# nv-tlabs/3dgrut

Measured on AMD Instinct MI355X. Metric: train rays/sec (3DGUT forward+backward, primary rays), higher is better.
Workload: dtype f32; 1 GPU; 3DGUT fwd+bwd, 1000000 Gaussians (cloud B trained-like, seed 42), 1920x1080, one view per GPU, SH degree 3, k_buffer 0; parallelism=view-dp1

## Files before the change

3dgrut_amd/_abi.py:

```python
from __future__ import annotations

import ctypes as C
import os

ABI_VERSION = 5
_HERE = os.path.dirname(os.path.abspath(__file__))
LIB_PATH = os.path.join(_HERE, "csrc", "libgrut_amd.so")

SHUTTER_ROLLING_TOP_TO_BOTTOM, SHUTTER_ROLLING_LEFT_TO_RIGHT, SHUTTER_ROLLING_BOTTOM_TO_TOP, \
    SHUTTER_ROLLING_RIGHT_TO_LEFT, SHUTTER_GLOBAL = range(5)
CAMERA_OPENCV_PINHOLE, CAMERA_OPENCV_FISHEYE, CAMERA_FTHETA = range(3)
FTHETA_PIXELDIST_TO_ANGLE, FTHETA_ANGLE_TO_PIXELDIST = range(2)

GUT_STAGES = ["project", "depth_sort", "scan", "expand", "tile_sort", "tile_ranges", "render_fwd", "render_bwd", "project_bwd"]

GRUT_OK = 0
STATUS_NAMES = {0: "OK", -1: "BAD_INPUT", -2: "RUNTIME", -3: "NOT_READY", -4: "UNSUPPORTED"}


class GrutCamera(C.Structure):
    _fields_ = [
        ("model", C.c_int32), ("shutter", C.c_int32), ("width", C.c_int32), ("height", C.c_int32),
        ("principal_point", C.c_float * 2), ("focal_length", C.c_float * 2),
        ("radial", C.c_float * 6), ("tangential", C.c_float * 2), ("thin_prism", C.c_float * 4),
# ... 26 lines not shown
        ("width", C.c_int32), ("height", C.c_int32), ("camera", GrutCamera),
        ("pose_start", C.c_float * 7), ("pose_end", C.c_float * 7),
        ("device_T_to_world", C.c_void_p), ("device_T_to_world_end", C.c_void_p), ("out_features", C.c_void_p), ("out_opacity", C.c_void_p),
    ]


class GutStats(C.Structure):
    _fields_ = [
        ("num_particles", C.c_uint32), ("num_visible", C.c_uint32), ("num_intersections", C.c_uint64),
        ("num_tiles", C.c_uint32), ("key_bits", C.c_uint32),
        ("fwd_entries_evaluated", C.c_uint64), ("fwd_entries_accepted", C.c_uint64),
        ("bwd_entries_evaluated", C.c_uint64), ("bwd_entries_accepted", C.c_uint64),
    ]


class GrtConfig(C.Structure):
    _fields_ = [
        ("particle_kernel_degree", C.c_int32), ("particle_kernel_min_response", C.c_float),
        ("particle_kernel_min_alpha", C.c_float), ("particle_kernel_max_alpha", C.c_float),
        ("particle_kernel_density_clamping", C.c_int32), ("particle_radiance_sph_degree", C.c_int32),
        ("enable_normals", C.c_int32), ("enable_hitcounts", C.c_int32), ("enable_kernel_timings", C.c_int32),
        ("max_hits_per_trace", C.c_int32), ("particle_feature_half", C.c_int32), ("feature_output_half", C.c_int32),
        ("feature_transform_type", C.c_int32), ("particle_feature_dim", C.c_int32), ("interp_point_feature_dim", C.c_int32),
        ("feature_interpolation_support", C.c_int32), ("feature_activation_type", C.c_int32), ("feature_activation_num_frequencies", C.c_int32),
        ("primitive_type", C.c_int32), ("pipeline_type", C.c_int32),
    ]


class GrtFrame(C.Structure):
    _fields_ = [
        ("frame_id", C.c_uint32), ("sph_degree", C.c_int32), ("min_transmittance", C.c_float),
        ("num_particles", C.c_uint32), ("width", C.c_int32), ("height", C.c_int32),
        ("ray_to_world", C.c_float * 12), ("keep_hits_for_backward", C.c_int32), ("device_ray_to_world", C.c_void_p),
    ]


class GrtStats(C.Structure):
    _fields_ = [
        ("num_particles", C.c_uint32), ("num_nodes", C.c_uint32), ("nodes_visited", C.c_uint64),
        ("candidates", C.c_uint64), ("processed_hits", C.c_uint64), ("scene_aabb", C.c_float * 6),
        ("list_entries", C.c_uint64), ("packet_tests", C.c_uint64), ("list_batches", C.c_uint64),
        ("bwd_rederived_rays", C.c_uint32), ("bwd_premise_rays", C.c_uint32),
        ("bwd_atomic_instructions", C.c_uint64), ("bwd_atomic_words", C.c_uint64),
    ]


class GrutAdamGroup(C.Structure):
    _fields_ = [
        ("param", C.c_void_p), ("grad", C.c_void_p), ("exp_avg", C.c_void_p), ("exp_avg_sq", C.c_void_p),
        ("row_width", C.c_uint32), ("lr", C.c_float), ("beta1", C.c_float), ("beta2", C.c_float), ("eps", C.c_float),
    ]


VIS_NONE, VIS_BOOL_U8, VIS_INT32, VIS_FLOAT_BITS = range(4)
GRT_PRIMITIVES = {"instances": 0, "icosahedron": 1, "octahedron": 2, "tetrahedron": 3, "diamond": 4, "custom": 5, "trisurfel": 6, "trihexa": 7, "sphere": 8}


class GrtTexture(C.Structure):
    _fields_ = [("data", C.c_void_p), ("height", C.c_int32), ("width", C.c_int32), ("channels", C.c_int32)]


class GrtMaterial(C.Structure):
    _fields_ = [("diffuse", GrtTexture), ("emissive", GrtTexture), ("metallic_roughness", GrtTexture), ("normal", GrtTexture),
                ("diffuse_factor", C.c_float * 4), ("emissive_factor", C.c_float * 3), ("metallic_factor", C.c_float), ("roughness_factor", C.c_float),
                ("transmission_factor", C.c_float), ("ior", C.c_float), ("alpha_cutoff", C.c_float), ("alpha_mode", C.c_uint32)]


class GrtMesh(C.Structure):
    _fields_ = [("num_vertices", C.c_uint32), ("num_faces", C.c_uint32), ("vertices", C.c_void_p), ("triangles", C.c_void_p),
                ("vertex_normals", C.c_void_p), ("vertex_tangents", C.c_void_p), ("vertex_has_tangents", C.c_void_p), ("prim_type", C.c_void_p),
                ("mat_uv", C.c_void_p), ("mat_id", C.c_void_p), ("refractive_index", C.c_void_p), ("num_materials", C.c_uint32),
                ("materials", C.POINTER(GrtMaterial)), ("envmap", GrtTexture), ("envmap_offset", C.c_float * 2)]


class GrtHybridOptions(C.Structure):
    _fields_ = [("playground_opts", C.c_uint32), ("max_pbr_bounces", C.c_uint32), ("frame_number", C.c_uint32)]



class GutGradIO(C.Structure):
    _fields_ = [("grad_features", C.c_void_p), ("grad_opacity", C.c_void_p), ("grad_positions", C.c_void_p), ("grad_density", C.c_void_p),
                ("grad_rotation", C.c_void_p), ("grad_scale", C.c_void_p)]

MLP_ACT_NONE, MLP_ACT_RELU, MLP_ACT_SIGMOID = range(3)
PPISP_CONTROLLER_SAVED = 1984


class GrutMlpConfig(C.Structure):
    _fields_ = [("n_features", C.c_int32), ("sh_degree", C.c_int32), ("n_hidden_layers", C.c_int32), ("width", C.c_int32),
                ("n_output_dims", C.c_int32), ("output_activation", C.c_int32)]


class GrutDecodeConfig(C.Structure):
    _fields_ = [("mlp", GrutMlpConfig), ("sh_scale", C.c_float), ("unpremultiply_alpha", C.c_int32), ("center_ray", C.c_int32)]


class GrutDenoiseConfig(C.Structure):
    _fields_ = [("patch_radius", C.c_int32), ("search_radius", C.c_int32), ("h", C.c_float)]


class McmcTensor(C.Structure):
    _fields_ = [("data", C.c_void_p), ("row_elems", C.c_uint32), ("role", C.c_uint32)]


MCMC_MAX_TENSORS = 32
MCMC_ROLE_COPY, MCMC_ROLE_NEW_DENSITY, MCMC_ROLE_NEW_SCALE, MCMC_ROLE_STATE = range(4)


EXPORTED_SYMBOLS = [
    "gut_create", "gut_destroy", "gut_forward", "gut_backward", "gut_backward_unpacked", "gut_forward_split", "gut_backward_split", "gut_backward_unpacked_split", "gut_backward_factored", "gut_backward_factored_chunked", "grut_sph_grad_from_views", "gut_timings", "gut_stats",
    "gut_profile_enable", "gut_profile_select", "gut_profile_read",
    "gut_debug_fetch", "gut_debug_fetch_work", "grut_debug_pose_from_c2w", "grut_debug_frame_poses", "grut_sort_pairs_u32", "grut_sort_scratch_bytes", "grut_inclusive_scan_u32",
    "grut_scan_scratch_bytes", "grut_debug_sort_pairs_u32", "grut_debug_scan_gather_u32", "gut_debug_tile_ranges", "grt_debug_list_ranges",
    "grt_create", "grt_destroy", "grt_build_bvh", "grt_forward", "grt_backward", "grt_timings", "grt_stats", "grt_debug_fetch_work",
    "grt_debug_forward_hits", "grt_debug_fetch_instances", "grt_debug_fetch_custom_boxes", "grt_debug_fetch_lists", "grt_debug_backward_signature", "grt_build_mesh_bvh", "grt_trace_hybrid",
    "grut_selective_adam_update", "grut_pack_particles", "grut_unpack_particle_grads", "grut_activate_pack", "grut_activate_pack_backward",
    "grut_reg_partials", "grut_reg_forward", "grut_reg_backward",
    "grut_denoise",
    "grut_mcmc_relocation", "grut_mcmc_perturb",
    "grut_mcmc_classify", "grut_mcmc_classify_scratch_bytes", "grut_mcmc_sample_plan", "grut_mcmc_relocate_rows", "grut_mcmc_append_rows",
    "grut_densify_accumulate", "grut_relayout_scan", "grut_relayout_scratch_bytes", "grut_relayout_rows", "grut_split_tail",
    "grut_ssim_forward", "grut_ssim_backward", "grut_ssim_partials",
    "grut_photo_loss_forward", "grut_photo_loss_backward", "grut_photo_loss_partials",
    "grut_knn", "grut_knn_scratch_bytes",
    "grut_ppisp_forward", "grut_ppisp_backward", "grut_ppisp_partials",
    "grut_ppisp_controller_forward", "grut_ppisp_controller_backward", "grut_ppisp_controller_forward_scratch", "grut_ppisp_controller_backward_scratch",
    "grut_mlp_forward", "grut_mlp_lds_bytes", "grut_mlp_num_params",
    "grut_mlp_backward", "grut_mlp_backward_lds_bytes", "grut_mlp_backward_scratch_bytes",
    "grut_decode_forward", "grut_decode_backward",
    "grut_last_error", "grut_abi_version", "grut_set_allocator", "gut_trim", "grt_trim",
]

_lib = None
ALLOC_FN = C.CFUNCTYPE(C.c_void_p, C.c_void_p, C.c_uint64)
FREE_FN = C.CFUNCTYPE(None, C.c_void_p, C.c_void_p)
CHUNK_FN = C.CFUNCTYPE(None, C.c_void_p, C.c_uint32, C.c_uint32, C.c_uint32)


def _declare(lib):
    vp, fp, ip, up = C.c_void_p, C.c_void_p, C.c_void_p, C.c_void_p
    lib.gut_create.argtypes = [C.POINTER(GutConfig), C.POINTER(C.c_void_p)]
    lib.gut_create.restype = C.c_int
    lib.gut_destroy.argtypes = [C.c_void_p]
    lib.gut_destroy.restype = None
    lib.gut_forward.argtypes = [C.c_void_p, vp, C.POINTER(GutFrame), fp, fp, fp, fp, fp, fp, fp, ip]
    lib.gut_forward.restype = C.c_int
    lib.gut_backward.argtypes = [C.c_void_p, vp, C.POINTER(GutFrame)] + [fp] * 10
    lib.gut_backward.restype = C.c_int
    lib.gut_backward_factored.argtypes = [C.c_void_p, vp, C.POINTER(GutFrame)] + [fp] * 10
    lib.gut_backward_factored.restype = C.c_int
    lib.gut_backward_factored_chunked.argtypes = [C.c_void_p, vp, C.POINTER(GutFrame)] + [fp] * 10 + [C.c_uint32, CHUNK_FN, C.c_void_p]
    lib.gut_backward_factored_chunked.restype = C.c_int
    lib.gut_backward_unpacked.argtypes = [C.c_void_p, vp, C.POINTER(GutFrame)] + [fp] * 7 + [C.POINTER(GutGradIO), fp]
    lib.gut_backward_unpacked.restype = C.c_int
    lib.gut_forward_split.argtypes = [C.c_void_p, vp, C.POINTER(GutFrame), fp, fp, fp, fp, fp, fp, fp, fp, ip]
    lib.gut_forward_split.restype = C.c_int
    lib.gut_backward_split.argtypes = [C.c_void_p, vp, C.POINTER(GutFrame)] + [fp] * 12
    lib.gut_backward_split.restype = C.c_int
    lib.gut_backward_unpacked_split.argtypes = [C.c_void_p, vp, C.POINTER(GutFrame)] + [fp] * 8 + [C.POINTER(GutGradIO), fp, fp]
    lib.gut_backward_unpacked_split.restype = C.c_int
    lib.grut_sph_grad_from_views.argtypes = [vp, C.c_uint32, C.c_uint32, fp, fp, C.c_uint32, C.c_int32, C.c_int32, C.c_float, fp]
    lib.grut_sph_grad_from_views.restype = C.c_int
    lib.gut_timings.argtypes = [C.c_void_p, C.POINTER(C.c_float), C.POINTER(C.c_float)]
    lib.gut_timings.restype = C.c_int
    lib.gut_stats.argtypes = [C.c_void_p, C.POINTER(GutStats)]
    lib.gut_stats.restype = C.c_int
    lib.gut_profile_enable.argtypes = [C.c_void_p, C.c_int]
    lib.gut_profile_enable.restype = C.c_int
    lib.gut_profile_select.argtypes = [C.c_void_p, C.c_uint32]
    lib.gut_profile_select.restype = C.c_int
    lib.gut_profile_read.argtypes = [C.c_void_p, C.POINTER(C.c_float)]
    lib.gut_profile_read.restype = C.c_int
    lib.gut_debug_fetch_work.argtypes = [C.c_void_p, vp, up, C.c_uint64]
    lib.gut_debug_fetch_work.restype = C.c_int
    lib.grut_debug_pose_from_c2w.argtypes = [C.POINTER(C.c_float), C.POINTER(C.c_float)]
    lib.grut_debug_pose_from_c2w.restype = C.c_int
    lib.grut_debug_frame_poses.argtypes = [vp, C.c_int, vp, vp, C.POINTER(C.c_float)]
    lib.grut_debug_frame_poses.restype = C.c_int
    lib.gut_debug_fetch.argtypes = [C.c_void_p, vp] + [up] * 8
    lib.gut_debug_fetch.restype = C.c_int
    lib.grut_sort_pairs_u32.argtypes = [vp, C.c_uint32, C.c_int, C.c_int, up, up, up, up, vp, C.c_uint64,
                                        C.POINTER(C.c_void_p), C.POINTER(C.c_void_p)]
    lib.grut_sort_pairs_u32.restype = C.c_int
    lib.grut_sort_scratch_bytes.argtypes = [C.c_uint32]
    lib.grut_sort_scratch_bytes.restype = C.c_uint64
    lib.grut_inclusive_scan_u32.argtypes = [vp, C.c_uint32, up, up, vp, C.c_uint64]
    lib.grut_inclusive_scan_u32.restype = C.c_int
    lib.grut_scan_scratch_bytes.argtypes = [C.c_uint32]
    lib.grut_scan_scratch_bytes.restype = C.c_uint64
    lib.grut_debug_sort_pairs_u32.argtypes = [vp, C.c_uint32, up, C.c_int, C.c_int, up, up, up, up, C.c_int, vp, C.c_uint64,
                                              C.POINTER(C.c_void_p), C.POINTER(C.c_void_p)]
    lib.grut_debug_sort_pairs_u32.restype = C.c_int
    lib.grut_debug_scan_gather_u32.argtypes = [vp, C.c_uint32, up, up, up, vp, C.c_uint64]
    lib.grut_debug_scan_gather_u32.restype = C.c_int
    lib.gut_debug_tile_ranges.argtypes = [vp, C.c_uint32, up, C.c_uint32, C.c_uint32, up, up, up, C.POINTER(C.c_uint32)]
    lib.gut_debug_tile_ranges.restype = C.c_int
    lib.grt_debug_list_ranges.argtypes = [vp, C.c_uint32, up, C.c_uint32, up, up]
    lib.grt_debug_list_ranges.restype = C.c_int
    lib.grt_debug_fetch_lists.argtypes = [C.c_void_p, vp, up, up, C.c_uint64]
    lib.grt_debug_fetch_lists.restype = C.c_int
    lib.grt_create.argtypes = [C.POINTER(GrtConfig), C.POINTER(C.c_void_p)]
    lib.grt_create.restype = C.c_int
    lib.grt_destroy.argtypes = [C.c_void_p]
    lib.grt_destroy.restype = None
    lib.grt_build_bvh.argtypes = [C.c_void_p, vp, C.c_uint32, fp, fp, fp, fp, C.c_int, C.c_int]
    lib.grt_build_bvh.restype = C.c_int
    lib.grt_forward.argtypes = [C.c_void_p, vp, C.POINTER(GrtFrame)] + [fp] * 9 + [ip]
    lib.grt_forward.restype = C.c_int
    lib.grt_backward.argtypes = [C.c_void_p, vp, C.POINTER(GrtFrame)] + [fp] * 14
    lib.grt_backward.restype = C.c_int
    lib.grt_debug_forward_hits.argtypes = [C.c_void_p, vp, C.POINTER(GrtFrame)] + [fp] * 9 + [ip, up, up, C.c_uint32]
    lib.grt_debug_forward_hits.restype = C.c_int
    lib.grt_debug_fetch_instances.argtypes = [C.c_void_p, vp, fp]
    lib.grt_debug_fetch_instances.restype = C.c_int
    lib.grt_debug_fetch_custom_boxes.argtypes = [C.c_void_p, vp, fp]
    lib.grt_debug_fetch_custom_boxes.restype = C.c_int
    lib.grt_debug_backward_signature.argtypes = [C.c_void_p, up, up]
    lib.grt_debug_backward_signature.restype = C.c_int
    lib.grt_build_mesh_bvh.argtypes = [C.c_void_p, vp, C.c_uint32, fp, C.c_uint32, ip, C.c_int, C.c_int]
    lib.grt_build_mesh_bvh.restype = C.c_int
    lib.grt_trace_hybrid.argtypes = [C.c_void_p, vp, C.POINTER(GrtFrame), fp, fp, fp, fp, fp, C.POINTER(GrtMesh), C.POINTER(GrtHybridOptions), fp, fp, fp, up]
    lib.grt_trace_hybrid.restype = C.c_int
    lib.grt_timings.argtypes = [C.c_void_p, C.POINTER(C.c_float), C.POINTER(C.c_float), C.POINTER(C.c_float)]
    lib.grt_timings.restype = C.c_int
    lib.grut_set_allocator.argtypes = [ALLOC_FN, FREE_FN, C.c_void_p]
    lib.grut_set_allocator.restype = C.c_int
    lib.gut_trim.argtypes = [C.c_void_p]
    lib.gut_trim.restype = C.c_int
    lib.grt_trim.argtypes = [C.c_void_p]
    lib.grt_trim.restype = C.c_int
    lib.grt_debug_fetch_work.argtypes = [C.c_void_p, vp, up, C.c_uint64]
    lib.grt_debug_fetch_work.restype = C.c_int
    lib.grt_stats.argtypes = [C.c_void_p, C.POINTER(GrtStats)]
    lib.grt_stats.restype = C.c_int
    lib.grut_selective_adam_update.argtypes = [vp, C.POINTER(GrutAdamGroup), C.c_int, C.c_uint32, vp, C.c_int]
    lib.grut_selective_adam_update.restype = C.c_int
    lib.grut_pack_particles.argtypes = [vp, C.c_uint32, fp, fp, fp, fp, fp]
    lib.grut_pack_particles.restype = C.c_int
    lib.grut_unpack_particle_grads.argtypes = [vp, C.c_uint32] + [fp] * 5
    lib.grut_unpack_particle_grads.restype = C.c_int
    lib.grut_activate_pack.argtypes = [vp, C.c_uint32, fp, fp, fp, fp, fp]
    lib.grut_activate_pack.restype = C.c_int
    lib.grut_activate_pack_backward.argtypes = [vp, C.c_uint32] + [fp] * 8
# ... 223 lines not shown
```

3dgrut_amd/csrc/gut_api.hip:

```cpp
#include <initializer_list>
#include <vector>

#include "gut_internal.hpp"

namespace grut {

static thread_local char g_last_error[512] = "";
ScratchAllocator& scratch_allocator() {
    static ScratchAllocator a;
    return a;
}
void set_last_error(const char* fmt, ...) {
    va_list ap;
    va_start(ap, fmt);
    vsnprintf(g_last_error, sizeof(g_last_error), fmt, ap);
    va_end(ap);
}

static uint32_t bits_for(uint32_t n) {
    uint32_t b = 1;
    while ((1ull << b) <= n) ++b;
    return b;
}

}

using namespace grut;

struct GutHandle {
    GutConfig cfg;
    int device = -1;
    DeviceBuffer tiles_count, proj_pos, conic_opacity, extent, depth, rgb, depth_key, particle_idx;
    DeviceBuffer depth_key_tmp, particle_idx_tmp, offsets, sort_scratch, scan_scratch, counters;
    DeviceBuffer rec64;
    DeviceBuffer part_offset, pos_particle, grad_partial, grad_flag, grad_touched, g_rgb, poses_dev, walk8;
    bool flags_dirty = false;
    DeviceBuffer tile_keys, tile_vals, tile_keys_tmp, tile_vals_tmp, tile_sort_scratch, ranges;
    DeviceBuffer ck_tc, ck_d, ck_reached, ck_boundary_tile, ck_nht;
    GutCheckpoints checkpoints;
    uint32_t* host_counters = nullptr;
    hipEvent_t count_event = nullptr;
    bool have_forward = false;
    hipStream_t fwd_stream = nullptr;
    const void* fwd_density = nullptr;
    const void* fwd_ray_o = nullptr;
    const void* fwd_ray_d = nullptr;
    uint32_t fwd_frame_id = 0;
    GutParams params;
    uint32_t num_intersections = 0;
    uint32_t tile_capacity = 0;
    uint32_t ck_boundaries_capacity = 0;
    uint32_t* sorted_pos = nullptr;
    uint32_t* sorted_tile_keys = nullptr;
    uint32_t* rank_to_particle = nullptr;
    GutStats stats;
    EventTimer fwd_timer, bwd_timer;
    bool profile = false;
    bool count_work = false;
    DeviceBuffer work_counters;
    unsigned long long work_host[4] = {0, 0, 0, 0};
    bool work_pending = false;
    static constexpr int kProfRing = 64;
    hipEvent_t prof_ev[kProfRing][GUT_NUM_STAGES][2];
    bool prof_used[kProfRing][GUT_NUM_STAGES];
    int prof_slot = 0, prof_created = 0;
    int prof_fwd_slot = 0;

    uint32_t profile_mask = 0xFFFFFFFFu;
    int stage_begin(int stage, hipStream_t s, int slot) {
        if (!profile || !((profile_mask >> stage) & 1u)) return GRUT_OK;
        GRUT_HIP(hipEventRecord(prof_ev[slot][stage][0], s));
        return GRUT_OK;
    }
    int stage_end(int stage, hipStream_t s, int slot) {
        if (!profile || !((profile_mask >> stage) & 1u)) return GRUT_OK;
        GRUT_HIP(hipEventRecord(prof_ev[slot][stage][1], s));
        prof_used[slot][stage] = true;
        return GRUT_OK;
    }
};

static int validate_config(const GutConfig& c) {
    GRUT_REQUIRE(c.ut_require_all_sigma_points_valid == 0, "ut_require_all_sigma_points_valid must be false (threedgut.cuh:78)");
    GRUT_REQUIRE(c.particle_radiance_sph_degree >= 0 && c.particle_radiance_sph_degree <= 3, "sph degree must be in [0,3]");
    if (c.k_buffer_size != 0 && c.k_buffer_size != 4 && c.k_buffer_size != 8 && c.k_buffer_size != 16) {
        set_last_error("k_buffer_size=%d: the hit buffer is instantiated for 0 (unsorted), 4, 8 and 16 entries", c.k_buffer_size);
        return GRUT_ERR_UNSUPPORTED;
    }
    if (c.feature_transform_type != 0) {
        GRUT_REQUIRE(c.feature_transform_type == 1, "feature_transform_type %d: 0 (SH) or 1 (neural harmonic features)", c.feature_transform_type);
        GRUT_REQUIRE(c.feature_interpolation_support == 0 || c.feature_interpolation_support == 1, "feature_interpolation_support must be 0 (centre) or 1 (tetrahedra)");
        GRUT_REQUIRE(c.feature_activation_type >= 0 && c.feature_activation_type <= 3, "feature_activation_type must be 0..3");
        const int points = c.feature_interpolation_support == 1 ? 4 : 1;
        GRUT_REQUIRE(c.interp_point_feature_dim >= 1 && c.interp_point_feature_dim <= 16 && c.particle_feature_dim == points * c.interp_point_feature_dim,
                     "particle_feature_dim %d must be %d x interp_point_feature_dim (1..16)", c.particle_feature_dim, points);
        const int nf = c.feature_activation_num_frequencies;
        const int nr = c.interp_point_feature_dim * (c.feature_activation_type == 2 ? 2 * nf : (c.feature_activation_type == 1 ? nf : 1));
        GRUT_REQUIRE(nf >= 1 && nr >= 1 && nr <= 32, "ray feature dim %d: 1..32 supported", nr);
    }
    const int d = c.particle_kernel_degree;
    GRUT_REQUIRE(d == 0 || d == 1 || d == 2 || d == 3 || d == 4 || d == 5 || d == 8, "unsupported particle_kernel_degree %d", d);
    return GRUT_OK;
}

static GutParams make_params(const GutConfig& c, const GutFrame& f) {
    GutParams P;
    memset(&P, 0, sizeof(P));
    P.degree = c.particle_kernel_degree;
    P.min_response = c.particle_kernel_min_response;
    P.min_alpha = c.particle_kernel_min_alpha;
    P.max_alpha = c.particle_kernel_max_alpha;
    P.min_transmittance = c.min_transmittance;
    P.n_active = f.n_active_features < c.particle_radiance_sph_degree ? f.n_active_features : c.particle_radiance_sph_degree;
    if (P.n_active < 0) P.n_active = 0;
    P.ncoef = (c.particle_radiance_sph_degree + 1) * (c.particle_radiance_sph_degree + 1);
    P.hitcounts = c.enable_hitcounts;
    const float D = 3.f;
    const float lambda = c.ut_alpha * c.ut_alpha * (D + c.ut_kappa) - D;
    P.ut_w0m = lambda / (D + lambda);
    P.ut_wi = 1.f / (2.f * (D + lambda));
    P.ut_w0c = lambda / (D + lambda) + (1.f - c.ut_alpha * c.ut_alpha + c.ut_beta);
    P.ut_delta = sqrtf(c.ut_alpha * c.ut_alpha * (D + c.ut_kappa));
    P.ut_margin = c.ut_in_image_margin_factor;
    P.ut_require_all = c.ut_require_all_sigma_points_valid;
    P.n_rs_iter = c.n_rolling_shutter_iterations;
    P.k_buffer = c.k_buffer_size;
    P.global_z = c.global_z_order;
// ... 48 lines not shown
}

static int ensure_intersection_scratch(GutHandle* h, uint32_t I, uint32_t tiles) {
    const size_t n = I ? I : 1;
    if (n > h->tile_capacity) h->tile_capacity = (uint32_t)n;
    GRUT_CHECK(h->tile_keys.ensure(n * 4, 1.3f));
    GRUT_CHECK(h->tile_vals.ensure(n * 4, 1.3f));
    GRUT_CHECK(h->tile_keys_tmp.ensure(n * 4, 1.3f));
    GRUT_CHECK(h->tile_vals_tmp.ensure(n * 4, 1.3f));
    GRUT_CHECK(h->pos_particle.ensure(n * 4, 1.3f));
    GRUT_CHECK(h->tile_sort_scratch.ensure(sort_scratch_bytes((uint32_t)n), 1.3f));
    GRUT_CHECK(h->ranges.ensure((size_t)tiles * 8 + 8));
    const size_t nb = (size_t)I / kGutSegment + 1;
    if (!h->params.nht && h->params.k_buffer == 0) {
        GRUT_CHECK(h->ck_tc.ensure(nb * 4 * 64 * 16, 1.3f));
        GRUT_CHECK(h->ck_d.ensure(nb * 4 * 64 * 4, 1.3f));
    }
    GRUT_CHECK(h->ck_reached.ensure(nb * 4, 1.3f));
    GRUT_CHECK(h->ck_boundary_tile.ensure(nb * 4, 1.3f));
    h->checkpoints.tc = h->ck_tc.as<float4>();
    h->checkpoints.d = h->ck_d.as<float>();
    h->checkpoints.reached = h->ck_reached.as<uint8_t>();
    h->checkpoints.boundary_tile = h->ck_boundary_tile.as<uint32_t>();
    h->checkpoints.num_boundaries = (uint32_t)nb;
    h->ck_boundaries_capacity = (uint32_t)nb;
    if (nht_fast_path(h->params)) GRUT_CHECK(h->ck_nht.ensure(nht_checkpoint_bytes((uint32_t)nb), 1.3f));
    return GRUT_OK;
}

static GutProjected projected_view(GutHandle* h) {
    GutProjected p;
    p.tiles_count = h->tiles_count.as<uint32_t>();
    p.proj_pos = h->proj_pos.as<float2>();
    p.conic_opacity = h->conic_opacity.as<float4>();
    p.extent = h->extent.as<float2>();
    p.depth = h->depth.as<float>();
    p.rgb = h->rgb.as<float>();
    p.depth_key = h->depth_key.as<uint32_t>();
    p.particle_idx = h->particle_idx.as<uint32_t>();
    p.part_offset = h->part_offset.as<uint32_t>();
    p.rec64 = h->rec64.as<float4>();
    static const bool no_walk_cache = getenv("GRUT_GUT_NO_WALK_CACHE") != nullptr;
    p.walk8 = (no_walk_cache || h->params.gx >= 4096 || h->params.gy >= 4096) ? nullptr : h->walk8.as<uint2>();
    return p;
}

extern "C" {

int grut_abi_version(void) { return GRUT_ABI_VERSION; }
int grut_set_allocator(GrutAllocFn alloc_fn, GrutFreeFn free_fn, void* user) {
    GRUT_REQUIRE((alloc_fn == nullptr) == (free_fn == nullptr), "grut_set_allocator: give both functions or neither");
    grut::ScratchAllocator& a = grut::scratch_allocator();
    a.alloc = alloc_fn;
    a.release = free_fn;
    a.user = user;
    return GRUT_OK;
}
const char* grut_last_error(void) { return grut::g_last_error; }

int gut_create(const GutConfig* config, GutHandle** handle) {
    GRUT_REQUIRE(config && handle, "gut_create: null argument");
    GRUT_CHECK(validate_config(*config));
    GutHandle* h = new GutHandle();
    h->cfg = *config;
    memset(&h->stats, 0, sizeof(h->stats));
    if (hipGetDevice(&h->device) != hipSuccess) {
        set_last_error("gut_create: no HIP device");
        delete h;
        return GRUT_ERR_RUNTIME;
    }
    if (hipHostMalloc(reinterpret_cast<void**>(&h->host_counters), 64, hipHostMallocDefault) != hipSuccess ||
        hipEventCreateWithFlags(&h->count_event, hipEventDisableTiming) != hipSuccess) {
        set_last_error("gut_create: pinned counter / event allocation failed");
        delete h;
        return GRUT_ERR_RUNTIME;
    }
    *handle = h;
    return GRUT_OK;
}

static void release_scratch(GutHandle* h) {
    DeviceBuffer* bufs[] = {&h->tiles_count, &h->proj_pos, &h->conic_opacity, &h->extent, &h->depth, &h->rgb, &h->depth_key,
                            &h->particle_idx, &h->depth_key_tmp, &h->particle_idx_tmp, &h->offsets, &h->sort_scratch,
                            &h->scan_scratch, &h->counters, &h->rec64, &h->walk8, &h->part_offset, &h->pos_particle, &h->grad_partial, &h->grad_flag,
                            &h->grad_touched,
                            &h->g_rgb, &h->poses_dev, &h->work_counters, &h->tile_keys, &h->tile_vals, &h->tile_keys_tmp,
                            &h->tile_vals_tmp, &h->tile_sort_scratch, &h->ranges, &h->ck_tc, &h->ck_d, &h->ck_nht, &h->ck_reached,
                            &h->ck_boundary_tile};
    for (DeviceBuffer* b : bufs) b->release();
}

int gut_trim(GutHandle* h) {
    GRUT_REQUIRE(h, "gut_trim: null handle");
    if (h->fwd_stream) GRUT_HIP(hipStreamSynchronize(h->fwd_stream));
    else GRUT_HIP(hipDeviceSynchronize());
    release_scratch(h);
    h->tile_capacity = 0;
    h->have_forward = false;
    h->num_intersections = 0;
    h->sorted_pos = nullptr;
    h->sorted_tile_keys = nullptr;
    h->work_pending = false;
    h->flags_dirty = false;
    h->ck_boundaries_capacity = 0;
    memset(&h->checkpoints, 0, sizeof(h->checkpoints));
    return GRUT_OK;
}

void gut_destroy(GutHandle* h) {
    if (!h) return;
    release_scratch(h);
    if (h->host_counters) (void)hipHostFree(h->host_counters);
    if (h->count_event) (void)hipEventDestroy(h->count_event);
    h->fwd_timer.destroy();
    h->bwd_timer.destroy();
    if (h->prof_created)
        for (int r = 0; r < GutHandle::kProfRing; ++r)
            for (int st = 0; st < GUT_NUM_STAGES; ++st) {
                (void)hipEventDestroy(h->prof_ev[r][st][0]);
                (void)hipEventDestroy(h->prof_ev[r][st][1]);
            }
    delete h;
}

static int forward_impl(GutHandle* h, void* stream_, const GutFrame* frame, const float* particle_density, const void* particle_sph_,
                        const GutSplitSph& split, const float* ray_origin, const float* ray_direction, void* out_feat_density_,
                        float* out_hit_distance, float* out_hit_count, int32_t* out_visibility) {
    const float* particle_sph = reinterpret_cast<const float*>(particle_sph_);
    float* out_feat_density = reinterpret_cast<float*>(out_feat_density_);
    GRUT_REQUIRE(h && frame, "gut_forward: null handle/frame");
    GRUT_REQUIRE(frame->width > 0 && frame->height > 0, "gut_forward: empty image");
    GRUT_REQUIRE(ray_origin && ray_direction && out_feat_density && out_hit_distance && out_hit_count, "gut_forward: null ray/output buffer");
    hipStream_t s = reinterpret_cast<hipStream_t>(stream_);
    ScratchStreamScope scratch_scope(s);
    h->have_forward = false;
    const uint32_t N = frame->num_particles;
    h->params = make_params(h->cfg, *frame);
    const GutParams& P = h->params;
    const uint32_t tiles = (uint32_t)(P.gx * P.gy);
    h->stats.num_particles = N;
    h->stats.num_tiles = tiles;
    h->stats.num_visible = 0;
    h->stats.num_intersections = 0;
    h->stats.key_bits = bits_for(tiles);
    h->num_intersections = 0;
    h->fwd_stream = s;
    h->fwd_density = particle_density;
    h->fwd_ray_o = ray_origin;
    h->fwd_ray_d = ray_direction;
    h->fwd_frame_id = frame->frame_id;
    if (N == 0) {
        h->have_forward = true;
        return GRUT_OK;
    }
    GRUT_REQUIRE(particle_density && (particle_sph || split.specular) && out_visibility, "gut_forward: null particle buffer");
    GRUT_REQUIRE(!h->cfg.feature_output_half || (!frame->out_features && !frame->out_opacity), "gut_forward: feature_output_half excludes out_features / out_opacity");
    GRUT_REQUIRE(!h->cfg.feature_transform_type || (!frame->out_features && !frame->out_opacity), "gut_forward: neural harmonic features exclude out_features / out_opacity");
    if (h->cfg.enable_kernel_timings) GRUT_CHECK(h->fwd_timer.begin(s));

    GRUT_CHECK(ensure_particle_scratch(h, N));
    static const bool legacy_lists = getenv("GRUT_GUT_LEGACY_LISTS") != nullptr;
    const bool direct = h->stats.key_bits <= 16 && !legacy_lists;
    h->params.rec64 = direct ? h->rec64.as<float4>() : nullptr;
    h->params.ord_shift = h->stats.key_bits;
    h->params.sorted_keys = nullptr;
    if (frame->device_T_to_world) {
        GRUT_CHECK(h->poses_dev.ensure(sizeof(FramePoses)));
        launch_frame_poses(s, frame->device_T_to_world, frame->device_T_to_world_end, h->poses_dev.as<FramePoses>());
        h->params.poses_dev = h->poses_dev.as<FramePoses>();
    }
    if (h->count_work) {
        const size_t fwd_words = 16 + 4 * ((((size_t)tiles + 7) & ~(size_t)7) * 2);
        GRUT_CHECK(h->work_counters.ensure(fwd_words * 8 + 8192 + ((size_t)h->tile_capacity / kGutSegment + tiles + 64) * 2 * 16, 1.2f));
        GRUT_HIP(hipMemsetAsync(h->work_counters.ptr, 0, h->work_counters.bytes, s));
        h->params.work = h->work_counters.as<unsigned long long>();
        h->params.work_task_capacity = (uint32_t)((h->work_counters.bytes / 8 - fwd_words) / 2);
        h->work_pending = true;
    }
    const GutProjected proj = projected_view(h);
    uint32_t* d_counters = h->counters.as<uint32_t>();

    const int slot = h->prof_slot % GutHandle::kProfRing;
    if (h->profile) {
        for (int st = 0; st < GUT_NUM_STAGES; ++st) h->prof_used[slot][st] = false;
        h->prof_fwd_slot = slot;
        h->prof_slot++;
    }
    GRUT_CHECK(h->stage_begin(GUT_STAGE_PROJECT, s, slot));
    launch_project(s, P, particle_density, particle_sph, split, proj, out_visibility, d_counters + 1);
    GRUT_CHECK(h->stage_end(GUT_STAGE_PROJECT, s, slot));
    GRUT_CHECK(h->stage_begin(GUT_STAGE_DEPTH_SORT, s, slot));
    uint32_t *sorted_depth = nullptr, *rank_to_particle = nullptr;
    GRUT_CHECK(sort_pairs_u32(s, N, nullptr, 0, 32, proj.depth_key, proj.particle_idx, h->depth_key_tmp.as<uint32_t>(),
                              h->particle_idx_tmp.as<uint32_t>(), h->sort_scratch.ptr, h->sort_scratch.bytes, &sorted_depth,
                              &rank_to_particle, true));
    h->rank_to_particle = rank_to_particle;
    GRUT_CHECK(h->stage_end(GUT_STAGE_DEPTH_SORT, s, slot));
    GRUT_CHECK(h->stage_begin(GUT_STAGE_SCAN, s, slot));
    GRUT_CHECK(inclusive_scan_u32(s, N, proj.tiles_count, rank_to_particle, h->offsets.as<uint32_t>(), h->scan_scratch.ptr,
                                  h->scan_scratch.bytes));
    GRUT_CHECK(h->stage_end(GUT_STAGE_SCAN, s, slot));
    GRUT_CHECK(h->ranges.ensure((size_t)tiles * 8 + 8));
    launch_prepare_tail(s, h->offsets.as<uint32_t>() + (N - 1), d_counters + 1, h->host_counters, h->ranges.as<uint32_t>(), tiles * 2u,
                        h->ck_reached.as<uint32_t>(), h->ck_reached.ptr ? h->ck_boundaries_capacity : 0u);
    GRUT_HIP(hipEventRecord(h->count_event, s));
    const uint32_t tile_mask = (h->stats.key_bits >= 32) ? 0xFFFFFFFFu : ((1u << h->stats.key_bits) - 1u);
    bool first_tail = true;
    auto enqueue_tail = [&](uint32_t n, const uint32_t* n_dev) -> int {
        GRUT_CHECK(h->stage_begin(GUT_STAGE_EXPAND, s, slot));
        launch_expand(s, P, proj, rank_to_particle, h->offsets.as<uint32_t>(), n, h->tile_keys.as<uint32_t>(),
                      direct ? h->tile_vals.as<uint32_t>() : nullptr , h->pos_particle.as<uint32_t>());
        GRUT_CHECK(h->stage_end(GUT_STAGE_EXPAND, s, slot));
        GRUT_CHECK(h->stage_begin(GUT_STAGE_TILE_SORT, s, slot));
        uint32_t *sorted_tiles = nullptr, *sorted_idx = nullptr;
        GRUT_CHECK(sort_pairs_u32(s, n, n_dev, 0, (int)h->stats.key_bits, h->tile_keys.as<uint32_t>(), h->tile_vals.as<uint32_t>(),
                                  h->tile_keys_tmp.as<uint32_t>(), h->tile_vals_tmp.as<uint32_t>(), h->tile_sort_scratch.ptr,
                                  h->tile_sort_scratch.bytes, &sorted_tiles, &sorted_idx, !direct));
        h->sorted_tile_keys = sorted_tiles;
        h->params.sorted_keys = sorted_tiles;
        h->sorted_pos = sorted_idx;
        GRUT_CHECK(h->stage_end(GUT_STAGE_TILE_SORT, s, slot));
        GRUT_CHECK(h->stage_begin(GUT_STAGE_TILE_RANGES, s, slot));
        if (!first_tail) {
            GRUT_HIP(hipMemsetAsync(h->ranges.ptr, 0, (size_t)tiles * 8, s));
            GRUT_HIP(hipMemsetAsync(h->ck_reached.ptr, 0, (size_t)h->ck_boundaries_capacity * 4, s));
        }
        first_tail = false;
        launch_tile_ranges(s, n, n_dev, tile_mask, tiles, sorted_tiles, h->ranges.as<uint32_t>(), h->checkpoints.boundary_tile);
        GRUT_CHECK(h->stage_end(GUT_STAGE_TILE_RANGES, s, slot));
        GRUT_CHECK(h->stage_begin(GUT_STAGE_RENDER_FWD, s, slot));
        if (nht_fast_path(P))
            launch_render_nhtp_fwd(s, P, h->ranges.as<uint32_t>(), sorted_idx, h->pos_particle.as<uint32_t>(), particle_density, particle_sph, ray_origin,
                                   ray_direction, out_feat_density, out_hit_distance, out_hit_count, h->ck_nht.ptr, h->checkpoints, true);
        else if (P.nht)
            launch_render_nht_fwd(s, P, h->ranges.as<uint32_t>(), sorted_idx, h->pos_particle.as<uint32_t>(), particle_density, particle_sph, ray_origin,
                                  ray_direction, out_feat_density, out_hit_distance, out_hit_count);
        else if (P.k_buffer > 0)
            launch_render_k_fwd(s, P, h->ranges.as<uint32_t>(), sorted_idx, h->pos_particle.as<uint32_t>(), particle_density, proj.rgb, ray_origin,
                                ray_direction, out_feat_density, out_hit_distance, out_hit_count);
        else
            launch_render_fwd(s, P, h->ranges.as<uint32_t>(), sorted_idx, h->pos_particle.as<uint32_t>(), particle_density, proj.rgb, ray_origin,
                              ray_direction, out_feat_density, out_hit_distance, out_hit_count, h->checkpoints, true);
        GRUT_CHECK(h->stage_end(GUT_STAGE_RENDER_FWD, s, slot));
        return GRUT_OK;
    };
    const bool speculative = h->tile_capacity > 0;
    if (speculative) GRUT_CHECK(enqueue_tail(h->tile_capacity, h->offsets.as<uint32_t>() + (N - 1)));
    GRUT_HIP(hipEventSynchronize(h->count_event));
    const uint32_t I = h->host_counters[0];
    h->stats.num_visible = h->host_counters[1];
    h->stats.num_intersections = I;
    h->num_intersections = I;
    if (I == 0) {
        const float far = 1e6f;
        uint32_t bits;
        memcpy(&bits, &far, 4);
        GRUT_HIP(hipMemsetAsync(out_feat_density, 0, (size_t)P.W * P.H * (P.nht ? P.nht_ray_dim + 1 : 4) * (P.out_half ? 2 : 4), s));
        GRUT_HIP(hipMemsetD32Async(reinterpret_cast<hipDeviceptr_t>(out_hit_distance), (int)bits, (size_t)P.W * P.H, s));
        GRUT_HIP(hipMemsetAsync(out_hit_count, 0, (size_t)P.W * P.H * 4, s));
        if (P.out_features) GRUT_HIP(hipMemsetAsync(P.out_features, 0, (size_t)P.W * P.H * 12, s));
        if (P.out_opacity) GRUT_HIP(hipMemsetAsync(P.out_opacity, 0, (size_t)P.W * P.H * 4, s));
        if (h->cfg.enable_kernel_timings) GRUT_CHECK(h->fwd_timer.end(s));
        h->have_forward = true;
        return GRUT_OK;
    }
    if (!speculative || I > h->tile_capacity) {
        GRUT_CHECK(ensure_intersection_scratch(h, I + I / 2, tiles));
        first_tail = false;
        GRUT_CHECK(enqueue_tail(I, nullptr));
    }
    h->checkpoints.num_boundaries = I / kGutSegment + 1;
    GRUT_HIP(hipGetLastError());
    if (h->cfg.enable_kernel_timings) GRUT_CHECK(h->fwd_timer.end(s));
    h->have_forward = true;
    return GRUT_OK;
}

int gut_forward(GutHandle* h, void* stream, const GutFrame* frame, const float* particle_density, const void* particle_sph,
                const float* ray_origin, const float* ray_direction, void* out_feat_density, float* out_hit_distance,
                float* out_hit_count, int32_t* out_visibility) {
    return forward_impl(h, stream, frame, particle_density, particle_sph, GutSplitSph{}, ray_origin, ray_direction, out_feat_density,
                        out_hit_distance, out_hit_count, out_visibility);
}

static int split_preconditions(const GutHandle* h, const char* who, std::initializer_list<const void*> buffers) {
    GRUT_REQUIRE(h, "%s: null handle", who);
    const GutConfig& cfg = h->cfg;
    const char* why = cfg.feature_transform_type ? "neural harmonic features have no albedo / specular tensors"
                      : cfg.particle_feature_half ? "particle_feature_half (the model's tensors are fp32)"
                      : cfg.particle_radiance_sph_degree != 3 ? "particle_radiance_sph_degree != 3 (the tensors are [N,3] and [N,45])"
                      : cfg.k_buffer_size != 0 ? "k_buffer_size > 0 (the sorted mode runs on the [N,48] buffer)" : nullptr;
    if (why) {
        set_last_error("%s: unsupported configuration: %s", who, why);
        return GRUT_ERR_UNSUPPORTED;
    }
    for (const void* p : buffers) {
        GRUT_REQUIRE(p, "%s: null albedo / specular buffer", who);
        GRUT_REQUIRE((reinterpret_cast<uintptr_t>(p) & 15u) == 0, "%s: the albedo / specular buffers must be 16-byte aligned", who);
    }
    return GRUT_OK;
}

int gut_forward_split(GutHandle* h, void* stream, const GutFrame* frame, const float* particle_density, const float* sph_albedo,
                      const float* sph_specular, const float* ray_origin, const float* ray_direction, void* out_feat_density,
                      float* out_hit_distance, float* out_hit_count, int32_t* out_visibility) {
    GRUT_CHECK(split_preconditions(h, "gut_forward_split", {sph_albedo, sph_specular}));
    return forward_impl(h, stream, frame, particle_density, nullptr, GutSplitSph{sph_albedo, sph_specular}, ray_origin, ray_direction,
                        out_feat_density, out_hit_distance, out_hit_count, out_visibility);
}

static int prepare_grad_slots(GutHandle* h, hipStream_t s, size_t I, GutGradSlots& slots) {
    const size_t touched_bytes = h->grad_touched.bytes, flag_bytes = h->grad_flag.bytes;
    GRUT_CHECK(h->grad_partial.ensure(2 * I * (size_t)slots.stride * 4, 1.3f));
    GRUT_CHECK(h->grad_touched.ensure((size_t)h->params.N * 8, 1.25f));
    GRUT_CHECK(h->grad_flag.ensure(2 * I, 1.3f));
    if (h->flags_dirty || h->grad_touched.bytes != touched_bytes) GRUT_HIP(hipMemsetAsync(h->grad_touched.ptr, 0, h->grad_touched.bytes, s));
    if (h->flags_dirty || h->grad_flag.bytes != flag_bytes) GRUT_HIP(hipMemsetAsync(h->grad_flag.ptr, 0, h->grad_flag.bytes, s));
    h->flags_dirty = true;
    slots.partial = h->grad_partial.as<float>();
    slots.touched = h->grad_touched.as<unsigned long long>();
    slots.flag = h->grad_flag.as<uint8_t>();
    return GRUT_OK;
}

static int backward_impl(GutHandle* h, void* stream_, const GutFrame* frame, const float* particle_density, const void* particle_sph_,
                         const float* ray_origin, const float* ray_direction, const void* feat_density_, const float* grad_feat_density,
                         const float* hit_distance, const float* grad_hit_distance, float* grad_particle_density, float* grad_particle_sph,
                         float* grad_radiance, const GutGradIO* io = nullptr, uint32_t num_chunks = 1, GrutChunkFn on_chunk = nullptr,
                         void* chunk_user = nullptr, const GutSplitSph& split = {}, const GutSplitSphGrad& g_split = {}) {
    const float* particle_sph = reinterpret_cast<const float*>(particle_sph_);
    const float* feat_density = reinterpret_cast<const float*>(feat_density_);
    GRUT_REQUIRE(h && frame, "gut_backward: null handle/frame");
    hipStream_t s = reinterpret_cast<hipStream_t>(stream_);
    ScratchStreamScope scratch_scope(s);
    if (!h->have_forward || h->fwd_stream != s) {
        set_last_error("gut_backward: no forward context on this stream");
        return GRUT_ERR_NOT_READY;
    }
    const GutParams& P = h->params;
    GRUT_REQUIRE(frame->num_particles == P.N && frame->width == P.W && frame->height == P.H, "gut_backward: frame differs from the forward frame");
    if (frame->frame_id != h->fwd_frame_id || (P.N > 0 && (particle_density != h->fwd_density || ray_origin != h->fwd_ray_o || ray_direction != h->fwd_ray_d))) {
        set_last_error("gut_backward: the forward context belongs to another forward (a later gut_forward ran on this handle before this "
                       "backward); run each backward before the next forward, or use one handle per in-flight frame");
        return GRUT_ERR_NOT_READY;
    }
    if (P.N == 0) return GRUT_OK;
    if (P.nht) {
        if (grad_radiance) {
            set_last_error("gut_backward_factored: neural harmonic features have no per-view factorisation; reduce the dense gradients");
            return GRUT_ERR_UNSUPPORTED;
        }
        const bool fast = nht_fast_path(P);
        if (io && !fast) {
            set_last_error("gut_backward_unpacked: this feature shape runs on the generic kernels, which write packed gradients only");
            return GRUT_ERR_UNSUPPORTED;
        }
        GRUT_REQUIRE(particle_density && particle_sph && feat_density && (io || grad_feat_density) && hit_distance && (io || grad_particle_density) &&
                         grad_particle_sph, "gut_backward: null buffer");
        if (h->cfg.enable_kernel_timings) GRUT_CHECK(h->bwd_timer.begin(s));
        GRUT_HIP(hipMemsetAsync(grad_particle_sph, 0, (size_t)P.N * P.nht_k * 4, s));
        const size_t I = h->num_intersections;
        if (fast) {
            const int slot = h->prof_fwd_slot;
            const GutProjected proj = projected_view(h);
            const GutGradOut g_out = io ? GutGradOut{nullptr, io->grad_positions, io->grad_density, io->grad_rotation, io->grad_scale}
                                        : GutGradOut{grad_particle_density, nullptr, nullptr, nullptr, nullptr};
            if (io) {
                GRUT_REQUIRE(io->grad_positions && io->grad_density && io->grad_rotation && io->grad_scale, "gut_backward_unpacked: null gradient output");
                GRUT_REQUIRE((reinterpret_cast<uintptr_t>(io->grad_rotation) & 15u) == 0, "gut_backward_unpacked: grad_rotation must be 16-byte aligned");
            }
            GutGradSlots slots;
            slots.stride = 16;
            slots.partial = nullptr;
            slots.touched = nullptr;
            slots.flag = nullptr;
            slots.pos_particle = h->pos_particle.as<uint32_t>();
            slots.part_offset = proj.part_offset;
            if (I > 0) {
                GRUT_CHECK(prepare_grad_slots(h, s, I, slots));
                GRUT_CHECK(h->stage_begin(GUT_STAGE_RENDER_BWD, s, slot));
                launch_render_nhtp_bwd(s, P, h->ranges.as<uint32_t>(), h->sorted_pos, particle_density, particle_sph, ray_origin, ray_direction, feat_density,
                                       io ? nullptr : grad_feat_density, io ? io->grad_features : nullptr, io ? io->grad_opacity : nullptr, hit_distance,
                                       grad_hit_distance, slots, grad_particle_sph, h->ck_nht.ptr, h->checkpoints);
                GRUT_CHECK(h->stage_end(GUT_STAGE_RENDER_BWD, s, slot));
            }
            GRUT_CHECK(h->stage_begin(GUT_STAGE_PROJECT_BWD, s, slot));
            launch_grad_finalize_nht(s, P, proj, particle_density, slots, I > 0, g_out);
            GRUT_CHECK(h->stage_end(GUT_STAGE_PROJECT_BWD, s, slot));
            GRUT_HIP(hipGetLastError());
            h->flags_dirty = false;
        } else {
            GRUT_HIP(hipMemsetAsync(grad_particle_density, 0, (size_t)P.N * 48, s));
            if (I > 0)
                launch_render_nht_bwd(s, P, h->ranges.as<uint32_t>(), h->sorted_pos, h->pos_particle.as<uint32_t>(), particle_density, particle_sph, ray_origin,
                                      ray_direction, feat_density, grad_feat_density, hit_distance, grad_hit_distance, grad_particle_density, grad_particle_sph);
        }
        GRUT_HIP(hipGetLastError());
        if (h->cfg.enable_kernel_timings) GRUT_CHECK(h->bwd_timer.end(s));
        return GRUT_OK;
    }
    const GutGradIn g_in = io ? GutGradIn{nullptr, io->grad_features, io->grad_opacity} : GutGradIn{grad_feat_density, nullptr, nullptr};
    const GutGradOut g_out = io ? GutGradOut{nullptr, io->grad_positions, io->grad_density, io->grad_rotation, io->grad_scale}
                                : GutGradOut{grad_particle_density, nullptr, nullptr, nullptr, nullptr};
    if (io) {
        GRUT_REQUIRE(io->grad_positions && io->grad_density && io->grad_rotation && io->grad_scale, "gut_backward_unpacked: null gradient output");
        GRUT_REQUIRE((reinterpret_cast<uintptr_t>(io->grad_rotation) & 15u) == 0, "gut_backward_unpacked: grad_rotation must be 16-byte aligned");
        if (P.k_buffer > 0) {
            set_last_error("gut_backward_unpacked: the sorted (k_buffer_size > 0) backward accumulates into packed rows; use gut_backward");
            return GRUT_ERR_UNSUPPORTED;
        }
    }
    GRUT_REQUIRE(particle_density && (particle_sph || split.specular) && feat_density && (io || grad_feat_density) && hit_distance &&
                     (io || grad_particle_density) && (grad_particle_sph || grad_radiance || g_split.specular), "gut_backward: null buffer");
    if (h->cfg.enable_kernel_timings) GRUT_CHECK(h->bwd_timer.begin(s));
    const GutProjected proj = projected_view(h);
    const int slot = h->prof_fwd_slot;
    const bool has_gdist = grad_hit_distance != nullptr;
    GutGradSlots slots;
    slots.stride = has_gdist ? 20 : 16;
    slots.partial = nullptr;
    slots.touched = nullptr;
    slots.flag = nullptr;
    slots.pos_particle = h->pos_particle.as<uint32_t>();
    slots.part_offset = proj.part_offset;
    const size_t I = h->num_intersections;
    if (P.k_buffer > 0) {
        GRUT_CHECK(h->g_rgb.ensure((size_t)P.N * 12, 1.25f));
        GRUT_HIP(hipMemsetAsync(h->g_rgb.ptr, 0, (size_t)P.N * 12, s));
        GRUT_HIP(hipMemsetAsync(grad_particle_density, 0, (size_t)P.N * 48, s));
        if (I > 0) {
            GRUT_CHECK(h->stage_begin(GUT_STAGE_RENDER_BWD, s, slot));
            launch_render_k_bwd(s, P, h->ranges.as<uint32_t>(), h->sorted_pos, h->pos_particle.as<uint32_t>(), particle_density, proj.rgb, ray_origin,
                                ray_direction, feat_density, grad_feat_density, hit_distance, grad_hit_distance, grad_particle_density,
                                h->g_rgb.as<float>());
            GRUT_CHECK(h->stage_end(GUT_STAGE_RENDER_BWD, s, slot));
        }
        GRUT_CHECK(h->stage_begin(GUT_STAGE_PROJECT_BWD, s, slot));
        launch_project_bwd(s, P, proj, particle_density, particle_sph, split, h->g_rgb.as<float>(), g_out, grad_particle_sph, g_split, grad_radiance);
        GRUT_CHECK(h->stage_end(GUT_STAGE_PROJECT_BWD, s, slot));
        GRUT_HIP(hipGetLastError());
        if (h->cfg.enable_kernel_timings) GRUT_CHECK(h->bwd_timer.end(s));
        return GRUT_OK;
    }
    if (I > 0) {
        GRUT_CHECK(prepare_grad_slots(h, s, I, slots));
        GRUT_CHECK(h->stage_begin(GUT_STAGE_RENDER_BWD, s, slot));
        launch_render_bwd(s, P, h->ranges.as<uint32_t>(), h->sorted_pos, particle_density, proj.rgb, ray_origin, ray_direction, feat_density,
                          g_in, hit_distance, grad_hit_distance, slots, h->checkpoints);
        GRUT_CHECK(h->stage_end(GUT_STAGE_RENDER_BWD, s, slot));
    }
    GRUT_CHECK(h->stage_begin(GUT_STAGE_PROJECT_BWD, s, slot));
    GRUT_CHECK(h->g_rgb.ensure((size_t)P.N * 12, 1.25f));
    if (num_chunks <= 1 || !on_chunk) {
        launch_grad_finalize(s, P, proj, particle_density, particle_sph, split, slots, has_gdist, I > 0, h->g_rgb.as<float>(), g_out,
                             grad_particle_sph, g_split, grad_radiance);
    } else {
        const uint32_t per = ((P.N + num_chunks - 1) / num_chunks + 127u) & ~127u;
        uint32_t c = 0;
        for (uint32_t first = 0; first < P.N; first += per, ++c) {
            const uint32_t end = first + per < P.N ? first + per : P.N;
            launch_grad_finalize(s, P, proj, particle_density, particle_sph, split, slots, has_gdist, I > 0, h->g_rgb.as<float>(), g_out,
                                 grad_particle_sph, g_split, grad_radiance, first, end);
            on_chunk(chunk_user, c, first, end - first);
        }
    }
    GRUT_CHECK(h->stage_end(GUT_STAGE_PROJECT_BWD, s, slot));
    GRUT_HIP(hipGetLastError());
    h->flags_dirty = false;
    if (h->cfg.enable_kernel_timings) GRUT_CHECK(h->bwd_timer.end(s));
    return GRUT_OK;
}

int gut_backward(GutHandle* h, void* stream, const GutFrame* frame, const float* particle_density, const void* particle_sph,
                 const float* ray_origin, const float* ray_direction, const void* feat_density, const float* grad_feat_density,
                 const float* hit_distance, const float* grad_hit_distance, float* grad_particle_density, float* grad_particle_sph) {
    return backward_impl(h, stream, frame, particle_density, particle_sph, ray_origin, ray_direction, feat_density, grad_feat_density, hit_distance,
                         grad_hit_distance, grad_particle_density, grad_particle_sph, nullptr);
}

int gut_backward_unpacked(GutHandle* h, void* stream, const GutFrame* frame, const float* particle_density, const void* particle_sph,
                          const float* ray_origin, const float* ray_direction, const void* feat_density, const float* hit_distance,
                          const float* grad_hit_distance, const GutGradIO* io, float* grad_particle_sph) {
    GRUT_REQUIRE(io, "gut_backward_unpacked: null GutGradIO");
    return backward_impl(h, stream, frame, particle_density, particle_sph, ray_origin, ray_direction, feat_density, nullptr, hit_distance,
                         grad_hit_distance, nullptr, grad_particle_sph, nullptr, io);
}

int gut_backward_split(GutHandle* h, void* stream, const GutFrame* frame, const float* particle_density, const float* sph_albedo,
                       const float* sph_specular, const float* ray_origin, const float* ray_direction, const void* feat_density,
                       const float* grad_feat_density, const float* hit_distance, const float* grad_hit_distance, float* grad_particle_density,
                       float* grad_sph_albedo, float* grad_sph_specular) {
    GRUT_CHECK(split_preconditions(h, "gut_backward_split", {sph_albedo, sph_specular, grad_sph_albedo, grad_sph_specular}));
    return backward_impl(h, stream, frame, particle_density, nullptr, ray_origin, ray_direction, feat_density, grad_feat_density, hit_distance,
                         grad_hit_distance, grad_particle_density, nullptr, nullptr, nullptr, 1, nullptr, nullptr,
                         GutSplitSph{sph_albedo, sph_specular}, GutSplitSphGrad{grad_sph_albedo, grad_sph_specular});
}

int gut_backward_unpacked_split(GutHandle* h, void* stream, const GutFrame* frame, const float* particle_density, const float* sph_albedo,
                                const float* sph_specular, const float* ray_origin, const float* ray_direction, const void* feat_density,
                                const float* hit_distance, const float* grad_hit_distance, const GutGradIO* io, float* grad_sph_albedo,
                                float* grad_sph_specular) {
    GRUT_CHECK(split_preconditions(h, "gut_backward_unpacked_split", {sph_albedo, sph_specular, grad_sph_albedo, grad_sph_specular}));
    GRUT_REQUIRE(io, "gut_backward_unpacked_split: null GutGradIO");
    return backward_impl(h, stream, frame, particle_density, nullptr, ray_origin, ray_direction, feat_density, nullptr, hit_distance,
                         grad_hit_distance, nullptr, nullptr, nullptr, io, 1, nullptr, nullptr, GutSplitSph{sph_albedo, sph_specular},
                         GutSplitSphGrad{grad_sph_albedo, grad_sph_specular});
}

int gut_backward_factored(GutHandle* h, void* stream, const GutFrame* frame, const float* particle_density, const void* particle_sph,
                          const float* ray_origin, const float* ray_direction, const void* feat_density, const float* grad_feat_density,
                          const float* hit_distance, const float* grad_hit_distance, float* grad_particle_density, float* grad_radiance) {
    GRUT_REQUIRE(grad_radiance, "gut_backward_factored: null buffer");
    return backward_impl(h, stream, frame, particle_density, particle_sph, ray_origin, ray_direction, feat_density, grad_feat_density, hit_distance,
                         grad_hit_distance, grad_particle_density, nullptr, grad_radiance);
}

int gut_backward_factored_chunked(GutHandle* h, void* stream, const GutFrame* frame, const float* particle_density, const void* particle_sph,
                                  const float* ray_origin, const float* ray_direction, const void* feat_density, const float* grad_feat_density,
                                  const float* hit_distance, const float* grad_hit_distance, float* grad_particle_density, float* grad_radiance,
                                  uint32_t num_chunks, GrutChunkFn on_chunk, void* user) {
    GRUT_REQUIRE(grad_radiance && on_chunk && num_chunks >= 1, "gut_backward_factored_chunked: null buffer / callback");
    GRUT_REQUIRE(!h || h->cfg.k_buffer_size == 0, "gut_backward_factored_chunked: the sorted mode finalises in one piece");
    return backward_impl(h, stream, frame, particle_density, particle_sph, ray_origin, ray_direction, feat_density, grad_feat_density, hit_distance,
                         grad_hit_distance, grad_particle_density, nullptr, grad_radiance, nullptr, num_chunks < 2 ? 2 : num_chunks, on_chunk, user);
}

int grut_sph_grad_from_views(void* stream, uint32_t num_particles, uint32_t num_views, const float* view_factors, const float* positions,
                             uint32_t position_stride, int32_t n_active_features, int32_t sph_degree, float scale, float* grad_particle_sph) {
    GRUT_REQUIRE(num_views > 0 && sph_degree >= 0 && sph_degree <= 3 && position_stride >= 3, "grut_sph_grad_from_views: bad arguments");
    if (num_particles == 0) return GRUT_OK;
    GRUT_REQUIRE(view_factors && positions && grad_particle_sph, "grut_sph_grad_from_views: null buffer");
    launch_sph_grad_from_views(reinterpret_cast<hipStream_t>(stream), num_particles, num_views, view_factors, positions, position_stride,
                               n_active_features, (sph_degree + 1) * (sph_degree + 1), scale, grad_particle_sph);
    GRUT_HIP(hipGetLastError());
    return GRUT_OK;
}

int gut_timings(GutHandle* h, float* forward_ms, float* backward_ms) {
    GRUT_REQUIRE(h, "gut_timings: null handle");
    if (forward_ms) *forward_ms = h->fwd_timer.collect();
    if (backward_ms) *backward_ms = h->bwd_timer.collect();
    return GRUT_OK;
}

int gut_profile_enable(GutHandle* h, int enable) {
    GRUT_REQUIRE(h, "gut_profile_enable: null handle");
    if (enable && h->prof_created == 0) {
        for (int r = 0; r < GutHandle::kProfRing; ++r)
            for (int st = 0; st < GUT_NUM_STAGES; ++st) {
                GRUT_HIP(hipEventCreate(&h->prof_ev[r][st][0]));
                GRUT_HIP(hipEventCreate(&h->prof_ev[r][st][1]));
                h->prof_used[r][st] = false;
            }
        h->prof_created = 1;
    }
    h->profile = enable != 0;
    h->count_work = enable >= 2;
    return GRUT_OK;
}

int gut_profile_select(GutHandle* h, uint32_t stage_mask) {
    GRUT_REQUIRE(h, "gut_profile_select: null handle");
    h->profile_mask = stage_mask;
    return GRUT_OK;
}

int gut_profile_read(GutHandle* h, float* stage_ms) {
    GRUT_REQUIRE(h && stage_ms, "gut_profile_read: null argument");
    GRUT_REQUIRE(h->prof_created, "gut_profile_read: profiling was never enabled");
    for (int st = 0; st < GUT_NUM_STAGES; ++st) {
        double sum = 0;
        int n = 0;
        for (int r = 0; r < GutHandle::kProfRing; ++r) {
            if (!h->prof_used[r][st]) continue;
            float ms = 0.f;
            GRUT_HIP(hipEventSynchronize(h->prof_ev[r][st][1]));
            GRUT_HIP(hipEventElapsedTime(&ms, h->prof_ev[r][st][0], h->prof_ev[r][st][1]));
            sum += ms;
            n++;
            h->prof_used[r][st] = false;
        }
        stage_ms[st] = n ? (float)(sum / n) : -1.f;
    }
    h->prof_slot = 0;
    return GRUT_OK;
}

int gut_stats(GutHandle* h, GutStats* stats) {
    GRUT_REQUIRE(h && stats, "gut_stats: null argument");
// ... 64 lines not shown
```

3dgrut_amd/csrc/gut_internal.hpp:

```cpp
#pragma once

#include "camera.hpp"
#include "common.hpp"

namespace grut {

struct GutParams {
    int degree;
    float min_response, min_alpha, max_alpha, min_transmittance;
    int n_active, ncoef, hitcounts;
    float ut_w0m, ut_wi, ut_w0c, ut_delta, ut_margin;
    int ut_require_all, n_rs_iter, k_buffer, global_z, rect_bounding, tight_opacity, tile_culling;
    int W, H, gx, gy;
    uint32_t N;
    GrutCamera cam;
    FramePoses poses;
    unsigned long long* work;
    const float4* rec64;
    const uint32_t* sorted_keys;
    uint32_t ord_shift;
    int nht, nht_k, nht_ipd, nht_support, nht_act, nht_nf, nht_ray_dim;
    int sph_half, out_half;
    uint32_t work_task_capacity;
    float* out_features;
    float* out_opacity;
    const FramePoses* poses_dev;
};
#ifdef __HIPCC__
__device__ __forceinline__ const FramePoses& frame_poses(const GutParams& P) { return P.poses_dev ? *P.poses_dev : P.poses; }
#endif
void launch_frame_poses(hipStream_t s, const float* T_start, const float* T_end, FramePoses* out);
void launch_prepare_tail(hipStream_t s, const uint32_t* last_offset, uint32_t* num_visible, uint32_t* host_counters, uint32_t* ranges_words,
                         uint32_t n_ranges_words, uint32_t* reached_words, uint32_t n_reached_words);

struct GutProjected {
    uint32_t* tiles_count;
    float2* proj_pos;
    float4* conic_opacity;
    float2* extent;
    float* depth;
    float* rgb;
    uint32_t* depth_key;
    uint32_t* particle_idx;
    uint32_t* part_offset;
    float4* rec64;
    uint2* walk8;
};

struct GutGradSlots {
    float* partial;
    unsigned long long* touched;
    uint8_t* flag;
    const uint32_t* pos_particle;
    const uint32_t* part_offset;
    int stride;
};
constexpr uint32_t kGutTouchBits = 64;

struct GutGradOut {
    float* packed;
    float* pos;
    float* dns;
    float* rot;
    float* scl;
};
struct GutGradIn {
    const float* fd;
    const float* rgb;
    const float* opa;
};
struct GutSplitSph {
    const float* albedo = nullptr;
    const float* specular = nullptr;
};
struct GutSplitSphGrad {
    float* albedo = nullptr;
    float* specular = nullptr;
};
#ifdef __HIPCC__
__device__ __forceinline__ float4 load_grad_in(const GutGradIn& g, size_t pix) {
    if (g.fd) return reinterpret_cast<const float4*>(g.fd)[pix];
    float4 r = make_float4(0.f, 0.f, 0.f, 0.f);
    if (g.rgb) { r.x = g.rgb[3 * pix]; r.y = g.rgb[3 * pix + 1]; r.z = g.rgb[3 * pix + 2]; }
    if (g.opa) r.w = g.opa[pix];
    return r;
}
#endif

#ifndef GRUT_GUT_SEGMENT
#define GRUT_GUT_SEGMENT 64
#endif
constexpr uint32_t kGutSegment = GRUT_GUT_SEGMENT;

struct GutCheckpoints {
    float4* tc;
    float* d;
    uint8_t* reached;
    uint32_t* boundary_tile;
    uint32_t num_boundaries;
};

constexpr uint32_t kGutCounterReplicas = 64, kGutCounterStride = 32, kGutCounterWords = kGutCounterReplicas * kGutCounterStride + 32;
void launch_project(hipStream_t s, const GutParams& P, const float* density12, const float* sph, const GutSplitSph& split, const GutProjected& out,
                    int32_t* visibility, uint32_t* num_visible);
void launch_expand(hipStream_t s, const GutParams& P, const GutProjected& proj, const uint32_t* rank_to_particle,
                   const uint32_t* offsets, uint32_t capacity, uint32_t* tile_keys, uint32_t* tile_vals, uint32_t* pos_particle);
void launch_gather_particle_idx(hipStream_t s, uint32_t n, const uint32_t* sorted_pos, const uint32_t* pos_particle, uint32_t* out);
void launch_tile_ranges(hipStream_t s, uint32_t n, const uint32_t* n_dev, uint32_t tile_mask, uint32_t num_tiles,
                        const uint32_t* sorted_tile_keys, uint32_t* ranges, uint32_t* boundary_tile);
void launch_render_fwd(hipStream_t s, const GutParams& P, const uint32_t* ranges, const uint32_t* sorted_pos, const uint32_t* pos_particle,
                       const float* density12,
                       const float* rgb, const float* ray_o, const float* ray_d, float* out_fd, float* out_dist, float* out_cnt,
                       const GutCheckpoints& ck, bool write_checkpoints);
void launch_render_bwd(hipStream_t s, const GutParams& P, const uint32_t* ranges, const uint32_t* sorted_pos, const float* density12,
                       const float* rgb, const float* ray_o, const float* ray_d, const float* fd, const GutGradIn& g_fd, const float* dist,
                       const float* g_dist, const GutGradSlots& slots, const GutCheckpoints& ck);
void launch_render_nht_fwd(hipStream_t s, const GutParams& P, const uint32_t* ranges, const uint32_t* sorted_pos, const uint32_t* pos_particle,
                           const float* density12, const float* features, const float* ray_o, const float* ray_d, float* out_fd, float* out_dist,
                           float* out_cnt);
void launch_render_nht_bwd(hipStream_t s, const GutParams& P, const uint32_t* ranges, const uint32_t* sorted_pos, const uint32_t* pos_particle,
                           const float* density12, const float* features, const float* ray_o, const float* ray_d, const float* fd, const float* g_fd,
                           const float* dist, const float* g_dist, float* g_density12, float* g_features);
bool nht_fast_path(const GutParams& P);
uint64_t nht_checkpoint_bytes(uint32_t num_boundaries);
void launch_render_nhtp_fwd(hipStream_t s, const GutParams& P, const uint32_t* ranges, const uint32_t* sorted_pos, const uint32_t* pos_particle,
                            const float* density12, const float* features, const float* ray_o, const float* ray_d, float* out_fd, float* out_dist,
                            float* out_cnt, void* ck_nht, const GutCheckpoints& ck, bool write_checkpoints);
void launch_render_nhtp_bwd(hipStream_t s, const GutParams& P, const uint32_t* ranges, const uint32_t* sorted_pos, const float* density12,
                            const float* features, const float* ray_o, const float* ray_d, const float* fd, const float* g_fd, const float* g_feat,
                            const float* g_opa, const float* dist, const float* g_dist, const GutGradSlots& slots, float* g_features,
                            const void* ck_nht, const GutCheckpoints& ck);
void launch_grad_finalize_nht(hipStream_t s, const GutParams& P, const GutProjected& proj, const float* density12, const GutGradSlots& slots,
                              bool have_partials, const GutGradOut& g_out);
void launch_render_k_fwd(hipStream_t s, const GutParams& P, const uint32_t* ranges, const uint32_t* sorted_pos, const uint32_t* pos_particle,
                         const float* density12, const float* rgb, const float* ray_o, const float* ray_d, float* out_fd, float* out_dist,
                         float* out_cnt);
void launch_render_k_bwd(hipStream_t s, const GutParams& P, const uint32_t* ranges, const uint32_t* sorted_pos, const uint32_t* pos_particle,
                         const float* density12, const float* rgb, const float* ray_o, const float* ray_d, const float* fd, const float* g_fd,
                         const float* dist, const float* g_dist, float* g_density12, float* g_rgb);
void launch_project_bwd(hipStream_t s, const GutParams& P, const GutProjected& proj, const float* density12, const float* sph,
                        const GutSplitSph& split, const float* g_rgb, const GutGradOut& g_out, float* g_sph, const GutSplitSphGrad& g_split,
                        float* g_radiance, uint32_t first = 0u, uint32_t end = 0xFFFFFFFFu);
void launch_grad_finalize(hipStream_t s, const GutParams& P, const GutProjected& proj, const float* density12, const float* sph,
                          const GutSplitSph& split, const GutGradSlots& slots, bool has_gdist, bool have_partials, float* g_rgb,
                          const GutGradOut& g_out, float* g_sph, const GutSplitSphGrad& g_split, float* g_radiance, uint32_t first = 0u,
                          uint32_t end = 0xFFFFFFFFu);
void launch_sph_grad_from_views(hipStream_t s, uint32_t N, uint32_t n_views, const float* factors, const float* positions, uint32_t pos_stride,
                                int n_active, int ncoef, float scale, float* g_sph);

}
```

3dgrut_amd/csrc/gut_kernels.hip:

```cpp
#include <cstdlib>

#include <hip/hip_fp16.h>

#include "gut_internal.hpp"

namespace grut {

namespace {

#define GRUT_SH_CONSTANTS                                                                                                   \
    constexpr float kC0 = 0.28209479177387814f, kC1 = 0.4886025119029199f;                                                  \
    constexpr float kC2[5] = {1.0925484305920792f, -1.0925484305920792f, 0.31539156525252005f, -1.0925484305920792f,        \
                              0.5462742152960396f};                                                                         \
    constexpr float kC3[7] = {-0.5900435899266435f, 2.890611442640554f, -0.4570457994644658f, 0.3731763325901154f,          \
                              -0.4570457994644658f, 1.445305721320277f, -0.5900435899266435f};                               \
    (void)kC0; (void)kC1; (void)kC2; (void)kC3

__device__ __forceinline__ void sh_basis(int deg, f3 d, float b[16]) {
    GRUT_SH_CONSTANTS;
    const float x = d.x, y = d.y, z = d.z;
#pragma unroll
    for (int i = 0; i < 16; ++i) b[i] = 0.f;
    b[0] = kC0;
    if (deg > 0) {
// ... 149 lines not shown

__device__ __forceinline__ int bcast_i(int v, int src) { return __builtin_amdgcn_readlane(v, src); }
__device__ __forceinline__ float bcast_f(float v, int src) { return __int_as_float(__builtin_amdgcn_readlane(__float_as_int(v), src)); }
template <typename Emit>
__device__ __forceinline__ void coop_tile_walk(int lane, int gx, bool culling, TileBBox bb, const TileConic& co, float cx, float cy, float pmax,
                                               Emit&& emit) {
    const int lx = lane & 7, ly = lane >> 3;
    for (int by = bb.miny; by < bb.maxy; by += 8)
        for (int bx = bb.minx; bx < bb.maxx; bx += 8) {
            const int x = bx + lx, y = by + ly;
            bool keep = (x < bb.maxx) && (y < bb.maxy);
            if (keep && culling) keep = tile_min_power((float)x, (float)y, co, cx, cy) < pmax;
            emit(keep, (uint32_t)(y * gx + x));
        }
}

constexpr int kRowWalkSide = 4;
__device__ __forceinline__ int row_bcast_i(int v, int src_lane) { return __shfl(v, src_lane, 64); }
__device__ __forceinline__ float row_bcast_f(float v, int src_lane) { return __shfl(v, src_lane, 64); }
template <typename Emit>
__device__ __forceinline__ void row_tile_walk(int lane, int gx, bool culling, bool active, TileBBox bb, const TileConic& co, float cx, float cy,
                                              float pmax, Emit&& emit) {
    const int lx = lane & 3, ly = (lane >> 2) & 3;
    int bx = bb.minx, by = bb.miny;
    bool run = active && bb.minx < bb.maxx && bb.miny < bb.maxy;
    while (__ballot(run)) {
        const int x = bx + lx, y = by + ly;
        bool keep = run && (x < bb.maxx) && (y < bb.maxy);
        if (keep && culling) keep = tile_min_power((float)x, (float)y, co, cx, cy) < pmax;
        emit(keep, (uint32_t)(y * gx + x));
        bx += 4;
        if (bx >= bb.maxx) {
            bx = bb.minx;
            by += 4;
            run = run && by < bb.maxy;
        }
    }
}
__device__ __forceinline__ int bbox_area(const TileBBox& b) { return (b.maxx - b.minx) * (b.maxy - b.miny); }
__device__ __forceinline__ bool bbox_fits_row(const TileBBox& b) { return (b.maxx - b.minx) <= kRowWalkSide && (b.maxy - b.miny) <= kRowWalkSide; }
__device__ __forceinline__ bool bbox_fits_half(const TileBBox& b) {
    const int w = b.maxx - b.minx, h = b.maxy - b.miny;
    return (w <= 8 && h <= 4) || (w <= 4 && h <= 8);
}
__device__ __forceinline__ bool half_block_tile(int lane, const TileBBox& b, int& x, int& y) {
    const int hl = lane & 31;
    const bool wide = (b.maxx - b.minx) > 4;
    x = b.minx + (wide ? (hl & 7) : (hl & 3));
    y = b.miny + (wide ? (hl >> 3) : (hl >> 2));
    return (x < b.maxx) && (y < b.maxy);
}
struct GroupPick {
    int rank;
    int steps;
};
template <int GROUP>
__device__ __forceinline__ GroupPick group_rank(int lane, bool member) {
    const unsigned long long m = __ballot(member);
    const int shift = lane & ~(GROUP - 1) & 63;
    const unsigned long long gmask = (GROUP == 64) ? ~0ull : ((1ull << GROUP) - 1ull);
    const unsigned long long mine = (m >> shift) & gmask;
    GroupPick g;
    g.rank = __popcll(mine & ((1ull << (lane & (GROUP - 1))) - 1ull));
    int steps = 0;
#pragma unroll
    for (int s = 0; s < 64; s += GROUP) steps = max(steps, (int)__popcll((m >> s) & gmask));
    g.steps = steps;
    return g;
}
template <int GROUP>
__device__ __forceinline__ int group_source(int lane, bool member, const GroupPick& g, int j, bool& act) {
    const unsigned long long sel = __ballot(member && g.rank == j);
    const int shift = lane & ~(GROUP - 1) & 63;
    const unsigned long long gmask = (GROUP == 64) ? ~0ull : ((1ull << GROUP) - 1ull);
    const unsigned long long mine = (sel >> shift) & gmask;
    act = mine != 0;
    return shift | (act ? (__ffsll((long long)mine) - 1) : 0);
}

struct __attribute__((packed, aligned(4))) Float4A4 {
    float x, y, z, w;
};

template <int MODEL, int ROLLING, bool SPLIT = false>
#ifndef GRUT_PROJECT_WAVES_MAX
#define GRUT_PROJECT_WAVES_MAX 6
#endif
__global__ __launch_bounds__(256) __attribute__((amdgpu_waves_per_eu(6, GRUT_PROJECT_WAVES_MAX))) void gut_project_kernel(GutParams P, const float4* __restrict__ density12,
                                                          const float* __restrict__ sph, GutProjected out,
                                                          int32_t* __restrict__ visibility, uint32_t* __restrict__ num_visible,
                                                          const float* __restrict__ sph_specular) {
    const uint32_t i = blockIdx.x * blockDim.x + threadIdx.x;
    const int lane = threadIdx.x & 63;
    const FramePoses& FP = frame_poses(P);
    bool has_tiles = false;
    uint32_t ntiles = 0;
    int vis = 0;
    float cx = 0.f, cy = 0.f, ex = 0.f, ey = 0.f, depth = 0.f, pmax_tile = 0.f, view_z_keep = 0.f;
    float4 co = make_float4(0.f, 0.f, 0.f, 0.f);
    TileBBox bb = {0, 0, 0, 0};
    f3 pos = mk3(0.f, 0.f, 0.f);
    float4 a = make_float4(0.f, 0.f, 0.f, 0.f), b = a, c = a;
    if (i < P.N) {
        a = density12[3 * (size_t)i + 0];
        b = density12[3 * (size_t)i + 1];
        c = density12[3 * (size_t)i + 2];
        pos = mk3(a.x, a.y, a.z);
        const float opacity = a.w;

        const float view_z = add_rn_u(FP.view_t[2], add_rn(add_rn(mul_rn_u(FP.view_R[6], pos.x), mul_rn_u(FP.view_R[7], pos.y)), mul_rn_u(FP.view_R[8], pos.z)));
        view_z_keep = view_z;
        bool ok = (opacity >= P.min_alpha) && (view_z >= 0.2f);
        if (ok) {
            const m3 rotT = quat_wxyz_to_rotT(b.x, b.y, b.z, b.w);
            float spx[7], spy[7];
            int nvalid = 0;
            nvalid += project_point_with_shutter<MODEL, ROLLING>(P.cam, FP, P.n_rs_iter, pos, P.ut_margin, spx[0], spy[0]) ? 1 : 0;
            cx = spx[0] * P.ut_w0m; cy = spy[0] * P.ut_w0m;
            const f3 axes[3] = {rotT.r0 * (P.ut_delta * c.x), rotT.r1 * (P.ut_delta * c.y), rotT.r2 * (P.ut_delta * c.z)};
#pragma unroll
            for (int k = 0; k < 3; ++k) {
                nvalid += project_point_with_shutter<MODEL, ROLLING>(P.cam, FP, P.n_rs_iter, pos + axes[k], P.ut_margin, spx[k + 1], spy[k + 1]) ? 1 : 0;
                cx += P.ut_wi * spx[k + 1]; cy += P.ut_wi * spy[k + 1];
                nvalid += project_point_with_shutter<MODEL, ROLLING>(P.cam, FP, P.n_rs_iter, pos - axes[k], P.ut_margin, spx[k + 4], spy[k + 4]) ? 1 : 0;
                cx += P.ut_wi * spx[k + 4]; cy += P.ut_wi * spy[k + 4];
            }
            ok = P.ut_require_all ? (nvalid == 7) : (nvalid > 0);
            if (ok) {
                float cov0, cov1, cov2;
                {
                    const float dx = spx[0] - cx, dy = spy[0] - cy;
                    cov0 = P.ut_w0c * dx * dx; cov1 = P.ut_w0c * dx * dy; cov2 = P.ut_w0c * dy * dy;
                }
#pragma unroll
                for (int k = 1; k < 7; ++k) {
                    const float dx = spx[k] - cx, dy = spy[k] - cy;
                    cov0 += P.ut_wi * dx * dx; cov1 += P.ut_wi * dx * dy; cov2 += P.ut_wi * dy * dy;
                }
                const float ca = cov0 + 0.3f, cb = cov1, cc = cov2 + 0.3f;
                const float det = ca * cc - cb * cb;
                ok = det != 0.f;
                if (ok) {
                    const float idet = 1.f / det;
                    co.x = cc * idet; co.y = -cb * idet; co.z = ca * idet;
                    const float cov_det = cov0 * cov2 - cov1 * cov1;
                    co.w = opacity * sqrtf(fmaxf(0.000025f, cov_det * idet));
                    ok = co.w >= P.min_alpha;
                    if (ok) {
                        const float pmax = logf(co.w / P.min_alpha);
                        const float ef = P.tight_opacity ? fminf(3.33f, sqrtf(2.f * pmax)) : 3.33f;
                        const float mid = 0.5f * (ca + cc);
                        const float lambda = mid + sqrtf(fmaxf(0.01f, mid * mid - det));
                        const float radius = ef * sqrtf(lambda);
                        ex = P.rect_bounding ? fminf(ef * sqrtf(ca), radius) : radius;
                        ey = P.rect_bounding ? fminf(ef * sqrtf(cc), radius) : radius;
                        ok = radius > 0.f;
                        if (ok) {
                            vis = 1;
                            bb = tile_space_bbox(P.gx, P.gy, cx, cy, ex, ey);
                            pmax_tile = logf(co.w / P.min_alpha);
                            if (!P.tile_culling) ntiles = (uint32_t)((bb.maxx - bb.minx) * (bb.maxy - bb.miny));
                        }
                    }
                }
            }
        }
    }
    uint32_t walk_mask = 0u, walk_kind = 0u;
    if (P.tile_culling) {
        const TileConic tc = tile_conic(co);
        const int area = vis ? bbox_area(bb) : 0;
        const bool small = area > 0 && bbox_fits_row(bb);
        const int row_shift = lane & 48;
        const GroupPick rows = group_rank<16>(lane, small);
        for (int k = 0; k < rows.steps; ++k) {
            bool act;
            const int src = group_source<16>(lane, small, rows, k, act);
            const TileBBox sb = {row_bcast_i(bb.minx, src), row_bcast_i(bb.miny, src), row_bcast_i(bb.maxx, src), row_bcast_i(bb.maxy, src)};
            const TileConic sco = {row_bcast_f(tc.cx, src), row_bcast_f(tc.cy, src), row_bcast_f(tc.cz, src), row_bcast_f(tc.rcpx, src),
                                   row_bcast_f(tc.rcpy, src)};
            uint32_t cnt = 0, m16 = 0u;
            row_tile_walk(lane, P.gx, true, act, sb, sco, row_bcast_f(cx, src), row_bcast_f(cy, src), row_bcast_f(pmax_tile, src),
                          [&](bool keep, uint32_t) { m16 = (uint32_t)((__ballot(keep) >> row_shift) & 0xFFFFull); cnt += (uint32_t)__popc(m16); });
            if (lane == src && act) { ntiles = cnt; walk_mask = m16; walk_kind = 1u; }
        }
        const bool halfc = area > 0 && !small && bbox_fits_half(bb);
        const int half_shift = lane & 32;
        const GroupPick halves = group_rank<32>(lane, halfc);
        for (int k = 0; k < halves.steps; ++k) {
// ... 296 lines not shown
}

constexpr uint32_t kGatherSmall = 32;

__device__ __forceinline__ float4 quat_contract(const float m[9], float4 q2) {
    const float r = q2.x, x = q2.y, y = q2.z, z = q2.w;
    const float m00 = m[0], m01 = m[1], m02 = m[2], m10 = m[3], m11 = m[4], m12 = m[5], m20 = m[6], m21 = m[7], m22 = m[8];
    const float s01 = m01 + m10, s02 = m02 + m20, s12 = m12 + m21;
    const float a01 = m01 - m10, a02 = m20 - m02, a12 = m12 - m21;
    float4 d;
    d.x = z * a01 + y * a02 + x * a12;
    d.y = y * s01 + z * s02 + r * a12 - 2.f * x * (m11 + m22);
    d.z = x * s01 + z * s12 + r * a02 - 2.f * y * (m00 + m22);
    d.w = x * s02 + y * s12 + r * a01 - 2.f * z * (m00 + m11);
    return d;
}

template <int STRIDE>
struct QuadAcc {
    float4 a;
    float4 x;
    __device__ __forceinline__ void clear() { a = make_float4(0.f, 0.f, 0.f, 0.f); x = a; }
    __device__ __forceinline__ void add_rows4(const float* __restrict__ partial, size_t sb, int b0, int b1, int b2, int b3, int c) {
        const float4 z = make_float4(0.f, 0.f, 0.f, 0.f);
        const float4* r0 = reinterpret_cast<const float4*>(partial + (sb + (size_t)b0) * STRIDE);
        const float4* r1 = reinterpret_cast<const float4*>(partial + (sb + (size_t)(b1 < 0 ? b0 : b1)) * STRIDE);
        const float4* r2 = reinterpret_cast<const float4*>(partial + (sb + (size_t)(b2 < 0 ? b0 : b2)) * STRIDE);
        const float4* r3 = reinterpret_cast<const float4*>(partial + (sb + (size_t)(b3 < 0 ? b0 : b3)) * STRIDE);
        const float4 v0 = r0[c], v1 = r1[c], v2 = r2[c], v3 = r3[c];
        float4 w0 = z, w1 = z, w2 = z, w3 = z;
        if (STRIDE > 16 && c == 0) { w0 = r0[4]; w1 = r1[4]; w2 = r2[4]; w3 = r3[4]; }
        a.x += v0.x; a.y += v0.y; a.z += v0.z; a.w += v0.w;
        if (b1 >= 0) { a.x += v1.x; a.y += v1.y; a.z += v1.z; a.w += v1.w; }
        if (b2 >= 0) { a.x += v2.x; a.y += v2.y; a.z += v2.z; a.w += v2.w; }
        if (b3 >= 0) { a.x += v3.x; a.y += v3.y; a.z += v3.z; a.w += v3.w; }
        if (STRIDE > 16 && c == 0) {
            x.x += w0.x; x.y += w0.y; x.z += w0.z; x.w += w0.w;
            if (b1 >= 0) { x.x += w1.x; x.y += w1.y; x.z += w1.z; x.w += w1.w; }
            if (b2 >= 0) { x.x += w2.x; x.y += w2.y; x.z += w2.z; x.w += w2.w; }
            if (b3 >= 0) { x.x += w3.x; x.y += w3.y; x.z += w3.z; x.w += w3.w; }
        }
    }
    __device__ __forceinline__ void add_row(const float* __restrict__ partial, size_t slot, int c) {
        const float4* row = reinterpret_cast<const float4*>(partial + slot * STRIDE);
        const float4 v = row[c];
        a.x += v.x; a.y += v.y; a.z += v.z; a.w += v.w;
        if (STRIDE > 16 && c == 0) {
            const float4 w = row[4];
            x.x += w.x; x.y += w.y; x.z += w.z; x.w += w.w;
        }
    }
};
template <int J>
__device__ __forceinline__ float quad_bcast(float v) {
    return __int_as_float(__builtin_amdgcn_update_dpp(0, __float_as_int(v), J | (J << 2) | (J << 4) | (J << 6), 0xf, 0xf, false));
}
template <int X>
__device__ __forceinline__ float quad_bcast_xor(float v) {
    constexpr int perm = X == 1 ? (1 | (0 << 2) | (3 << 4) | (2 << 6)) : (2 | (3 << 2) | (0 << 4) | (1 << 6));
    return __int_as_float(__builtin_amdgcn_update_dpp(0, __float_as_int(v), perm, 0xf, 0xf, false));
}
__device__ __forceinline__ float xor_sum_quads(float v) {
    v += __shfl_xor(v, 4, 64);
    v += __shfl_xor(v, 8, 64);
    v += __shfl_xor(v, 16, 64);
    v += __shfl_xor(v, 32, 64);
    return v;
}

__device__ __forceinline__ void store_split_sh_part(float* __restrict__ g_albedo, float* __restrict__ g_specular, size_t i, int c, const float (&o)[12]) {
    const bool first = c == 0;
    float* sp = g_specular + 45 * i + (first ? 0 : 12 * c - 3);
    Float4A4* w = reinterpret_cast<Float4A4*>(sp);
    w[0] = first ? Float4A4{o[3], o[4], o[5], o[6]} : Float4A4{o[0], o[1], o[2], o[3]};
    w[1] = first ? Float4A4{o[7], o[8], o[9], o[10]} : Float4A4{o[4], o[5], o[6], o[7]};
    if (first) {
        sp[8] = o[11];
        float* al = g_albedo + 3 * i;
        al[0] = o[0]; al[1] = o[1]; al[2] = o[2];
    } else {
        w[2] = Float4A4{o[8], o[9], o[10], o[11]};
    }
}
template <int STRIDE, bool NHT = false, bool FUSE_SH = false, bool SPLIT = false>
__global__ __launch_bounds__(256) void gut_grad_gather_kernel(GutParams P, GutProjected proj, const float4* __restrict__ density12,
                                                              GutGradSlots slots, int have_partials, GutGradOut g_out,
                                                              float* __restrict__ g_rgb, uint32_t first, uint32_t end,
                                                              const float* __restrict__ sph = nullptr, float* __restrict__ g_sph = nullptr,
                                                              const float* __restrict__ sph_specular = nullptr,
                                                              float* __restrict__ g_sph_specular = nullptr) {
    static_assert(!SPLIT || FUSE_SH, "split rows exist in the fused finalisation only");
    const int lane = threadIdx.x & 63, c = threadIdx.x & 3;
    const uint32_t i = first + blockIdx.x * 64u + (threadIdx.x >> 2);
    const uint32_t count = (i < end) ? proj.tiles_count[i] : 0u;
    const bool has = count != 0;
    QuadAcc<STRIDE> acc;
    acc.clear();
    const uint32_t off = (i < end) ? proj.part_offset[i] : 0u;
    const unsigned long long touched = (have_partials && i < end) ? slots.touched[i] : 0ull;
    float4 q = make_float4(1.f, 0.f, 0.f, 0.f), sc = make_float4(1.f, 1.f, 1.f, 0.f);
    if (has) { q = density12[3 * (size_t)i + 1]; sc = density12[3 * (size_t)i + 2]; }
    float4 sh0 = make_float4(0.f, 0.f, 0.f, 0.f), sh1 = sh0, sh2 = sh0, pa = sh0;
    f3 rad = mk3(0.f, 0.f, 0.f);
    if (FUSE_SH && has) {
        if (SPLIT) {
            const float* sp = sph_specular + 45 * (size_t)i + (c == 0 ? 0 : 12 * c - 3);
            const Float4A4 v0 = reinterpret_cast<const Float4A4*>(sp)[0], v1 = reinterpret_cast<const Float4A4*>(sp)[1];
            const Float4A4 v2 = *reinterpret_cast<const Float4A4*>(sp + (c == 0 ? 5 : 8));
            sh0 = make_float4(v0.x, v0.y, v0.z, v0.w);
            sh1 = make_float4(v1.x, v1.y, v1.z, v1.w);
            sh2 = make_float4(v2.x, v2.y, v2.z, v2.w);
            if (c == 0) {
                const float* al = sph + 3 * (size_t)i;
                sh0 = make_float4(al[0], al[1], al[2], v0.x);
                sh1 = make_float4(v0.y, v0.z, v0.w, v1.x);
                sh2 = make_float4(v1.y, v1.z, v1.w, v2.w);
            }
        } else {
            const float4* row = reinterpret_cast<const float4*>(sph + 48 * (size_t)i) + 3 * c;
            sh0 = row[0]; sh1 = row[1]; sh2 = row[2];
        }
        pa = density12[3 * (size_t)i];
        rad = mk3(proj.rgb[3 * (size_t)i], proj.rgb[3 * (size_t)i + 1], proj.rgb[3 * (size_t)i + 2]);
    }
    if (have_partials) {
        if (has && count <= kGatherSmall) {
            static_assert(2 * kGatherSmall <= kGutTouchBits, "the quad path reads its marks from the particle's word alone");
            const size_t sb = 2 * (size_t)off;
            const uint32_t nb = 2 * count;
            unsigned long long m = touched;
            if (nb < 64) m &= (1ull << nb) - 1ull;
            while (m) {
                const int b0 = __ffsll((long long)m) - 1;
                m &= m - 1;
                const int b1 = m ? __ffsll((long long)m) - 1 : -1;
                m &= m - 1;
                const int b2 = m ? __ffsll((long long)m) - 1 : -1;
                m &= m - 1;
                const int b3 = m ? __ffsll((long long)m) - 1 : -1;
                m &= m - 1;
                acc.add_rows4(slots.partial, sb, b0, b1, b2, b3, c);
            }
        }
        unsigned long long big = __ballot(has && count > kGatherSmall && c == 0);
        while (big) {
            const int src = __ffsll((long long)big) - 1;
            big &= big - 1;
            const size_t s0 = 2 * (size_t)(uint32_t)__builtin_amdgcn_readlane((int)off, src);
            const uint32_t n2 = 2u * (uint32_t)__builtin_amdgcn_readlane((int)count, src);
            QuadAcc<STRIDE> part;
            part.clear();
            const int g = lane >> 2;
            const unsigned long long m0 = (unsigned long long)(uint32_t)__builtin_amdgcn_readlane((int)(uint32_t)touched, src) |
                                          ((unsigned long long)(uint32_t)__builtin_amdgcn_readlane((int)(uint32_t)(touched >> 32), src) << 32);
#pragma nounroll
            for (uint32_t base = 0; base < n2; base += 64) {
                unsigned long long m = m0;
                if (base > 0) {
                    const bool set = (base + (uint32_t)lane < n2) && slots.flag[s0 + base + lane] != 0;
                    if (set) slots.flag[s0 + base + lane] = 0;
                    m = __ballot(set);
                }
                if (m == 0) continue;
                int b[4], nb = 0;
#pragma unroll
                for (int j = 0; j < 4; ++j)
                    if ((m >> (g + 16 * j)) & 1ull) b[nb++] = g + 16 * j;
                if (nb > 0)
                    part.add_rows4(slots.partial, s0 + base, b[0], nb > 1 ? b[1] : -1, nb > 2 ? b[2] : -1, nb > 3 ? b[3] : -1, c);
            }
            part.a.x = xor_sum_quads(part.a.x); part.a.y = xor_sum_quads(part.a.y);
            part.a.z = xor_sum_quads(part.a.z); part.a.w = xor_sum_quads(part.a.w);
            if (STRIDE > 16) {
                part.x.x = xor_sum_quads(part.x.x); part.x.y = xor_sum_quads(part.x.y);
                part.x.z = xor_sum_quads(part.x.z); part.x.w = xor_sum_quads(part.x.w);
            }
            if ((lane >> 2) == (src >> 2)) acc = part;
        }
        if (touched != 0ull && c == 0) slots.touched[i] = 0ull;
    }
    float r[20];
    r[0] = quad_bcast<0>(acc.a.x); r[1] = quad_bcast<0>(acc.a.y); r[2] = quad_bcast<0>(acc.a.z); r[3] = quad_bcast<0>(acc.a.w);
    r[4] = quad_bcast<1>(acc.a.x); r[5] = quad_bcast<1>(acc.a.y); r[6] = quad_bcast<1>(acc.a.z); r[7] = quad_bcast<1>(acc.a.w);
    r[8] = quad_bcast<2>(acc.a.x); r[9] = quad_bcast<2>(acc.a.y); r[10] = quad_bcast<2>(acc.a.z); r[11] = quad_bcast<2>(acc.a.w);
    r[12] = quad_bcast<3>(acc.a.x); r[13] = quad_bcast<3>(acc.a.y); r[14] = quad_bcast<3>(acc.a.z); r[15] = quad_bcast<3>(acc.a.w);
    r[16] = quad_bcast<0>(acc.x.x); r[17] = quad_bcast<0>(acc.x.y); r[18] = quad_bcast<0>(acc.x.z); r[19] = 0.f;
    if (i >= end) return;
    float4* gd = reinterpret_cast<float4*>(g_out.packed + 12 * (size_t)i);
    if (FUSE_SH && !has) {
        if (SPLIT) {
            const float zero[12] = {0.f, 0.f, 0.f, 0.f, 0.f, 0.f, 0.f, 0.f, 0.f, 0.f, 0.f, 0.f};
            store_split_sh_part(g_sph, g_sph_specular, (size_t)i, c, zero);
        } else {
            float4* out = reinterpret_cast<float4*>(g_sph + 48 * (size_t)i) + 3 * c;
            out[0] = out[1] = out[2] = make_float4(0.f, 0.f, 0.f, 0.f);
        }
    }
    if (!has) {
        if (g_out.packed) {
            if (c < 3) gd[c] = make_float4(0.f, 0.f, 0.f, 0.f);
        } else if (c == 0) {
            g_out.pos[3 * (size_t)i] = 0.f; g_out.pos[3 * (size_t)i + 1] = 0.f; g_out.pos[3 * (size_t)i + 2] = 0.f;
            g_out.dns[i] = 0.f;
        } else if (c == 1) {
            reinterpret_cast<float4*>(g_out.rot)[i] = make_float4(0.f, 0.f, 0.f, 0.f);
        } else if (c == 2) {
// ... 259 lines not shown
    } else {
        for (int row = 0; row < nrows; ++row)
            if (lane < rowlen) g_sph[(size_t)(wave_base + row) * rowlen + lane] = rows[row * kShStride + lane];
    }
}

__global__ __launch_bounds__(128) void sph_grad_from_views_kernel(uint32_t N, uint32_t n_views, const float* __restrict__ factors,
                                                                  const float* __restrict__ positions, uint32_t pos_stride, int n_active,
                                                                  int ncoef, float scale, float* __restrict__ g_sph) {
    __shared__ float s_rows[2][64 * kShStride];
    const int wave = threadIdx.x >> 6, lane = threadIdx.x & 63;
    const uint32_t wave_base = blockIdx.x * 128u + (uint32_t)wave * 64u;
    const uint32_t i = wave_base + lane;
    const int rowlen = 3 * ncoef;
    const int nact = min((n_active + 1) * (n_active + 1), ncoef);
    float* rows = s_rows[wave];
    float* myrow = rows + lane * kShStride;
    const int nrows = (int)min(64u, N > wave_base ? N - wave_base : 0u);
    if (i < N) {
        const f3 mu = mk3(positions[(size_t)i * pos_stride], positions[(size_t)i * pos_stride + 1], positions[(size_t)i * pos_stride + 2]);
        float acc[48];
#pragma unroll
        for (int k = 0; k < 48; ++k) acc[k] = 0.f;
        for (uint32_t v = 0; v < n_views; ++v) {
            const float* view = factors + (size_t)v * 3 * ((size_t)N + 1);
            const f3 g = mk3(view[3 * (size_t)i], view[3 * (size_t)i + 1], view[3 * (size_t)i + 2]);
            if (g.x == 0.f && g.y == 0.f && g.z == 0.f) continue;
            float ilen;
            const f3 dir = sh_view_direction(mu, mk3(view[3 * (size_t)N], view[3 * (size_t)N + 1], view[3 * (size_t)N + 2]), ilen);
            float basis[16];
            sh_basis_pinned(n_active, dir, basis);
#pragma unroll
            for (int k = 0; k < 16; ++k)
                if (k < nact) { acc[3 * k] = add_rn(acc[3 * k], mul_rn(basis[k], g.x)); acc[3 * k + 1] = add_rn(acc[3 * k + 1], mul_rn(basis[k], g.y)); acc[3 * k + 2] = add_rn(acc[3 * k + 2], mul_rn(basis[k], g.z)); }
        }
#pragma unroll
        for (int k = 0; k < 48; ++k)
            if (k < rowlen) myrow[k] = acc[k] * scale;
    }
    __syncthreads();
    if (rowlen == 48) {
        float4* dst = reinterpret_cast<float4*>(g_sph + (size_t)wave_base * 48);
        const int total4 = nrows * 12;
#pragma unroll
        for (int it = 0; it < 12; ++it) {
            const int q = lane + 64 * it;
            if (q < total4) {
                const float* d = rows + (q / 12) * kShStride + 4 * (q % 12);
                dst[q] = make_float4(d[0], d[1], d[2], d[3]);
            }
        }
    } else {
        for (int row = 0; row < nrows; ++row)
            if (lane < rowlen) g_sph[(size_t)(wave_base + row) * rowlen + lane] = rows[row * kShStride + lane];
    }
}

__global__ __launch_bounds__(256) void gut_prepare_tail_kernel(const uint32_t* __restrict__ last_offset, uint32_t* __restrict__ num_visible,
                                                               uint32_t* __restrict__ host_counters, uint32_t* __restrict__ ranges_words,
                                                               uint32_t n_ranges_words, uint32_t* __restrict__ reached_words, uint32_t n_reached_words) {
    const uint32_t i = blockIdx.x * blockDim.x + threadIdx.x, stride = gridDim.x * blockDim.x;
    if (blockIdx.x == 0 && threadIdx.x < 64) {
        uint32_t v = 0u;
        if (threadIdx.x < kGutCounterReplicas) { v = num_visible[threadIdx.x * kGutCounterStride]; num_visible[threadIdx.x * kGutCounterStride] = 0u; }
#pragma unroll
        for (int o = 32; o >= 1; o >>= 1) v += __shfl_xor(v, o, 64);
        if (threadIdx.x == 0) {
            __hip_atomic_store(&host_counters[0], *last_offset, __ATOMIC_RELAXED, __HIP_MEMORY_SCOPE_SYSTEM);
            __hip_atomic_store(&host_counters[1], v, __ATOMIC_RELAXED, __HIP_MEMORY_SCOPE_SYSTEM);
        }
    }
    for (uint32_t k = i; k < n_ranges_words; k += stride) ranges_words[k] = 0u;
    for (uint32_t k = i; k < n_reached_words; k += stride) reached_words[k] = 0u;
}

}

void launch_prepare_tail(hipStream_t s, const uint32_t* last_offset, uint32_t* num_visible, uint32_t* host_counters, uint32_t* ranges_words,
                         uint32_t n_ranges_words, uint32_t* reached_words, uint32_t n_reached_words) {
    hipLaunchKernelGGL(gut_prepare_tail_kernel, dim3(64), dim3(256), 0, s, last_offset, num_visible, host_counters, ranges_words, n_ranges_words,
                       reached_words, n_reached_words);
}

void launch_project(hipStream_t s, const GutParams& P, const float* density12, const float* sph, const GutSplitSph& split, const GutProjected& out,
                    int32_t* visibility, uint32_t* num_visible) {
#define GRUT_PROJECT_LAUNCH(M_, R_)                                                                                                                 \
    do {                                                                                                                                            \
        if (split.specular)                                                                                                                         \
            hipLaunchKernelGGL((gut_project_kernel<M_, R_, true>), dim3(div_up(P.N, 256)), dim3(256), 0, s, P,                                      \
                               reinterpret_cast<const float4*>(density12), split.albedo, out, visibility, num_visible, split.specular);           \
        else                                                                                                                                        \
            hipLaunchKernelGGL((gut_project_kernel<M_, R_, false>), dim3(div_up(P.N, 256)), dim3(256), 0, s, P,                                     \
                               reinterpret_cast<const float4*>(density12), sph, out, visibility, num_visible, static_cast<const float*>(nullptr)); \
    } while (0)
    const bool rolling = P.cam.shutter != GRUT_SHUTTER_GLOBAL;
    switch (P.cam.model) {
    case GRUT_CAMERA_OPENCV_PINHOLE: if (rolling) GRUT_PROJECT_LAUNCH(GRUT_CAMERA_OPENCV_PINHOLE, 1); else GRUT_PROJECT_LAUNCH(GRUT_CAMERA_OPENCV_PINHOLE, 0); break;
    case GRUT_CAMERA_OPENCV_FISHEYE: if (rolling) GRUT_PROJECT_LAUNCH(GRUT_CAMERA_OPENCV_FISHEYE, 1); else GRUT_PROJECT_LAUNCH(GRUT_CAMERA_OPENCV_FISHEYE, 0); break;
    case GRUT_CAMERA_FTHETA: if (rolling) GRUT_PROJECT_LAUNCH(GRUT_CAMERA_FTHETA, 1); else GRUT_PROJECT_LAUNCH(GRUT_CAMERA_FTHETA, 0); break;
    default: GRUT_PROJECT_LAUNCH(-1, 1); break;
    }
#undef GRUT_PROJECT_LAUNCH
}
void launch_expand(hipStream_t s, const GutParams& P, const GutProjected& proj, const uint32_t* rank_to_particle,
                   const uint32_t* offsets, uint32_t capacity, uint32_t* tile_keys, uint32_t* tile_vals, uint32_t* pos_particle) {
    hipLaunchKernelGGL(gut_expand_kernel, dim3(div_up(P.N, 256)), dim3(256), 0, s, P, proj, rank_to_particle, offsets, capacity,
                       tile_keys, tile_vals, pos_particle);
}
void launch_gather_particle_idx(hipStream_t s, uint32_t n, const uint32_t* sorted_pos, const uint32_t* pos_particle, uint32_t* out) {
    if (n) hipLaunchKernelGGL(gut_gather_particle_idx_kernel, dim3(div_up(n, 256)), dim3(256), 0, s, n, sorted_pos, pos_particle, out);
}
void launch_tile_ranges(hipStream_t s, uint32_t n, const uint32_t* n_dev, uint32_t tile_mask, uint32_t num_tiles,
                        const uint32_t* sorted_tile_keys, uint32_t* ranges, uint32_t* boundary_tile) {
    hipLaunchKernelGGL(gut_tile_ranges_kernel, dim3(div_up(div_up(n, 4u), 256)), dim3(256), 0, s, n, n_dev, tile_mask, num_tiles, sorted_tile_keys,
                       reinterpret_cast<uint2*>(ranges), boundary_tile);
}

void launch_project_bwd(hipStream_t s, const GutParams& P, const GutProjected& proj, const float* density12, const float* sph,
                        const GutSplitSph& split, const float* g_rgb, const GutGradOut& g_out, float* g_sph, const GutSplitSphGrad& g_split,
                        float* g_radiance, uint32_t first, uint32_t end) {
    if (end > P.N) end = P.N;
    if (end <= first) return;
    if (split.specular)
        hipLaunchKernelGGL((gut_project_bwd_kernel<false, true>), dim3(div_up(end - first, 128)), dim3(128), 0, s, P, proj.tiles_count,
                           reinterpret_cast<const float4*>(density12), split.albedo, proj.rgb, g_rgb, g_out, g_split.albedo, g_radiance, first, end,
                           split.specular, g_split.specular);
    else if (g_radiance)
        hipLaunchKernelGGL(gut_project_bwd_kernel<true>, dim3(div_up(end - first, 128)), dim3(128), 0, s, P, proj.tiles_count,
                           reinterpret_cast<const float4*>(density12), sph, proj.rgb, g_rgb, g_out, g_sph, g_radiance, first, end);
    else
        hipLaunchKernelGGL(gut_project_bwd_kernel<false>, dim3(div_up(end - first, 128)), dim3(128), 0, s, P, proj.tiles_count,
                           reinterpret_cast<const float4*>(density12), sph, proj.rgb, g_rgb, g_out, g_sph, g_radiance, first, end);
}
void launch_sph_grad_from_views(hipStream_t s, uint32_t N, uint32_t n_views, const float* factors, const float* positions, uint32_t pos_stride,
                                int n_active, int ncoef, float scale, float* g_sph) {
    hipLaunchKernelGGL(sph_grad_from_views_kernel, dim3(div_up(N, 128)), dim3(128), 0, s, N, n_views, factors, positions, pos_stride, n_active,
                       ncoef, scale, g_sph);
}
void launch_grad_finalize_nht(hipStream_t s, const GutParams& P, const GutProjected& proj, const float* density12, const GutGradSlots& slots,
                              bool have_partials, const GutGradOut& g_out) {
    hipLaunchKernelGGL((gut_grad_gather_kernel<16, true>), dim3(div_up(P.N, 64)), dim3(256), 0, s, P, proj, reinterpret_cast<const float4*>(density12),
                       slots, have_partials ? 1 : 0, g_out, static_cast<float*>(nullptr), 0u, P.N);
}
void launch_grad_finalize(hipStream_t s, const GutParams& P, const GutProjected& proj, const float* density12, const float* sph,
                          const GutSplitSph& split, const GutGradSlots& slots, bool has_gdist, bool have_partials, float* g_rgb,
                          const GutGradOut& g_out, float* g_sph, const GutSplitSphGrad& g_split, float* g_radiance, uint32_t first, uint32_t end) {
    if (end > P.N) end = P.N;
    if (end <= first) return;
    const dim3 grid(div_up(end - first, 64)), block(256);
    static const bool unfused = [] { const char* e = getenv("GRUT_GUT_UNFUSED_FINALIZE"); return e && e[0] == '1'; }();
    if (!unfused && split.specular) {
        if (has_gdist)
            hipLaunchKernelGGL((gut_grad_gather_kernel<20, false, true, true>), grid, block, 0, s, P, proj, reinterpret_cast<const float4*>(density12),
                               slots, have_partials ? 1 : 0, g_out, g_rgb, first, end, split.albedo, g_split.albedo, split.specular, g_split.specular);
        else
            hipLaunchKernelGGL((gut_grad_gather_kernel<16, false, true, true>), grid, block, 0, s, P, proj, reinterpret_cast<const float4*>(density12),
                               slots, have_partials ? 1 : 0, g_out, g_rgb, first, end, split.albedo, g_split.albedo, split.specular, g_split.specular);
        return;
    }
    if (!unfused && !g_radiance && g_sph && P.ncoef == 16 && !P.sph_half) {
        if (has_gdist)
            hipLaunchKernelGGL((gut_grad_gather_kernel<20, false, true>), grid, block, 0, s, P, proj, reinterpret_cast<const float4*>(density12), slots,
                               have_partials ? 1 : 0, g_out, g_rgb, first, end, sph, g_sph);
        else
            hipLaunchKernelGGL((gut_grad_gather_kernel<16, false, true>), grid, block, 0, s, P, proj, reinterpret_cast<const float4*>(density12), slots,
                               have_partials ? 1 : 0, g_out, g_rgb, first, end, sph, g_sph);
        return;
    }
    if (has_gdist)
        hipLaunchKernelGGL(gut_grad_gather_kernel<20>, grid, block, 0, s, P, proj, reinterpret_cast<const float4*>(density12), slots,
                           have_partials ? 1 : 0, g_out, g_rgb, first, end);
    else
        hipLaunchKernelGGL(gut_grad_gather_kernel<16>, grid, block, 0, s, P, proj, reinterpret_cast<const float4*>(density12), slots,
                           have_partials ? 1 : 0, g_out, g_rgb, first, end);
    launch_project_bwd(s, P, proj, density12, sph, split, g_rgb, g_out, g_sph, g_split, g_radiance, first, end);
}

}
```

3dgrut_amd/gut_tracer.py:

```python
from __future__ import annotations

import ctypes as C
import os

import torch

from . import _abi
from .camera import camera_from_batch

_FALSE_DEFAULTS = dict(
    particle_kernel_degree=2, particle_kernel_min_response=0.0113, particle_kernel_min_alpha=1.0 / 255.0,
    particle_kernel_max_alpha=0.99, min_transmittance=0.0001, particle_radiance_sph_degree=3,
    enable_hitcounts=True, enable_kernel_timings=False)
_SPLAT_DEFAULTS = dict(
    ut_alpha=1.0, ut_beta=2.0, ut_kappa=0.0, ut_in_image_margin_factor=0.1, ut_require_all_sigma_points_valid=False,
    n_rolling_shutter_iterations=5, k_buffer_size=0, global_z_order=True, rect_bounding=True,
    tight_opacity_bounding=True, tile_based_culling=True)


def _conf_get(node, name, default=None):
    if node is None:
        return default
    if isinstance(node, dict):
        return node.get(name, default)
# ... 5 lines not shown
            return node[name]
        except Exception:
            return default


def fused_activations_requested(conf) -> bool:
    return bool(_conf_get(_conf_get(conf, "render"), "fused_activations", False)) or bool(os.environ.get("GRUT_FUSED_ACTIVATIONS"))


def split_sh_requested(conf) -> bool:
    return bool(_conf_get(_conf_get(conf, "render"), "split_sh_features", False)) or bool(os.environ.get("GRUT_SPLIT_SH"))


def has_standard_activations(gaussians) -> bool:
    return (all(hasattr(gaussians, a) for a in ("density", "rotation", "scale", "density_activation", "scale_activation", "rotation_activation"))
            and gaussians.density_activation is torch.sigmoid and gaussians.scale_activation is torch.exp
            and gaussians.rotation_activation is torch.nn.functional.normalize)


def nht_config_from_conf(conf, cfg) -> bool:
    model = _conf_get(conf, "model")
    if str(_conf_get(model, "feature_type", "sh")).lower() != "nht":
        return False
    nf = _conf_get(model, "nht_features")
    act = _conf_get(nf, "activation")
    interp = str(_conf_get(nf, "interpolation_type", "none")).lower()
    if interp not in ("none", "barycentric"):
        raise NotImplementedError(f"3dgrut_amd: nht_features.interpolation_type={interp!r} (the reference supports none / barycentric)")
    points = 4 if interp == "barycentric" else 1
    dim = int(_conf_get(nf, "dim", 48))
    if dim % points:
        raise ValueError(f"nht_features.dim = {dim} is not divisible by the {points} interpolation points of interpolation_type={interp!r}")
    cfg.feature_transform_type = 1
    cfg.particle_feature_dim = dim
    cfg.interp_point_feature_dim = dim // points
    cfg.feature_interpolation_support = 1 if points == 4 else 0
    act_name = str(_conf_get(act, "type", "none") if act is not None else "none").lower()
    if act_name not in ("none", "siren", "sincos", "relu"):
        raise ValueError(f"Unknown nht_features.activation.type: {act_name}")
    cfg.feature_activation_type = {"none": 0, "siren": 1, "sincos": 2, "relu": 3}[act_name]
    cfg.feature_activation_num_frequencies = 1 if act_name in ("none", "relu") else int(_conf_get(act, "num_frequencies", 1))
    return True


def ray_feature_dim_of(cfg) -> int:
    if not cfg.feature_transform_type:
        return 3
    a, n = cfg.feature_activation_type, cfg.feature_activation_num_frequencies
    return cfg.interp_point_feature_dim * (2 * n if a == 2 else (n if a == 1 else 1))


def gut_config_from_conf(conf) -> _abi.GutConfig:
    render = _conf_get(conf, "render")
    splat = _conf_get(render, "splat")
    cfg = _abi.GutConfig()
    for k, d in _FALSE_DEFAULTS.items():
        v = _conf_get(render, k, d)
        setattr(cfg, k, type(d)(v) if not isinstance(d, bool) else int(bool(v)))
    for k, d in _SPLAT_DEFAULTS.items():
        v = _conf_get(splat, k, d)
        setattr(cfg, k, type(d)(v) if not isinstance(d, bool) else int(bool(v)))
    nht_config_from_conf(conf, cfg)
    cfg.particle_feature_half = int(bool(_conf_get(render, "particle_feature_half", False)))
    cfg.feature_output_half = int(bool(_conf_get(render, "feature_output_half", False)))
    if _conf_get(splat, "fine_grained_load_balancing", False):
        pass
    return cfg


def _ptr(t):
    return C.c_void_p(t.data_ptr()) if t is not None else None


def _stream_ptr(device):
    return C.c_void_p(torch.cuda.current_stream(device).cuda_stream)


def _uninitialised(shape, **opts):
    if os.environ.get("GRUT_POISON_OUTPUTS"):
        return torch.full(shape, float("nan") if opts.get("dtype") == torch.float32 else -1, **opts)
    return torch.empty(shape, **opts)


class _GutNative:

    def __init__(self, cfg: _abi.GutConfig):
        if not torch.cuda.is_available():
            raise RuntimeError("3dgrut_amd.Tracer needs a ROCm GPU (there is no CPU fallback)")
        torch.zeros(1, device="cuda")
        self.lib = _abi.load_library()
        self.cfg = cfg
        self.handle = C.c_void_p()
        _abi.check(self.lib.gut_create(C.byref(cfg), C.byref(self.handle)), "gut_create")
        self.ncoef = (cfg.particle_radiance_sph_degree + 1) ** 2
        self._timings = {}

    def __del__(self):
        try:
            if getattr(self, "handle", None) and self.handle.value:
                self.lib.gut_destroy(self.handle)
                self.handle = C.c_void_p()
        except Exception:
            pass

    def make_frame(self, frame_id, n_active, n, height, width, cam, pose_start, pose_end) -> _abi.GutFrame:
        f = _abi.GutFrame()
        f.frame_id, f.n_active_features, f.num_particles = int(frame_id) & 0xFFFFFFFF, int(n_active), int(n)
        f.width, f.height = int(width), int(height)
        f.camera = cam
        for i in range(7):
            f.pose_start[i] = float(pose_start[i])
            f.pose_end[i] = float(pose_end[i])
        return f

    def trace(self, frame, particle_density, particle_sph, ray_ori, ray_dir):
        return self._trace(frame, particle_density, (particle_sph,), ray_ori, ray_dir)

    def trace_split(self, frame, particle_density, sph_albedo, sph_specular, ray_ori, ray_dir):
        return self._trace(frame, particle_density, (sph_albedo, sph_specular), ray_ori, ray_dir)

    def _trace(self, frame, particle_density, sph, ray_ori, ray_dir):
        dev = ray_ori.device
        H, W = frame.height, frame.width
        N = frame.num_particles
        opts = dict(dtype=torch.float32, device=dev)
        half_out = bool(self.cfg.feature_output_half)
        fd_opts = dict(dtype=torch.float16 if half_out else torch.float32, device=dev)
        if N == 0:
            out_fd = torch.zeros((H, W, 4), **fd_opts)
            out_dist = torch.full((H, W, 1), 1e6, **opts)
            out_cnt = torch.zeros((H, W, 1), **opts)
            vis_i32 = torch.zeros((N, 1), dtype=torch.int32, device=dev)
        else:
            out_fd = _uninitialised((H, W, 4), **fd_opts)
            out_dist = _uninitialised((H, W, 1), **opts)
            out_cnt = _uninitialised((H, W, 1), **opts) if self.cfg.enable_hitcounts else torch.zeros((H, W, 1), **opts)
            vis_i32 = _uninitialised((N, 1), dtype=torch.int32, device=dev)
        if half_out:
            out_feat = out_opa = None
        elif N == 0:
            out_feat, out_opa = torch.zeros((H, W, 3), **opts), torch.zeros((H, W, 1), **opts)
        else:
            out_feat, out_opa = _uninitialised((H, W, 3), **opts), _uninitialised((H, W, 1), **opts)
        frame.out_features, frame.out_opacity = (None, None) if half_out else (out_feat.data_ptr(), out_opa.data_ptr())
        fn, name = (self.lib.gut_forward, "gut_forward") if len(sph) == 1 else (self.lib.gut_forward_split, "gut_forward_split")
        _abi.check(fn(self.handle, _stream_ptr(dev), C.byref(frame), _ptr(particle_density), *map(_ptr, sph),
                      _ptr(ray_ori), _ptr(ray_dir), _ptr(out_fd), _ptr(out_dist), _ptr(out_cnt), _ptr(vis_i32)), name)
        frame.out_features, frame.out_opacity = None, None
        if half_out:
            f32 = out_fd.float()
            out_feat, out_opa = f32[..., :3].contiguous(), f32[..., 3:].contiguous()
        return out_fd, out_dist, out_cnt, vis_i32.view(torch.float32), out_feat, out_opa

    @property
    def ray_feature_dim(self):
        return ray_feature_dim_of(self.cfg)

    def trace_nht(self, frame, particle_density, particle_features, ray_ori, ray_dir):
        dev = ray_ori.device
        H, W, N = frame.height, frame.width, frame.num_particles
        nr = self.ray_feature_dim
        fd = torch.zeros((H, W, nr + 1), dtype=torch.float16 if self.cfg.feature_output_half else torch.float32, device=dev)
        dist = torch.full((H, W, 1), 1e6, dtype=torch.float32, device=dev)
        cnt = torch.zeros((H, W, 1), dtype=torch.float32, device=dev)
        vis = torch.zeros((N, 1), dtype=torch.int32, device=dev)
        if self.cfg.particle_feature_half and particle_features.dtype != torch.float16:
            particle_features = particle_features.to(torch.float16)
        _abi.check(self.lib.gut_forward(self.handle, _stream_ptr(dev), C.byref(frame), _ptr(particle_density), _ptr(particle_features.contiguous()),
                                        _ptr(ray_ori), _ptr(ray_dir), _ptr(fd), _ptr(dist), _ptr(cnt), _ptr(vis)), "gut_forward")
        return fd, dist, cnt, vis.view(torch.float32), particle_features

    def trace_bwd_nht(self, frame, particle_density, particle_features, ray_ori, ray_dir, fd, g_fd, dist, g_dist):
        dev = ray_ori.device
        g_density = torch.empty_like(particle_density)
        g_feat = torch.empty(particle_features.shape, dtype=torch.float32, device=dev)
        _abi.check(self.lib.gut_backward(self.handle, _stream_ptr(dev), C.byref(frame), _ptr(particle_density), _ptr(particle_features),
                                         _ptr(ray_ori), _ptr(ray_dir), _ptr(fd), _ptr(g_fd), _ptr(dist), _ptr(g_dist),
                                         _ptr(g_density), _ptr(g_feat)), "gut_backward")
        return g_density, g_feat

    def trace_bwd(self, frame, particle_density, particle_sph, ray_ori, ray_dir, fd, g_fd, dist, g_dist):
        dev = ray_ori.device
        g_density = torch.empty_like(particle_density)
        g_sph = torch.empty_like(particle_sph, dtype=torch.float32)
        _abi.check(self.lib.gut_backward(self.handle, _stream_ptr(dev), C.byref(frame), _ptr(particle_density), _ptr(particle_sph),
                                         _ptr(ray_ori), _ptr(ray_dir), _ptr(fd), _ptr(g_fd), _ptr(dist), _ptr(g_dist),
                                         _ptr(g_density), _ptr(g_sph)), "gut_backward")
        return g_density, g_sph

    def trace_bwd_unpacked(self, frame, particle_density, particle_sph, ray_ori, ray_dir, fd, g_feat, g_opa, dist, g_dist):
        dev = ray_ori.device
        n = particle_density.shape[0]
        opts = dict(dtype=torch.float32, device=dev)
        g_pos, g_dns, g_rot, g_scl = torch.empty((n, 3), **opts), torch.empty((n, 1), **opts), torch.empty((n, 4), **opts), torch.empty((n, 3), **opts)
        g_sph = torch.empty_like(particle_sph, dtype=torch.float32)
        io = _abi.GutGradIO(_ptr(g_feat), _ptr(g_opa), _ptr(g_pos), _ptr(g_dns), _ptr(g_rot), _ptr(g_scl))
        _abi.check(self.lib.gut_backward_unpacked(self.handle, _stream_ptr(dev), C.byref(frame), _ptr(particle_density), _ptr(particle_sph),
                                                  _ptr(ray_ori), _ptr(ray_dir), _ptr(fd), _ptr(dist), _ptr(g_dist), C.byref(io), _ptr(g_sph)),
                   "gut_backward_unpacked")
        return g_pos, g_dns, g_rot, g_scl, g_sph

    def trace_bwd_split(self, frame, particle_density, sph_albedo, sph_specular, ray_ori, ray_dir, fd, g_fd, dist, g_dist):
        g_density, g_albedo, g_specular = torch.empty_like(particle_density), torch.empty_like(sph_albedo), torch.empty_like(sph_specular)
        _abi.check(self.lib.gut_backward_split(self.handle, _stream_ptr(ray_ori.device), C.byref(frame), _ptr(particle_density), _ptr(sph_albedo),
                                               _ptr(sph_specular), _ptr(ray_ori), _ptr(ray_dir), _ptr(fd), _ptr(g_fd), _ptr(dist), _ptr(g_dist),
                                               _ptr(g_density), _ptr(g_albedo), _ptr(g_specular)), "gut_backward_split")
        return g_density, g_albedo, g_specular

    def trace_bwd_unpacked_split(self, frame, particle_density, sph_albedo, sph_specular, ray_ori, ray_dir, fd, g_feat, g_opa, dist, g_dist):
        n = particle_density.shape[0]
        opts = dict(dtype=torch.float32, device=ray_ori.device)
        g_pos, g_dns, g_rot, g_scl = torch.empty((n, 3), **opts), torch.empty((n, 1), **opts), torch.empty((n, 4), **opts), torch.empty((n, 3), **opts)
        g_albedo, g_specular = torch.empty_like(sph_albedo), torch.empty_like(sph_specular)
        io = _abi.GutGradIO(_ptr(g_feat), _ptr(g_opa), _ptr(g_pos), _ptr(g_dns), _ptr(g_rot), _ptr(g_scl))
        _abi.check(self.lib.gut_backward_unpacked_split(self.handle, _stream_ptr(ray_ori.device), C.byref(frame), _ptr(particle_density),
                                                        _ptr(sph_albedo), _ptr(sph_specular), _ptr(ray_ori), _ptr(ray_dir), _ptr(fd), _ptr(dist),
                                                        _ptr(g_dist), C.byref(io), _ptr(g_albedo), _ptr(g_specular)), "gut_backward_unpacked_split")
        return g_pos, g_dns, g_rot, g_scl, g_albedo, g_specular

    def trace_bwd_factored(self, frame, particle_density, particle_sph, ray_ori, ray_dir, fd, g_fd, dist, g_dist):
        dev = ray_ori.device
        g_density = torch.empty_like(particle_density)
        g_radiance = torch.empty((particle_density.shape[0] + 1, 3), dtype=torch.float32, device=dev)
        _abi.check(self.lib.gut_backward_factored(self.handle, _stream_ptr(dev), C.byref(frame), _ptr(particle_density), _ptr(particle_sph),
                                                  _ptr(ray_ori), _ptr(ray_dir), _ptr(fd), _ptr(g_fd), _ptr(dist), _ptr(g_dist),
                                                  _ptr(g_density), _ptr(g_radiance)), "gut_backward_factored")
        return g_density, g_radiance

    def trace_bwd_factored_chunked(self, frame, particle_density, particle_sph, ray_ori, ray_dir, fd, g_fd, dist, g_dist, num_chunks, on_chunk):
        dev = ray_ori.device
        g_density = torch.empty_like(particle_density)
        g_radiance = torch.empty((particle_density.shape[0] + 1, 3), dtype=torch.float32, device=dev)
        errors = []

        def _cb(_user, chunk, first, count):
            try:
                on_chunk(int(chunk), int(first), int(count), g_density, g_radiance)
            except BaseException as e:
                errors.append(e)
        cb = _abi.CHUNK_FN(_cb)
        rc = self.lib.gut_backward_factored_chunked(self.handle, _stream_ptr(dev), C.byref(frame), _ptr(particle_density), _ptr(particle_sph),
                                                    _ptr(ray_ori), _ptr(ray_dir), _ptr(fd), _ptr(g_fd), _ptr(dist), _ptr(g_dist),
                                                    _ptr(g_density), _ptr(g_radiance), int(num_chunks), cb, None)
        if errors:
            raise errors[0]
        _abi.check(rc, "gut_backward_factored_chunked")
        return g_density, g_radiance

    def collect_times(self):
        if not self.cfg.enable_kernel_timings:
            return {}
        f, b = C.c_float(-1), C.c_float(-1)
        _abi.check(self.lib.gut_timings(self.handle, C.byref(f), C.byref(b)), "gut_timings")
        if f.value >= 0:
            self._timings["forward_render"] = f.value
        if b.value >= 0:
            self._timings["backward_render"] = b.value
        return dict(self._timings)

    def trim(self):
        _abi.check(self.lib.gut_trim(self.handle), "gut_trim")

    def stats(self) -> _abi.GutStats:
        s = _abi.GutStats()
        _abi.check(self.lib.gut_stats(self.handle, C.byref(s)), "gut_stats")
        return s


class _NhtAutograd(torch.autograd.Function):

    @staticmethod
    def forward(ctx, native, frame, ray_ori, ray_dir, mog_pos, mog_rot, mog_scl, mog_dns, mog_feat, exchange=None):
        particle_density = _abi.pack_particles(mog_pos, mog_dns, mog_rot, mog_scl)
        fd, dist, cnt, vis, feats_k = native.trace_nht(frame, particle_density, mog_feat.contiguous(), ray_ori, ray_dir)
        ctx.save_for_backward(ray_ori, ray_dir, fd, dist, particle_density, feats_k)
        ctx.native, ctx.frame, ctx.exchange = native, frame, exchange
        nr = native.ray_feature_dim
        f32 = fd.float()
        ctx.mark_non_differentiable(cnt, vis)
        ctx.set_materialize_grads(False)
        return f32[..., :nr].unsqueeze(0).contiguous(), f32[..., nr:].unsqueeze(0).contiguous(), dist, cnt, vis

    @staticmethod
    def backward(ctx, g_feat, g_opa, g_dist, _g_cnt, _g_vis):
        ray_ori, ray_dir, fd, dist, particle_density, feats_k = ctx.saved_tensors
        H, W, nr = fd.shape[0], fd.shape[1], fd.shape[2] - 1
        c = ctx.native.cfg
        if (ctx.exchange is None and c.particle_feature_dim == 48 and c.interp_point_feature_dim == 12 and c.feature_interpolation_support == 1
                and c.feature_activation_type == 2 and c.feature_activation_num_frequencies == 1 and int(c.k_buffer_size) == 0
                and not os.environ.get("GRUT_NHT_GENERIC")):
            g_pos, g_dns, g_rot, g_scl, g_features = ctx.native.trace_bwd_unpacked(
                ctx.frame, particle_density, feats_k, ray_ori, ray_dir, fd,
                None if g_feat is None else g_feat.reshape(H, W, nr).float().contiguous(), None if g_opa is None else g_opa.reshape(H, W, 1).float().contiguous(),
                dist, None if g_dist is None else g_dist.contiguous())
            return None, None, None, None, g_pos, g_rot, g_scl, g_dns, g_features, None
        g_feat = fd.new_zeros((H, W, nr), dtype=torch.float32) if g_feat is None else g_feat.reshape(H, W, nr).float()
        g_opa = fd.new_zeros((H, W, 1), dtype=torch.float32) if g_opa is None else g_opa.reshape(H, W, 1).float()
        g_fd = torch.cat([g_feat, g_opa], dim=-1).contiguous()
        g_density, g_features = ctx.native.trace_bwd_nht(ctx.frame, particle_density, feats_k, ray_ori, ray_dir, fd, g_fd, dist,
                                                         None if g_dist is None else g_dist.contiguous())
        if ctx.exchange is not None:
            g_density, g_features = ctx.exchange.reduce_dense(g_density, g_features)
        g_pos, g_dns, g_rot, g_scl = _abi.unpack_particle_grads(g_density)
        return None, None, None, None, g_pos, g_rot, g_scl, g_dns, g_features, None


class Tracer:
    class _Autograd(torch.autograd.Function):
        @staticmethod
        def forward(ctx, native, frame, ray_ori, ray_dir, mog_pos, mog_rot, mog_scl, mog_dns, mog_sph, raw=False, exchange=None):
            if raw:
                particle_density = _abi.activate_pack(mog_pos, mog_dns, mog_rot, mog_scl)
            else:
                particle_density = _abi.pack_particles(mog_pos, mog_dns, mog_rot, mog_scl)
            ctx.raw = (mog_dns, mog_rot, mog_scl) if raw else None
            particle_features = mog_sph.contiguous()
            if native.cfg.particle_feature_half and particle_features.dtype != torch.float16:
                particle_features = particle_features.to(torch.float16)
            fd, dist, cnt, vis, feat, opa = native.trace(frame, particle_density, particle_features, ray_ori, ray_dir)
            ctx.save_for_backward(ray_ori, ray_dir, fd, dist, particle_density, particle_features)
            ctx.native, ctx.frame, ctx.exchange = native, frame, exchange
            feat = feat.unsqueeze(0)
            opa = opa.unsqueeze(0)
            ctx.mark_non_differentiable(cnt, vis)
            ctx.set_materialize_grads(False)
            return feat, opa, dist, cnt, vis

        @staticmethod
        def backward(ctx, g_feat, g_opa, g_dist, _g_cnt, _g_vis):
            ray_ori, ray_dir, fd, dist, particle_density, particle_features = ctx.saved_tensors
            H, W = fd.shape[0], fd.shape[1]
            g_dist = None if g_dist is None else g_dist.contiguous()
            if ctx.exchange is None and ctx.raw is None and int(ctx.native.cfg.k_buffer_size) == 0:
                g_pos, g_dns, g_rot, g_scl, g_sph = ctx.native.trace_bwd_unpacked(
                    ctx.frame, particle_density, particle_features, ray_ori, ray_dir, fd,
                    None if g_feat is None else g_feat.reshape(H, W, 3).contiguous(), None if g_opa is None else g_opa.reshape(H, W, 1).contiguous(),
                    dist, g_dist)
                return None, None, None, None, g_pos, g_rot, g_scl, g_dns, g_sph, None, None
            g_feat = fd.new_zeros((H, W, 3)) if g_feat is None else g_feat.reshape(H, W, 3)
            g_opa = fd.new_zeros((H, W, 1)) if g_opa is None else g_opa.reshape(H, W, 1)
            g_fd = torch.cat([g_feat, g_opa], dim=-1)
            if ctx.exchange is None:
                g_density, g_sph = ctx.native.trace_bwd(ctx.frame, particle_density, particle_features, ray_ori, ray_dir, fd, g_fd, dist, g_dist)
            else:
                if getattr(ctx.exchange, "chunks", 1) > 1 and int(ctx.native.cfg.k_buffer_size) == 0:
                    g_density, g_sph = ctx.exchange.reduce_packed_pipelined(
                        lambda n, cb: ctx.native.trace_bwd_factored_chunked(ctx.frame, particle_density, particle_features, ray_ori, ray_dir, fd, g_fd,
                                                                            dist, g_dist, n, cb),
                        particle_density, int(ctx.frame.n_active_features), int(ctx.native.cfg.particle_radiance_sph_degree))
                else:
                    g_density, g_radiance = ctx.native.trace_bwd_factored(ctx.frame, particle_density, particle_features, ray_ori, ray_dir,
                                                                          fd, g_fd, dist, g_dist)
                    g_density, g_sph = ctx.exchange.reduce_packed(g_density, g_radiance, particle_density, int(ctx.frame.n_active_features),
                                                                  int(ctx.native.cfg.particle_radiance_sph_degree))
            if ctx.raw is not None:
                g_pos, g_dns, g_rot, g_scl = _abi.activate_pack_backward(*ctx.raw, g_density)
                return None, None, None, None, g_pos, g_rot, g_scl, g_dns, g_sph, None, None
            g_pos, g_dns, g_rot, g_scl = _abi.unpack_particle_grads(g_density)
            return None, None, None, None, g_pos, g_rot, g_scl, g_dns, g_sph, None, None

    class _AutogradSplit(torch.autograd.Function):

        @staticmethod
        def forward(ctx, native, frame, ray_ori, ray_dir, mog_pos, mog_rot, mog_scl, mog_dns, sph_albedo, sph_specular, raw=False):
            if raw:
                particle_density = _abi.activate_pack(mog_pos, mog_dns, mog_rot, mog_scl)
            else:
                particle_density = _abi.pack_particles(mog_pos, mog_dns, mog_rot, mog_scl)
            ctx.raw = (mog_dns, mog_rot, mog_scl) if raw else None
            fd, dist, cnt, vis, feat, opa = native.trace_split(frame, particle_density, sph_albedo, sph_specular, ray_ori, ray_dir)
            ctx.save_for_backward(ray_ori, ray_dir, fd, dist, particle_density, sph_albedo, sph_specular)
            ctx.native, ctx.frame = native, frame
            feat = feat.unsqueeze(0)
            opa = opa.unsqueeze(0)
            ctx.mark_non_differentiable(cnt, vis)
            ctx.set_materialize_grads(False)
            return feat, opa, dist, cnt, vis

        @staticmethod
        def backward(ctx, g_feat, g_opa, g_dist, _g_cnt, _g_vis):
            ray_ori, ray_dir, fd, dist, particle_density, sph_albedo, sph_specular = ctx.saved_tensors
            H, W = fd.shape[0], fd.shape[1]
            g_dist = None if g_dist is None else g_dist.contiguous()
            if ctx.raw is None:
                g_pos, g_dns, g_rot, g_scl, g_albedo, g_specular = ctx.native.trace_bwd_unpacked_split(
                    ctx.frame, particle_density, sph_albedo, sph_specular, ray_ori, ray_dir, fd,
                    None if g_feat is None else g_feat.reshape(H, W, 3).contiguous(), None if g_opa is None else g_opa.reshape(H, W, 1).contiguous(),
                    dist, g_dist)
                return None, None, None, None, g_pos, g_rot, g_scl, g_dns, g_albedo, g_specular, None
            g_feat = fd.new_zeros((H, W, 3)) if g_feat is None else g_feat.reshape(H, W, 3)
            g_opa = fd.new_zeros((H, W, 1)) if g_opa is None else g_opa.reshape(H, W, 1)
            g_fd = torch.cat([g_feat, g_opa], dim=-1)
            g_density, g_albedo, g_specular = ctx.native.trace_bwd_split(ctx.frame, particle_density, sph_albedo, sph_specular, ray_ori, ray_dir,
                                                                         fd, g_fd, dist, g_dist)
            g_pos, g_dns, g_rot, g_scl = _abi.activate_pack_backward(*ctx.raw, g_density)
            return None, None, None, None, g_pos, g_rot, g_scl, g_dns, g_albedo, g_specular, None

    def __init__(self, conf):
        self.device = "cuda"
        self.conf = conf
        self.tracer_wrapper = _GutNative(gut_config_from_conf(conf))
        self._fused_activations = fused_activations_requested(conf)
        self._split_sh = split_sh_requested(conf)
        self.stats_split = {"split_calls": 0, "cat_calls": 0}
        self.gradient_exchange = None

    @property
    def timings(self):
        return self.tracer_wrapper.collect_times()

    def build_acc(self, gaussians, rebuild=True):
        pass

    def _constant_normals(self, like):
        key = (tuple(like.shape), like.device, like.dtype)
        if getattr(self, "_normals_key", None) != key:
            self._normals = torch.nn.functional.normalize(torch.ones_like(like), dim=3)
            self._normals_key = key
        return self._normals

    def _split_sh_tensors(self, gaussians, device):
        c = self.tracer_wrapper.cfg
        if (not self._split_sh or self.gradient_exchange is not None or c.feature_transform_type or c.particle_feature_half
                or int(c.particle_radiance_sph_degree) != 3 or int(c.k_buffer_size) != 0):
            return None
        n = int(gaussians.num_gaussians)
        albedo, specular = getattr(gaussians, "features_albedo", None), getattr(gaussians, "features_specular", None)
        for t, cols in ((albedo, 3), (specular, 45)):
            if (n == 0 or not torch.is_tensor(t) or t.dtype != torch.float32 or t.device != device or tuple(t.shape) != (n, cols)
                    or not t.is_contiguous() or t.data_ptr() % 16):
                return None
        return albedo, specular

    def render(self, gaussians, gpu_batch, train=False, frame_id=0):
        rays_o = gpu_batch.rays_ori if not isinstance(gpu_batch, dict) else gpu_batch["rays_ori"]
        rays_d = gpu_batch.rays_dir if not isinstance(gpu_batch, dict) else gpu_batch["rays_dir"]
        T0 = gpu_batch["T_to_world"] if isinstance(gpu_batch, dict) else gpu_batch.T_to_world
        T1 = (gpu_batch.get("T_to_world_end") if isinstance(gpu_batch, dict) else getattr(gpu_batch, "T_to_world_end", None))
        in_world = bool(gpu_batch.get("rays_in_world_space", False) if isinstance(gpu_batch, dict) else getattr(gpu_batch, "rays_in_world_space", False))
        dev_poses = torch.is_tensor(T0) and T0.is_cuda and not in_world and (T1 is None or (torch.is_tensor(T1) and T1.is_cuda))
        cam, pose_start, pose_end = camera_from_batch(gpu_batch, poses_on_device=dev_poses)
        H, W = int(rays_o.shape[1]), int(rays_o.shape[2])
        native = self.tracer_wrapper
        frame = native.make_frame(frame_id, gaussians.n_active_features, gaussians.num_gaussians, H, W, cam, pose_start, pose_end)
        if dev_poses:
            t0 = T0.detach().reshape(-1, 4, 4)[0].to(torch.float32).contiguous()
            t1 = None if T1 is None else T1.detach().reshape(-1, 4, 4)[0].to(torch.float32).contiguous()
            frame.device_T_to_world = t0.data_ptr()
            frame.device_T_to_world_end = None if t1 is None else t1.data_ptr()
            frame._keepalive = (t0, t1)
        split = self._split_sh_tensors(gaussians, rays_o.device)
        if split is not None:
            if getattr(gaussians, "ray_feature_dim", 3) != 3:
                raise NotImplementedError("3dgrut_amd: only SH radiance features (ray_feature_dim = 3) are supported")
            self.stats_split["split_calls"] += 1
            raw = self._fused_activations and has_standard_activations(gaussians)
            pred_features, pred_opacity, pred_dist, hits_count, mog_visibility = Tracer._AutogradSplit.apply(
                native, frame, rays_o.contiguous().float(), rays_d.contiguous().float(), gaussians.positions.contiguous(),
                (gaussians.rotation if raw else gaussians.get_rotation()).contiguous(), (gaussians.scale if raw else gaussians.get_scale()).contiguous(),
                (gaussians.density if raw else gaussians.get_density()).contiguous(), split[0], split[1], raw)
            timings = native.collect_times()
            return {"pred_features": pred_features, "pred_opacity": pred_opacity, "pred_dist": pred_dist.unsqueeze(0),
                    "pred_normals": self._constant_normals(pred_features), "hits_count": hits_count.unsqueeze(0),
                    "frame_time_ms": timings["forward_render"] if "forward_render" in timings else 0.0, "mog_visibility": mog_visibility}
        self.stats_split["cat_calls"] += 1
        feats = gaussians.get_features()
# ... 37 lines not shown
```

include/grut_amd.h:

```cpp
#ifndef GRUT_AMD_H
#define GRUT_AMD_H

#include <stddef.h>
#include <stdint.h>

#ifdef __cplusplus
extern "C" {
#endif

typedef enum GrutStatus {
    GRUT_OK              = 0,
    GRUT_ERR_BAD_INPUT   = -1,
    GRUT_ERR_RUNTIME     = -2,
    GRUT_ERR_NOT_READY   = -3,
    GRUT_ERR_UNSUPPORTED = -4
} GrutStatus;

enum { GRUT_SHUTTER_ROLLING_TOP_TO_BOTTOM = 0,
       GRUT_SHUTTER_ROLLING_LEFT_TO_RIGHT = 1,
       GRUT_SHUTTER_ROLLING_BOTTOM_TO_TOP = 2,
       GRUT_SHUTTER_ROLLING_RIGHT_TO_LEFT = 3,
       GRUT_SHUTTER_GLOBAL                = 4 };

enum { GRUT_CAMERA_OPENCV_PINHOLE = 0,
// ... 40 lines not shown
    int32_t particle_feature_half;
    int32_t feature_output_half;
    int32_t feature_transform_type;
    int32_t particle_feature_dim;
    int32_t interp_point_feature_dim;
    int32_t feature_interpolation_support;
    int32_t feature_activation_type;
    int32_t feature_activation_num_frequencies;
} GutConfig;

typedef struct GutFrame {
    uint32_t   frame_id;
    int32_t    n_active_features;
    uint32_t   num_particles;
    int32_t    width, height;
    GrutCamera camera;
    float      pose_start[7];
    float      pose_end[7];
    const float* device_T_to_world;
    const float* device_T_to_world_end;
    float* out_features;
    float* out_opacity;
} GutFrame;

typedef struct GutStats {
    uint32_t num_particles;
    uint32_t num_visible;
    uint64_t num_intersections;
    uint32_t num_tiles;
    uint32_t key_bits;
    uint64_t fwd_entries_evaluated, fwd_entries_accepted;
    uint64_t bwd_entries_evaluated, bwd_entries_accepted;
} GutStats;

typedef struct GutHandle GutHandle;

int  gut_create(const GutConfig* config, GutHandle** handle);
void gut_destroy(GutHandle* handle);
int  gut_trim(GutHandle* handle);

int gut_forward(GutHandle* handle, void* stream, const GutFrame* frame,
                const float* particle_density, const void* particle_sph,
                const float* ray_origin, const float* ray_direction,
                void* out_feat_density, float* out_hit_distance,
                float* out_hit_count, int32_t* out_visibility);

int gut_backward(GutHandle* handle, void* stream, const GutFrame* frame,
                 const float* particle_density, const void* particle_sph,
                 const float* ray_origin, const float* ray_direction,
                 const void* feat_density, const float* grad_feat_density,
                 const float* hit_distance, const float* grad_hit_distance,
                 float* grad_particle_density, float* grad_particle_sph);

typedef struct GutGradIO {
    const float* grad_features;
    const float* grad_opacity;
    float* grad_positions;
    float* grad_density;
    float* grad_rotation;
    float* grad_scale;
} GutGradIO;
int gut_backward_unpacked(GutHandle* handle, void* stream, const GutFrame* frame,
                          const float* particle_density, const void* particle_sph,
                          const float* ray_origin, const float* ray_direction,
                          const void* feat_density, const float* hit_distance, const float* grad_hit_distance,
                          const GutGradIO* io, float* grad_particle_sph);

int gut_forward_split(GutHandle* handle, void* stream, const GutFrame* frame,
                      const float* particle_density, const float* sph_albedo, const float* sph_specular,
                      const float* ray_origin, const float* ray_direction,
                      void* out_feat_density, float* out_hit_distance,
                      float* out_hit_count, int32_t* out_visibility);
int gut_backward_split(GutHandle* handle, void* stream, const GutFrame* frame,
                       const float* particle_density, const float* sph_albedo, const float* sph_specular,
                       const float* ray_origin, const float* ray_direction,
                       const void* feat_density, const float* grad_feat_density,
                       const float* hit_distance, const float* grad_hit_distance,
                       float* grad_particle_density, float* grad_sph_albedo, float* grad_sph_specular);
int gut_backward_unpacked_split(GutHandle* handle, void* stream, const GutFrame* frame,
                                const float* particle_density, const float* sph_albedo, const float* sph_specular,
                                const float* ray_origin, const float* ray_direction,
                                const void* feat_density, const float* hit_distance, const float* grad_hit_distance,
                                const GutGradIO* io, float* grad_sph_albedo, float* grad_sph_specular);

int gut_backward_factored(GutHandle* handle, void* stream, const GutFrame* frame,
                          const float* particle_density, const void* particle_sph,
                          const float* ray_origin, const float* ray_direction,
                          const void* feat_density, const float* grad_feat_density,
                          const float* hit_distance, const float* grad_hit_distance,
                          float* grad_particle_density, float* grad_radiance);

typedef void (*GrutChunkFn)(void* user, uint32_t chunk, uint32_t first_particle, uint32_t num_particles);
int gut_backward_factored_chunked(GutHandle* handle, void* stream, const GutFrame* frame,
                                  const float* particle_density, const void* particle_sph,
                                  const float* ray_origin, const float* ray_direction,
                                  const void* feat_density, const float* grad_feat_density,
                                  const float* hit_distance, const float* grad_hit_distance,
                                  float* grad_particle_density, float* grad_radiance,
                                  uint32_t num_chunks, GrutChunkFn on_chunk, void* user);
int grut_sph_grad_from_views(void* stream, uint32_t num_particles, uint32_t num_views, const float* view_factors,
                             const float* positions, uint32_t position_stride, int32_t n_active_features, int32_t sph_degree,
                             float scale, float* grad_particle_sph);

int gut_timings(GutHandle* handle, float* forward_ms, float* backward_ms);
int gut_stats(GutHandle* handle, GutStats* stats);

enum { GUT_STAGE_PROJECT = 0, GUT_STAGE_DEPTH_SORT, GUT_STAGE_SCAN, GUT_STAGE_EXPAND, GUT_STAGE_TILE_SORT,
       GUT_STAGE_TILE_RANGES, GUT_STAGE_RENDER_FWD, GUT_STAGE_RENDER_BWD, GUT_STAGE_PROJECT_BWD, GUT_NUM_STAGES };
int gut_profile_enable(GutHandle* handle, int enable);
int gut_profile_select(GutHandle* handle, uint32_t stage_mask);
int gut_profile_read(GutHandle* handle, float* stage_ms );

int grut_sort_pairs_u32(void* stream, uint32_t n, int begin_bit, int end_bit,
                        uint32_t* keys, uint32_t* values,
                        uint32_t* keys_tmp, uint32_t* values_tmp,
                        void* scratch, uint64_t scratch_bytes,
                        uint32_t** sorted_keys, uint32_t** sorted_values);
uint64_t grut_sort_scratch_bytes(uint32_t n);
int grut_inclusive_scan_u32(void* stream, uint32_t n, const uint32_t* in, uint32_t* out,
                            void* scratch, uint64_t scratch_bytes);
uint64_t grut_scan_scratch_bytes(uint32_t n);
int grut_debug_sort_pairs_u32(void* stream, uint32_t n, const uint32_t* n_dev, int begin_bit, int end_bit,
                              uint32_t* keys, uint32_t* values, uint32_t* keys_tmp, uint32_t* values_tmp, int values_iota,
                              void* scratch, uint64_t scratch_bytes, uint32_t** sorted_keys, uint32_t** sorted_values);
int grut_debug_scan_gather_u32(void* stream, uint32_t n, const uint32_t* in, const uint32_t* gather, uint32_t* out,
                               void* scratch, uint64_t scratch_bytes);
int gut_debug_tile_ranges(void* stream, uint32_t n, const uint32_t* n_dev, uint32_t tile_mask, uint32_t num_tiles,
                          const uint32_t* sorted_tile_keys, uint32_t* ranges, uint32_t* boundary_tile, uint32_t* segment);

int gut_debug_fetch_work(GutHandle* handle, void* stream, unsigned long long* out, uint64_t count);
int grut_debug_pose_from_c2w(const float* c2w16, float* out7);
int grut_debug_frame_poses(void* stream, int on_device, const float* T_start, const float* T_end, float* host_out47);
int gut_debug_fetch(GutHandle* handle, void* stream,
                    uint32_t* tiles_count, float* proj_pos, float* conic_opacity, float* extent,
                    float* depth, float* rgb, uint32_t* sorted_particle_idx, uint32_t* tile_ranges);

typedef struct GrtConfig {
    int32_t particle_kernel_degree;
    float   particle_kernel_min_response;
    float   particle_kernel_min_alpha;
    float   particle_kernel_max_alpha;
    int32_t particle_kernel_density_clamping;
    int32_t particle_radiance_sph_degree;
    int32_t enable_normals;
    int32_t enable_hitcounts;
    int32_t enable_kernel_timings;
    int32_t max_hits_per_trace;
    int32_t particle_feature_half;
    int32_t feature_output_half;
    int32_t feature_transform_type;
    int32_t particle_feature_dim;
    int32_t interp_point_feature_dim;
    int32_t feature_interpolation_support;
    int32_t feature_activation_type;
    int32_t feature_activation_num_frequencies;
    int32_t primitive_type;
    int32_t pipeline_type;
} GrtConfig;
enum { GRUT_PIPELINE_REFERENCE = 0, GRUT_PIPELINE_BARYCENTRIC_SURFELS = 1, GRUT_PIPELINE_REFERENCE_SLANG = 2 };
enum { GRUT_PRIM_INSTANCES = 0, GRUT_PRIM_ICOSAHEDRON = 1, GRUT_PRIM_OCTAHEDRON = 2, GRUT_PRIM_TETRAHEDRON = 3, GRUT_PRIM_DIAMOND = 4, GRUT_PRIM_CUSTOM = 5,
       GRUT_PRIM_TRISURFEL = 6,
       GRUT_PRIM_TRIHEXA = 7,
       GRUT_PRIM_SPHERE = 8 };

typedef struct GrtFrame {
    uint32_t frame_id;
// ... 263 lines not shown
```

Before: 1.081 billion rays/s.

## Read particle attributes directly from separate tensors, skipping the pack kernel

Adds tensor-based forward/backward entry points that take separate position, density, rotation and scale tensors. When the configuration allows, the project and gradient-finalize kernels read these rows in place, so the per-iteration pack into a packed [N,12] buffer is skipped. Otherwise the pack runs into a cached internal buffer. The autograd path uses the new entry points by default for fp32, non-raw, no-exchange training. This removes one full pass over the particle data plus its allocation, but the kernels now gather from several separate arrays, which may coalesce less well.

```diff
diff --git a/3dgrut_amd/_abi.py b/3dgrut_amd/_abi.py
--- a/3dgrut_amd/_abi.py
+++ b/3dgrut_amd/_abi.py
@@ -132,6 +132,11 @@
     _fields_ = [("grad_features", C.c_void_p), ("grad_opacity", C.c_void_p), ("grad_positions", C.c_void_p), ("grad_density", C.c_void_p),
                 ("grad_rotation", C.c_void_p), ("grad_scale", C.c_void_p)]
 
+
+class GutParticleTensors(C.Structure):
+    _fields_ = [("positions", C.c_void_p), ("density", C.c_void_p), ("rotation", C.c_void_p), ("scale", C.c_void_p)]
+
+
 MLP_ACT_NONE, MLP_ACT_RELU, MLP_ACT_SIGMOID = range(3)
 PPISP_CONTROLLER_SAVED = 1984
 
@@ -158,7 +163,8 @@
 
 
 EXPORTED_SYMBOLS = [
-    "gut_create", "gut_destroy", "gut_forward", "gut_backward", "gut_backward_unpacked", "gut_forward_split", "gut_backward_split", "gut_backward_unpacked_split", "gut_backward_factored", "gut_backward_factored_chunked", "grut_sph_grad_from_views", "gut_timings", "gut_stats",
+    "gut_create", "gut_destroy", "gut_forward", "gut_backward", "gut_backward_unpacked", "gut_forward_split", "gut_backward_split", "gut_backward_unpacked_split",
+    "gut_forward_tensors", "gut_backward_unpacked_tensors", "gut_forward_split_tensors", "gut_backward_unpacked_split_tensors", "gut_backward_factored", "gut_backward_factored_chunked", "grut_sph_grad_from_views", "gut_timings", "gut_stats",
     "gut_profile_enable", "gut_profile_select", "gut_profile_read",
     "gut_debug_fetch", "gut_debug_fetch_work", "grut_debug_pose_from_c2w", "grut_debug_frame_poses", "grut_sort_pairs_u32", "grut_sort_scratch_bytes", "grut_inclusive_scan_u32",
     "grut_scan_scratch_bytes", "grut_debug_sort_pairs_u32", "grut_debug_scan_gather_u32", "gut_debug_tile_ranges", "grt_debug_list_ranges",
@@ -209,6 +215,15 @@
     lib.gut_backward_split.restype = C.c_int
     lib.gut_backward_unpacked_split.argtypes = [C.c_void_p, vp, C.POINTER(GutFrame)] + [fp] * 8 + [C.POINTER(GutGradIO), fp, fp]
     lib.gut_backward_unpacked_split.restype = C.c_int
+    pt = C.POINTER(GutParticleTensors)
+    lib.gut_forward_tensors.argtypes = [C.c_void_p, vp, C.POINTER(GutFrame), pt, fp, fp, fp, fp, fp, fp, ip]
+    lib.gut_forward_tensors.restype = C.c_int
+    lib.gut_backward_unpacked_tensors.argtypes = [C.c_void_p, vp, C.POINTER(GutFrame), pt] + [fp] * 6 + [C.POINTER(GutGradIO), fp]
+    lib.gut_backward_unpacked_tensors.restype = C.c_int
+    lib.gut_forward_split_tensors.argtypes = [C.c_void_p, vp, C.POINTER(GutFrame), pt, fp, fp, fp, fp, fp, fp, fp, ip]
+    lib.gut_forward_split_tensors.restype = C.c_int
+    lib.gut_backward_unpacked_split_tensors.argtypes = [C.c_void_p, vp, C.POINTER(GutFrame), pt] + [fp] * 7 + [C.POINTER(GutGradIO), fp, fp]
+    lib.gut_backward_unpacked_split_tensors.restype = C.c_int
     lib.grut_sph_grad_from_views.argtypes = [vp, C.c_uint32, C.c_uint32, fp, fp, C.c_uint32, C.c_int32, C.c_int32, C.c_float, fp]
     lib.grut_sph_grad_from_views.restype = C.c_int
     lib.gut_timings.argtypes = [C.c_void_p, C.POINTER(C.c_float), C.POINTER(C.c_float)]
diff --git a/3dgrut_amd/csrc/gut_api.hip b/3dgrut_amd/csrc/gut_api.hip
--- a/3dgrut_amd/csrc/gut_api.hip
+++ b/3dgrut_amd/csrc/gut_api.hip
@@ -32,6 +32,7 @@
     int device = -1;
     DeviceBuffer tiles_count, proj_pos, conic_opacity, extent, depth, rgb, depth_key, particle_idx;
     DeviceBuffer depth_key_tmp, particle_idx_tmp, offsets, sort_scratch, scan_scratch, counters;
+    DeviceBuffer packed;
     DeviceBuffer rec64;
     DeviceBuffer part_offset, pos_particle, grad_partial, grad_flag, grad_touched, g_rgb, poses_dev, walk8;
     bool flags_dirty = false;
@@ -43,6 +44,8 @@
     bool have_forward = false;
     hipStream_t fwd_stream = nullptr;
     const void* fwd_density = nullptr;
+    bool fwd_tensors = false;
+    const float* fwd_rows = nullptr;
     const void* fwd_ray_o = nullptr;
     const void* fwd_ray_d = nullptr;
     uint32_t fwd_frame_id = 0;
@@ -257,7 +260,7 @@
 static void release_scratch(GutHandle* h) {
     DeviceBuffer* bufs[] = {&h->tiles_count, &h->proj_pos, &h->conic_opacity, &h->extent, &h->depth, &h->rgb, &h->depth_key,
                             &h->particle_idx, &h->depth_key_tmp, &h->particle_idx_tmp, &h->offsets, &h->sort_scratch,
-                            &h->scan_scratch, &h->counters, &h->rec64, &h->walk8, &h->part_offset, &h->pos_particle, &h->grad_partial, &h->grad_flag,
+                            &h->scan_scratch, &h->counters, &h->packed, &h->rec64, &h->walk8, &h->part_offset, &h->pos_particle, &h->grad_partial, &h->grad_flag,
                             &h->grad_touched,
                             &h->g_rgb, &h->poses_dev, &h->work_counters, &h->tile_keys, &h->tile_vals, &h->tile_keys_tmp,
                             &h->tile_vals_tmp, &h->tile_sort_scratch, &h->ranges, &h->ck_tc, &h->ck_d, &h->ck_nht, &h->ck_reached,
@@ -300,7 +303,7 @@
 
 static int forward_impl(GutHandle* h, void* stream_, const GutFrame* frame, const float* particle_density, const void* particle_sph_,
                         const GutSplitSph& split, const float* ray_origin, const float* ray_direction, void* out_feat_density_,
-                        float* out_hit_distance, float* out_hit_count, int32_t* out_visibility) {
+                        float* out_hit_distance, float* out_hit_count, int32_t* out_visibility, const GutParticleTensors* tensors = nullptr) {
     const float* particle_sph = reinterpret_cast<const float*>(particle_sph_);
     float* out_feat_density = reinterpret_cast<float*>(out_feat_density_);
     GRUT_REQUIRE(h && frame, "gut_forward: null handle/frame");
@@ -320,7 +323,9 @@
     h->stats.key_bits = bits_for(tiles);
     h->num_intersections = 0;
     h->fwd_stream = s;
-    h->fwd_density = particle_density;
+    h->fwd_density = tensors ? tensors->positions : particle_density;
+    h->fwd_tensors = tensors != nullptr;
+    h->fwd_rows = nullptr;
     h->fwd_ray_o = ray_origin;
     h->fwd_ray_d = ray_direction;
     h->fwd_frame_id = frame->frame_id;
@@ -328,7 +333,7 @@
         h->have_forward = true;
         return GRUT_OK;
     }
-    GRUT_REQUIRE(particle_density && (particle_sph || split.specular) && out_visibility, "gut_forward: null particle buffer");
+    GRUT_REQUIRE((particle_density || tensors) && (particle_sph || split.specular) && out_visibility, "gut_forward: null particle buffer");
     GRUT_REQUIRE(!h->cfg.feature_output_half || (!frame->out_features && !frame->out_opacity), "gut_forward: feature_output_half excludes out_features / out_opacity");
     GRUT_REQUIRE(!h->cfg.feature_transform_type || (!frame->out_features && !frame->out_opacity), "gut_forward: neural harmonic features exclude out_features / out_opacity");
     if (h->cfg.enable_kernel_timings) GRUT_CHECK(h->fwd_timer.begin(s));
@@ -339,6 +344,17 @@
     h->params.rec64 = direct ? h->rec64.as<float4>() : nullptr;
     h->params.ord_shift = h->stats.key_bits;
     h->params.sorted_keys = nullptr;
+    GutTensorRows rows;
+    if (tensors) {
+        if (gut_rows_in_place(h->params, split.specular != nullptr)) {
+            rows = GutTensorRows{tensors->positions, tensors->density, reinterpret_cast<const float4*>(tensors->rotation), tensors->scale};
+        } else {
+            GRUT_CHECK(h->packed.ensure((size_t)N * 48, 1.25f));
+            GRUT_CHECK(grut_pack_particles(s, N, tensors->positions, tensors->density, tensors->rotation, tensors->scale, h->packed.as<float>()));
+            particle_density = h->packed.as<float>();
+        }
+        h->fwd_rows = particle_density;
+    }
     if (frame->device_T_to_world) {
         GRUT_CHECK(h->poses_dev.ensure(sizeof(FramePoses)));
         launch_frame_poses(s, frame->device_T_to_world, frame->device_T_to_world_end, h->poses_dev.as<FramePoses>());
@@ -362,7 +378,7 @@
         h->prof_slot++;
     }
     GRUT_CHECK(h->stage_begin(GUT_STAGE_PROJECT, s, slot));
-    launch_project(s, P, particle_density, particle_sph, split, proj, out_visibility, d_counters + 1);
+    launch_project(s, P, particle_density, rows, particle_sph, split, proj, out_visibility, d_counters + 1);
     GRUT_CHECK(h->stage_end(GUT_STAGE_PROJECT, s, slot));
     GRUT_CHECK(h->stage_begin(GUT_STAGE_DEPTH_SORT, s, slot));
     uint32_t *sorted_depth = nullptr, *rank_to_particle = nullptr;
@@ -502,7 +518,8 @@
                          const float* ray_origin, const float* ray_direction, const void* feat_density_, const float* grad_feat_density,
                          const float* hit_distance, const float* grad_hit_distance, float* grad_particle_density, float* grad_particle_sph,
                          float* grad_radiance, const GutGradIO* io = nullptr, uint32_t num_chunks = 1, GrutChunkFn on_chunk = nullptr,
-                         void* chunk_user = nullptr, const GutSplitSph& split = {}, const GutSplitSphGrad& g_split = {}) {
+                         void* chunk_user = nullptr, const GutSplitSph& split = {}, const GutSplitSphGrad& g_split = {},
+                         const GutParticleTensors* tensors = nullptr) {
     const float* particle_sph = reinterpret_cast<const float*>(particle_sph_);
     const float* feat_density = reinterpret_cast<const float*>(feat_density_);
     GRUT_REQUIRE(h && frame, "gut_backward: null handle/frame");
@@ -514,12 +531,16 @@
     }
     const GutParams& P = h->params;
     GRUT_REQUIRE(frame->num_particles == P.N && frame->width == P.W && frame->height == P.H, "gut_backward: frame differs from the forward frame");
-    if (frame->frame_id != h->fwd_frame_id || (P.N > 0 && (particle_density != h->fwd_density || ray_origin != h->fwd_ray_o || ray_direction != h->fwd_ray_d))) {
+    const void* token = tensors ? tensors->positions : particle_density;
+    if (frame->frame_id != h->fwd_frame_id || (tensors != nullptr) != h->fwd_tensors ||
+        (P.N > 0 && (token != h->fwd_density || ray_origin != h->fwd_ray_o || ray_direction != h->fwd_ray_d))) {
         set_last_error("gut_backward: the forward context belongs to another forward (a later gut_forward ran on this handle before this "
                        "backward); run each backward before the next forward, or use one handle per in-flight frame");
         return GRUT_ERR_NOT_READY;
     }
     if (P.N == 0) return GRUT_OK;
+    const bool rows_in_records = tensors && !h->fwd_rows;
+    if (tensors) particle_density = h->fwd_rows;
     if (P.nht) {
         if (grad_radiance) {
             set_last_error("gut_backward_factored: neural harmonic features have no per-view factorisation; reduce the dense gradients");
@@ -585,7 +606,7 @@
             return GRUT_ERR_UNSUPPORTED;
         }
     }
-    GRUT_REQUIRE(particle_density && (particle_sph || split.specular) && feat_density && (io || grad_feat_density) && hit_distance &&
+    GRUT_REQUIRE((particle_density || rows_in_records) && (particle_sph || split.specular) && feat_density && (io || grad_feat_density) && hit_distance &&
                      (io || grad_particle_density) && (grad_particle_sph || grad_radiance || g_split.specular), "gut_backward: null buffer");
     if (h->cfg.enable_kernel_timings) GRUT_CHECK(h->bwd_timer.begin(s));
     const GutProjected proj = projected_view(h);
@@ -628,7 +649,7 @@
     GRUT_CHECK(h->g_rgb.ensure((size_t)P.N * 12, 1.25f));
     if (num_chunks <= 1 || !on_chunk) {
         launch_grad_finalize(s, P, proj, particle_density, particle_sph, split, slots, has_gdist, I > 0, h->g_rgb.as<float>(), g_out,
-                             grad_particle_sph, g_split, grad_radiance);
+                             grad_particle_sph, g_split, grad_radiance, 0u, 0xFFFFFFFFu, rows_in_records);
     } else {
         const uint32_t per = ((P.N + num_chunks - 1) / num_chunks + 127u) & ~127u;
         uint32_t c = 0;
@@ -680,6 +701,66 @@
     return backward_impl(h, stream, frame, particle_density, nullptr, ray_origin, ray_direction, feat_density, nullptr, hit_distance,
                          grad_hit_distance, nullptr, nullptr, nullptr, io, 1, nullptr, nullptr, GutSplitSph{sph_albedo, sph_specular},
                          GutSplitSphGrad{grad_sph_albedo, grad_sph_specular});
+}
+
+}
+
+static int tensor_preconditions(const GutHandle* h, const char* who, const GutFrame* frame, const GutParticleTensors* t) {
+    GRUT_REQUIRE(h && frame, "%s: null handle/frame", who);
+    const GutConfig& cfg = h->cfg;
+    const char* why = cfg.feature_transform_type ? "neural harmonic features run on the packed [N,12] rows"
+                      : cfg.particle_feature_half ? "particle_feature_half (the fused gradient finalisation reads fp32 coefficients)"
+                      : cfg.k_buffer_size != 0 ? "k_buffer_size > 0 (the sorted mode runs on the packed [N,12] rows)" : nullptr;
+    if (why) {
+        set_last_error("%s: unsupported configuration: %s", who, why);
+        return GRUT_ERR_UNSUPPORTED;
+    }
+    GRUT_REQUIRE(t, "%s: null GutParticleTensors", who);
+    if (frame->num_particles == 0) return GRUT_OK;
+    GRUT_REQUIRE(t->positions && t->density && t->rotation && t->scale, "%s: null positions / density / rotation / scale tensor", who);
+    GRUT_REQUIRE((reinterpret_cast<uintptr_t>(t->rotation) & 15u) == 0, "%s: the rotation tensor must be 16-byte aligned", who);
+    GRUT_REQUIRE(frame->num_particles <= 0x55555555u, "%s: too many particles", who);
+    return GRUT_OK;
+}
+
+extern "C" {
+
+int gut_forward_tensors(GutHandle* h, void* stream, const GutFrame* frame, const GutParticleTensors* particles, const void* particle_sph,
+                        const float* ray_origin, const float* ray_direction, void* out_feat_density, float* out_hit_distance,
+                        float* out_hit_count, int32_t* out_visibility) {
+    GRUT_CHECK(tensor_preconditions(h, "gut_forward_tensors", frame, particles));
+    return forward_impl(h, stream, frame, nullptr, particle_sph, GutSplitSph{}, ray_origin, ray_direction, out_feat_density, out_hit_distance,
+                        out_hit_count, out_visibility, particles);
+}
+
+int gut_backward_unpacked_tensors(GutHandle* h, void* stream, const GutFrame* frame, const GutParticleTensors* particles,
+                                  const void* particle_sph, const float* ray_origin, const float* ray_direction, const void* feat_density,
+                                  const float* hit_distance, const float* grad_hit_distance, const GutGradIO* io, float* grad_particle_sph) {
+    GRUT_CHECK(tensor_preconditions(h, "gut_backward_unpacked_tensors", frame, particles));
+    GRUT_REQUIRE(io, "gut_backward_unpacked_tensors: null GutGradIO");
+    return backward_impl(h, stream, frame, nullptr, particle_sph, ray_origin, ray_direction, feat_density, nullptr, hit_distance, grad_hit_distance,
+                         nullptr, grad_particle_sph, nullptr, io, 1, nullptr, nullptr, GutSplitSph{}, GutSplitSphGrad{}, particles);
+}
+
+int gut_forward_split_tensors(GutHandle* h, void* stream, const GutFrame* frame, const GutParticleTensors* particles, const float* sph_albedo,
+                              const float* sph_specular, const float* ray_origin, const float* ray_direction, void* out_feat_density,
+                              float* out_hit_distance, float* out_hit_count, int32_t* out_visibility) {
+    GRUT_CHECK(split_preconditions(h, "gut_forward_split_tensors", {sph_albedo, sph_specular}));
+    GRUT_CHECK(tensor_preconditions(h, "gut_forward_split_tensors", frame, particles));
+    return forward_impl(h, stream, frame, nullptr, nullptr, GutSplitSph{sph_albedo, sph_specular}, ray_origin, ray_direction, out_feat_density,
+                        out_hit_distance, out_hit_count, out_visibility, particles);
+}
+
+int gut_backward_unpacked_split_tensors(GutHandle* h, void* stream, const GutFrame* frame, const GutParticleTensors* particles,
+                                        const float* sph_albedo, const float* sph_specular, const float* ray_origin, const float* ray_direction,
+                                        const void* feat_density, const float* hit_distance, const float* grad_hit_distance, const GutGradIO* io,
+                                        float* grad_sph_albedo, float* grad_sph_specular) {
+    GRUT_CHECK(split_preconditions(h, "gut_backward_unpacked_split_tensors", {sph_albedo, sph_specular, grad_sph_albedo, grad_sph_specular}));
+    GRUT_CHECK(tensor_preconditions(h, "gut_backward_unpacked_split_tensors", frame, particles));
+    GRUT_REQUIRE(io, "gut_backward_unpacked_split_tensors: null GutGradIO");
+    return backward_impl(h, stream, frame, nullptr, nullptr, ray_origin, ray_direction, feat_density, nullptr, hit_distance, grad_hit_distance,
+                         nullptr, nullptr, nullptr, io, 1, nullptr, nullptr, GutSplitSph{sph_albedo, sph_specular},
+                         GutSplitSphGrad{grad_sph_albedo, grad_sph_specular}, particles);
 }
 
 int gut_backward_factored(GutHandle* h, void* stream, const GutFrame* frame, const float* particle_density, const void* particle_sph,
diff --git a/3dgrut_amd/csrc/gut_internal.hpp b/3dgrut_amd/csrc/gut_internal.hpp
--- a/3dgrut_amd/csrc/gut_internal.hpp
+++ b/3dgrut_amd/csrc/gut_internal.hpp
@@ -77,6 +77,16 @@
     float* albedo = nullptr;
     float* specular = nullptr;
 };
+struct GutTensorRows {
+    const float* pos = nullptr;
+    const float* dns = nullptr;
+    const float4* rot = nullptr;
+    const float* scl = nullptr;
+};
+bool gut_finalize_unfused();
+inline bool gut_rows_in_place(const GutParams& P, bool split) {
+    return P.rec64 && !P.nht && P.k_buffer == 0 && !P.sph_half && (split || P.ncoef == 16) && !gut_finalize_unfused();
+}
 #ifdef __HIPCC__
 __device__ __forceinline__ float4 load_grad_in(const GutGradIn& g, size_t pix) {
     if (g.fd) return reinterpret_cast<const float4*>(g.fd)[pix];
@@ -101,8 +111,8 @@
 };
 
 constexpr uint32_t kGutCounterReplicas = 64, kGutCounterStride = 32, kGutCounterWords = kGutCounterReplicas * kGutCounterStride + 32;
-void launch_project(hipStream_t s, const GutParams& P, const float* density12, const float* sph, const GutSplitSph& split, const GutProjected& out,
-                    int32_t* visibility, uint32_t* num_visible);
+void launch_project(hipStream_t s, const GutParams& P, const float* density12, const GutTensorRows& rows, const float* sph, const GutSplitSph& split,
+                    const GutProjected& out, int32_t* visibility, uint32_t* num_visible);
 void launch_expand(hipStream_t s, const GutParams& P, const GutProjected& proj, const uint32_t* rank_to_particle,
                    const uint32_t* offsets, uint32_t capacity, uint32_t* tile_keys, uint32_t* tile_vals, uint32_t* pos_particle);
 void launch_gather_particle_idx(hipStream_t s, uint32_t n, const uint32_t* sorted_pos, const uint32_t* pos_particle, uint32_t* out);
@@ -144,7 +154,7 @@
 void launch_grad_finalize(hipStream_t s, const GutParams& P, const GutProjected& proj, const float* density12, const float* sph,
                           const GutSplitSph& split, const GutGradSlots& slots, bool has_gdist, bool have_partials, float* g_rgb,
                           const GutGradOut& g_out, float* g_sph, const GutSplitSphGrad& g_split, float* g_radiance, uint32_t first = 0u,
-                          uint32_t end = 0xFFFFFFFFu);
+                          uint32_t end = 0xFFFFFFFFu, bool rows_in_records = false);
 void launch_sph_grad_from_views(hipStream_t s, uint32_t N, uint32_t n_views, const float* factors, const float* positions, uint32_t pos_stride,
                                 int n_active, int ncoef, float scale, float* g_sph);
 
diff --git a/3dgrut_amd/csrc/gut_kernels.hip b/3dgrut_amd/csrc/gut_kernels.hip
--- a/3dgrut_amd/csrc/gut_kernels.hip
+++ b/3dgrut_amd/csrc/gut_kernels.hip
@@ -255,11 +255,13 @@
     float x, y, z, w;
 };
 
-template <int MODEL, int ROLLING, bool SPLIT = false>
+template <bool TENSORS> struct ProjectRows { using type = const float4* __restrict__; };
+template <> struct ProjectRows<true> { using type = GutTensorRows; };
+template <int MODEL, int ROLLING, bool SPLIT = false, bool TENSORS = false>
 #ifndef GRUT_PROJECT_WAVES_MAX
 #define GRUT_PROJECT_WAVES_MAX 6
 #endif
-__global__ __launch_bounds__(256) __attribute__((amdgpu_waves_per_eu(6, GRUT_PROJECT_WAVES_MAX))) void gut_project_kernel(GutParams P, const float4* __restrict__ density12,
+__global__ __launch_bounds__(256) __attribute__((amdgpu_waves_per_eu(6, GRUT_PROJECT_WAVES_MAX))) void gut_project_kernel(GutParams P, typename ProjectRows<TENSORS>::type density12,
                                                           const float* __restrict__ sph, GutProjected out,
                                                           int32_t* __restrict__ visibility, uint32_t* __restrict__ num_visible,
                                                           const float* __restrict__ sph_specular) {
@@ -275,9 +277,16 @@
     f3 pos = mk3(0.f, 0.f, 0.f);
     float4 a = make_float4(0.f, 0.f, 0.f, 0.f), b = a, c = a;
     if (i < P.N) {
-        a = density12[3 * (size_t)i + 0];
-        b = density12[3 * (size_t)i + 1];
-        c = density12[3 * (size_t)i + 2];
+        if constexpr (TENSORS) {
+            const GutTensorRows& t = density12;
+            a = make_float4(t.pos[3 * (size_t)i], t.pos[3 * (size_t)i + 1], t.pos[3 * (size_t)i + 2], t.dns[i]);
+            b = t.rot[i];
+            c = make_float4(t.scl[3 * (size_t)i], t.scl[3 * (size_t)i + 1], t.scl[3 * (size_t)i + 2], 0.f);
+        } else {
+            a = density12[3 * (size_t)i + 0];
+            b = density12[3 * (size_t)i + 1];
+            c = density12[3 * (size_t)i + 2];
+        }
         pos = mk3(a.x, a.y, a.z);
         const float opacity = a.w;
 
@@ -740,7 +749,7 @@
         w[2] = Float4A4{o[8], o[9], o[10], o[11]};
     }
 }
-template <int STRIDE, bool NHT = false, bool FUSE_SH = false, bool SPLIT = false>
+template <int STRIDE, bool NHT = false, bool FUSE_SH = false, bool SPLIT = false, bool REC = false>
 __global__ __launch_bounds__(256) void gut_grad_gather_kernel(GutParams P, GutProjected proj, const float4* __restrict__ density12,
                                                               GutGradSlots slots, int have_partials, GutGradOut g_out,
                                                               float* __restrict__ g_rgb, uint32_t first, uint32_t end,
@@ -748,6 +757,7 @@
                                                               const float* __restrict__ sph_specular = nullptr,
                                                               float* __restrict__ g_sph_specular = nullptr) {
     static_assert(!SPLIT || FUSE_SH, "split rows exist in the fused finalisation only");
+    static_assert(!REC || FUSE_SH, "frames without packed rows run the fused finalisation only");
     const int lane = threadIdx.x & 63, c = threadIdx.x & 3;
     const uint32_t i = first + blockIdx.x * 64u + (threadIdx.x >> 2);
     const uint32_t count = (i < end) ? proj.tiles_count[i] : 0u;
@@ -757,7 +767,11 @@
     const uint32_t off = (i < end) ? proj.part_offset[i] : 0u;
     const unsigned long long touched = (have_partials && i < end) ? slots.touched[i] : 0ull;
     float4 q = make_float4(1.f, 0.f, 0.f, 0.f), sc = make_float4(1.f, 1.f, 1.f, 0.f);
-    if (has) { q = density12[3 * (size_t)i + 1]; sc = density12[3 * (size_t)i + 2]; }
+    const float4* rec = proj.rec64 + 4 * (size_t)i;
+    if (has) {
+        if (REC) { q = rec[1]; sc = rec[2]; }
+        else { q = density12[3 * (size_t)i + 1]; sc = density12[3 * (size_t)i + 2]; }
+    }
     float4 sh0 = make_float4(0.f, 0.f, 0.f, 0.f), sh1 = sh0, sh2 = sh0, pa = sh0;
     f3 rad = mk3(0.f, 0.f, 0.f);
     if (FUSE_SH && has) {
@@ -778,8 +792,14 @@
             const float4* row = reinterpret_cast<const float4*>(sph + 48 * (size_t)i) + 3 * c;
             sh0 = row[0]; sh1 = row[1]; sh2 = row[2];
         }
-        pa = density12[3 * (size_t)i];
-        rad = mk3(proj.rgb[3 * (size_t)i], proj.rgb[3 * (size_t)i + 1], proj.rgb[3 * (size_t)i + 2]);
+        if (REC) {
+            pa = rec[0];
+            const float4 c3 = rec[3];
+            rad = mk3(c3.x, c3.y, c3.z);
+        } else {
+            pa = density12[3 * (size_t)i];
+            rad = mk3(proj.rgb[3 * (size_t)i], proj.rgb[3 * (size_t)i + 1], proj.rgb[3 * (size_t)i + 2]);
+        }
     }
     if (have_partials) {
         if (has && count <= kGatherSmall) {
@@ -1205,11 +1225,17 @@
                        reached_words, n_reached_words);
 }
 
-void launch_project(hipStream_t s, const GutParams& P, const float* density12, const float* sph, const GutSplitSph& split, const GutProjected& out,
-                    int32_t* visibility, uint32_t* num_visible) {
+void launch_project(hipStream_t s, const GutParams& P, const float* density12, const GutTensorRows& rows, const float* sph, const GutSplitSph& split,
+                    const GutProjected& out, int32_t* visibility, uint32_t* num_visible) {
 #define GRUT_PROJECT_LAUNCH(M_, R_)                                                                                                                 \
     do {                                                                                                                                            \
-        if (split.specular)                                                                                                                         \
+        if (rows.rot && split.specular)                                                                                                             \
+            hipLaunchKernelGGL((gut_project_kernel<M_, R_, true, true>), dim3(div_up(P.N, 256)), dim3(256), 0, s, P, rows, split.albedo, out,       \
+                               visibility, num_visible, split.specular);                                                                            \
+        else if (rows.rot)                                                                                                                          \
+            hipLaunchKernelGGL((gut_project_kernel<M_, R_, false, true>), dim3(div_up(P.N, 256)), dim3(256), 0, s, P, rows, sph, out, visibility,   \
+                               num_visible, static_cast<const float*>(nullptr));                                                                    \
+        else if (split.specular)                                                                                                                    \
             hipLaunchKernelGGL((gut_project_kernel<M_, R_, true>), dim3(div_up(P.N, 256)), dim3(256), 0, s, P,                                      \
                                reinterpret_cast<const float4*>(density12), split.albedo, out, visibility, num_visible, split.specular);           \
         else                                                                                                                                        \
@@ -1265,13 +1291,37 @@
     hipLaunchKernelGGL((gut_grad_gather_kernel<16, true>), dim3(div_up(P.N, 64)), dim3(256), 0, s, P, proj, reinterpret_cast<const float4*>(density12),
                        slots, have_partials ? 1 : 0, g_out, static_cast<float*>(nullptr), 0u, P.N);
 }
+bool gut_finalize_unfused() {
+    static const bool unfused = [] { const char* e = getenv("GRUT_GUT_UNFUSED_FINALIZE"); return e && e[0] == '1'; }();
+    return unfused;
+}
 void launch_grad_finalize(hipStream_t s, const GutParams& P, const GutProjected& proj, const float* density12, const float* sph,
                           const GutSplitSph& split, const GutGradSlots& slots, bool has_gdist, bool have_partials, float* g_rgb,
-                          const GutGradOut& g_out, float* g_sph, const GutSplitSphGrad& g_split, float* g_radiance, uint32_t first, uint32_t end) {
+                          const GutGradOut& g_out, float* g_sph, const GutSplitSphGrad& g_split, float* g_radiance, uint32_t first, uint32_t end,
+                          bool rows_in_records) {
     if (end > P.N) end = P.N;
     if (end <= first) return;
     const dim3 grid(div_up(end - first, 64)), block(256);
-    static const bool unfused = [] { const char* e = getenv("GRUT_GUT_UNFUSED_FINALIZE"); return e && e[0] == '1'; }();
+    const bool unfused = gut_finalize_unfused();
+    if (rows_in_records) {
+        const float4* none = nullptr;
+        if (split.specular) {
+            if (has_gdist)
+                hipLaunchKernelGGL((gut_grad_gather_kernel<20, false, true, true, true>), grid, block, 0, s, P, proj, none, slots, have_partials ? 1 : 0,
+                                   g_out, g_rgb, first, end, split.albedo, g_split.albedo, split.specular, g_split.specular);
+            else
+                hipLaunchKernelGGL((gut_grad_gather_kernel<16, false, true, true, true>), grid, block, 0, s, P, proj, none, slots, have_partials ? 1 : 0,
+                                   g_out, g_rgb, first, end, split.albedo, g_split.albedo, split.specular, g_split.specular);
+        } else {
+            if (has_gdist)
+                hipLaunchKernelGGL((gut_grad_gather_kernel<20, false, true, false, true>), grid, block, 0, s, P, proj, none, slots, have_partials ? 1 : 0,
+                                   g_out, g_rgb, first, end, sph, g_sph);
+            else
+                hipLaunchKernelGGL((gut_grad_gather_kernel<16, false, true, false, true>), grid, block, 0, s, P, proj, none, slots, have_partials ? 1 : 0,
+                                   g_out, g_rgb, first, end, sph, g_sph);
+        }
+        return;
+    }
     if (!unfused && split.specular) {
         if (has_gdist)
             hipLaunchKernelGGL((gut_grad_gather_kernel<20, false, true, true>), grid, block, 0, s, P, proj, reinterpret_cast<const float4*>(density12),
diff --git a/3dgrut_amd/gut_tracer.py b/3dgrut_amd/gut_tracer.py
--- a/3dgrut_amd/gut_tracer.py
+++ b/3dgrut_amd/gut_tracer.py
@@ -111,6 +111,17 @@
     return torch.empty(shape, **opts)
 
 
+def particle_tensors_in_place(cfg, mog_pos, mog_dns, mog_rot, mog_scl):
+    n = int(mog_pos.shape[0])
+    if n == 0 or cfg.feature_transform_type or cfg.particle_feature_half or int(cfg.k_buffer_size) != 0:
+        return None
+    parts = tuple(t.detach().reshape(n, -1) for t in (mog_pos, mog_dns, mog_rot, mog_scl))
+    for t, cols in zip(parts, (3, 1, 4, 3)):
+        if t.dtype != torch.float32 or not t.is_cuda or t.shape[1] != cols or not t.is_contiguous():
+            return None
+    return None if parts[2].data_ptr() % 16 else parts
+
+
 class _GutNative:
 
     def __init__(self, cfg: _abi.GutConfig):
@@ -148,7 +159,18 @@
     def trace_split(self, frame, particle_density, sph_albedo, sph_specular, ray_ori, ray_dir):
         return self._trace(frame, particle_density, (sph_albedo, sph_specular), ray_ori, ray_dir)
 
-    def _trace(self, frame, particle_density, sph, ray_ori, ray_dir):
+    @staticmethod
+    def _tensors_arg(parts):
+        pos, dns, rot, scl = parts
+        return _abi.GutParticleTensors(pos.data_ptr(), dns.data_ptr(), rot.data_ptr(), scl.data_ptr())
+
+    def trace_tensors(self, frame, parts, particle_sph, ray_ori, ray_dir):
+        return self._trace(frame, parts, (particle_sph,), ray_ori, ray_dir, tensors=True)
+
+    def trace_split_tensors(self, frame, parts, sph_albedo, sph_specular, ray_ori, ray_dir):
+        return self._trace(frame, parts, (sph_albedo, sph_specular), ray_ori, ray_dir, tensors=True)
+
+    def _trace(self, frame, particle_density, sph, ray_ori, ray_dir, tensors=False):
         dev = ray_ori.device
         H, W = frame.height, frame.width
         N = frame.num_particles
@@ -172,8 +194,9 @@
         else:
             out_feat, out_opa = _uninitialised((H, W, 3), **opts), _uninitialised((H, W, 1), **opts)
         frame.out_features, frame.out_opacity = (None, None) if half_out else (out_feat.data_ptr(), out_opa.data_ptr())
-        fn, name = (self.lib.gut_forward, "gut_forward") if len(sph) == 1 else (self.lib.gut_forward_split, "gut_forward_split")
-        _abi.check(fn(self.handle, _stream_ptr(dev), C.byref(frame), _ptr(particle_density), *map(_ptr, sph),
+        name = ("gut_forward" if len(sph) == 1 else "gut_forward_split") + ("_tensors" if tensors else "")
+        fn = getattr(self.lib, name)
+        _abi.check(fn(self.handle, _stream_ptr(dev), C.byref(frame), C.byref(self._tensors_arg(particle_density)) if tensors else _ptr(particle_density), *map(_ptr, sph),
                       _ptr(ray_ori), _ptr(ray_dir), _ptr(out_fd), _ptr(out_dist), _ptr(out_cnt), _ptr(vis_i32)), name)
         frame.out_features, frame.out_opacity = None, None
         if half_out:
@@ -228,6 +251,29 @@
                                                   _ptr(ray_ori), _ptr(ray_dir), _ptr(fd), _ptr(dist), _ptr(g_dist), C.byref(io), _ptr(g_sph)),
                    "gut_backward_unpacked")
         return g_pos, g_dns, g_rot, g_scl, g_sph
+
+    def trace_bwd_unpacked_tensors(self, frame, parts, particle_sph, ray_ori, ray_dir, fd, g_feat, g_opa, dist, g_dist):
+        n = parts[0].shape[0]
+        opts = dict(dtype=torch.float32, device=ray_ori.device)
+        g_pos, g_dns, g_rot, g_scl = torch.empty((n, 3), **opts), torch.empty((n, 1), **opts), torch.empty((n, 4), **opts), torch.empty((n, 3), **opts)
+        g_sph = torch.empty_like(particle_sph, dtype=torch.float32)
+        io = _abi.GutGradIO(_ptr(g_feat), _ptr(g_opa), _ptr(g_pos), _ptr(g_dns), _ptr(g_rot), _ptr(g_scl))
+        _abi.check(self.lib.gut_backward_unpacked_tensors(self.handle, _stream_ptr(ray_ori.device), C.byref(frame), C.byref(self._tensors_arg(parts)),
+                                                          _ptr(particle_sph), _ptr(ray_ori), _ptr(ray_dir), _ptr(fd), _ptr(dist), _ptr(g_dist),
+                                                          C.byref(io), _ptr(g_sph)), "gut_backward_unpacked_tensors")
+        return g_pos, g_dns, g_rot, g_scl, g_sph
+
+    def trace_bwd_unpacked_split_tensors(self, frame, parts, sph_albedo, sph_specular, ray_ori, ray_dir, fd, g_feat, g_opa, dist, g_dist):
+        n = parts[0].shape[0]
+        opts = dict(dtype=torch.float32, device=ray_ori.device)
+        g_pos, g_dns, g_rot, g_scl = torch.empty((n, 3), **opts), torch.empty((n, 1), **opts), torch.empty((n, 4), **opts), torch.empty((n, 3), **opts)
+        g_albedo, g_specular = torch.empty_like(sph_albedo), torch.empty_like(sph_specular)
+        io = _abi.GutGradIO(_ptr(g_feat), _ptr(g_opa), _ptr(g_pos), _ptr(g_dns), _ptr(g_rot), _ptr(g_scl))
+        _abi.check(self.lib.gut_backward_unpacked_split_tensors(self.handle, _stream_ptr(ray_ori.device), C.byref(frame), C.byref(self._tensors_arg(parts)),
+                                                                _ptr(sph_albedo), _ptr(sph_specular), _ptr(ray_ori), _ptr(ray_dir), _ptr(fd), _ptr(dist),
+                                                                _ptr(g_dist), C.byref(io), _ptr(g_albedo), _ptr(g_specular)),
+                   "gut_backward_unpacked_split_tensors")
+        return g_pos, g_dns, g_rot, g_scl, g_albedo, g_specular
 
     def trace_bwd_split(self, frame, particle_density, sph_albedo, sph_specular, ray_ori, ray_dir, fd, g_fd, dist, g_dist):
         g_density, g_albedo, g_specular = torch.empty_like(particle_density), torch.empty_like(sph_albedo), torch.empty_like(sph_specular)
@@ -338,15 +384,22 @@
     class _Autograd(torch.autograd.Function):
         @staticmethod
         def forward(ctx, native, frame, ray_ori, ray_dir, mog_pos, mog_rot, mog_scl, mog_dns, mog_sph, raw=False, exchange=None):
-            if raw:
-                particle_density = _abi.activate_pack(mog_pos, mog_dns, mog_rot, mog_scl)
-            else:
-                particle_density = _abi.pack_particles(mog_pos, mog_dns, mog_rot, mog_scl)
-            ctx.raw = (mog_dns, mog_rot, mog_scl) if raw else None
             particle_features = mog_sph.contiguous()
             if native.cfg.particle_feature_half and particle_features.dtype != torch.float16:
                 particle_features = particle_features.to(torch.float16)
-            fd, dist, cnt, vis, feat, opa = native.trace(frame, particle_density, particle_features, ray_ori, ray_dir)
+            ctx.parts = None
+            if not raw and exchange is None and particle_features.dtype == torch.float32:
+                ctx.parts = particle_tensors_in_place(native.cfg, mog_pos, mog_dns, mog_rot, mog_scl)
+            ctx.raw = (mog_dns, mog_rot, mog_scl) if raw else None
+            if ctx.parts is not None:
+                particle_density = None
+                fd, dist, cnt, vis, feat, opa = native.trace_tensors(frame, ctx.parts, particle_features, ray_ori, ray_dir)
+            else:
+                if raw:
+                    particle_density = _abi.activate_pack(mog_pos, mog_dns, mog_rot, mog_scl)
+                else:
+                    particle_density = _abi.pack_particles(mog_pos, mog_dns, mog_rot, mog_scl)
+                fd, dist, cnt, vis, feat, opa = native.trace(frame, particle_density, particle_features, ray_ori, ray_dir)
             ctx.save_for_backward(ray_ori, ray_dir, fd, dist, particle_density, particle_features)
             ctx.native, ctx.frame, ctx.exchange = native, frame, exchange
             feat = feat.unsqueeze(0)
@@ -360,6 +413,12 @@
             ray_ori, ray_dir, fd, dist, particle_density, particle_features = ctx.saved_tensors
             H, W = fd.shape[0], fd.shape[1]
             g_dist = None if g_dist is None else g_dist.contiguous()
+            if ctx.parts is not None:
+                g_pos, g_dns, g_rot, g_scl, g_sph = ctx.native.trace_bwd_unpacked_tensors(
+                    ctx.frame, ctx.parts, particle_features, ray_ori, ray_dir, fd,
+                    None if g_feat is None else g_feat.reshape(H, W, 3).contiguous(), None if g_opa is None else g_opa.reshape(H, W, 1).contiguous(),
+                    dist, g_dist)
+                return None, None, None, None, g_pos, g_rot, g_scl, g_dns, g_sph, None, None
             if ctx.exchange is None and ctx.raw is None and int(ctx.native.cfg.k_buffer_size) == 0:
                 g_pos, g_dns, g_rot, g_scl, g_sph = ctx.native.trace_bwd_unpacked(
                     ctx.frame, particle_density, particle_features, ray_ori, ray_dir, fd,
@@ -392,12 +451,14 @@
 
         @staticmethod
         def forward(ctx, native, frame, ray_ori, ray_dir, mog_pos, mog_rot, mog_scl, mog_dns, sph_albedo, sph_specular, raw=False):
-            if raw:
-                particle_density = _abi.activate_pack(mog_pos, mog_dns, mog_rot, mog_scl)
+            ctx.parts = None if raw else particle_tensors_in_place(native.cfg, mog_pos, mog_dns, mog_rot, mog_scl)
+            ctx.raw = (mog_dns, mog_rot, mog_scl) if raw else None
+            if ctx.parts is not None:
+                particle_density = None
+                fd, dist, cnt, vis, feat, opa = native.trace_split_tensors(frame, ctx.parts, sph_albedo, sph_specular, ray_ori, ray_dir)
             else:
-                particle_density = _abi.pack_particles(mog_pos, mog_dns, mog_rot, mog_scl)
-            ctx.raw = (mog_dns, mog_rot, mog_scl) if raw else None
-            fd, dist, cnt, vis, feat, opa = native.trace_split(frame, particle_density, sph_albedo, sph_specular, ray_ori, ray_dir)
+                particle_density = _abi.activate_pack(mog_pos, mog_dns, mog_rot, mog_scl) if raw else _abi.pack_particles(mog_pos, mog_dns, mog_rot, mog_scl)
+                fd, dist, cnt, vis, feat, opa = native.trace_split(frame, particle_density, sph_albedo, sph_specular, ray_ori, ray_dir)
             ctx.save_for_backward(ray_ori, ray_dir, fd, dist, particle_density, sph_albedo, sph_specular)
             ctx.native, ctx.frame = native, frame
             feat = feat.unsqueeze(0)
@@ -411,6 +472,12 @@
             ray_ori, ray_dir, fd, dist, particle_density, sph_albedo, sph_specular = ctx.saved_tensors
             H, W = fd.shape[0], fd.shape[1]
             g_dist = None if g_dist is None else g_dist.contiguous()
+            if ctx.parts is not None:
+                g_pos, g_dns, g_rot, g_scl, g_albedo, g_specular = ctx.native.trace_bwd_unpacked_split_tensors(
+                    ctx.frame, ctx.parts, sph_albedo, sph_specular, ray_ori, ray_dir, fd,
+                    None if g_feat is None else g_feat.reshape(H, W, 3).contiguous(), None if g_opa is None else g_opa.reshape(H, W, 1).contiguous(),
+                    dist, g_dist)
+                return None, None, None, None, g_pos, g_rot, g_scl, g_dns, g_albedo, g_specular, None
             if ctx.raw is None:
                 g_pos, g_dns, g_rot, g_scl, g_albedo, g_specular = ctx.native.trace_bwd_unpacked_split(
                     ctx.frame, particle_density, sph_albedo, sph_specular, ray_ori, ray_dir, fd,
diff --git a/include/grut_amd.h b/include/grut_amd.h
--- a/include/grut_amd.h
+++ b/include/grut_amd.h
@@ -146,6 +146,33 @@
                                 const float* ray_origin, const float* ray_direction,
                                 const void* feat_density, const float* hit_distance, const float* grad_hit_distance,
                                 const GutGradIO* io, float* grad_sph_albedo, float* grad_sph_specular);
+
+typedef struct GutParticleTensors {
+    const float* positions;
+    const float* density;
+    const float* rotation;
+    const float* scale;
+} GutParticleTensors;
+int gut_forward_tensors(GutHandle* handle, void* stream, const GutFrame* frame,
+                        const GutParticleTensors* particles, const void* particle_sph,
+                        const float* ray_origin, const float* ray_direction,
+                        void* out_feat_density, float* out_hit_distance,
+                        float* out_hit_count, int32_t* out_visibility);
+int gut_backward_unpacked_tensors(GutHandle* handle, void* stream, const GutFrame* frame,
+                                  const GutParticleTensors* particles, const void* particle_sph,
+                                  const float* ray_origin, const float* ray_direction,
+                                  const void* feat_density, const float* hit_distance, const float* grad_hit_distance,
+                                  const GutGradIO* io, float* grad_particle_sph);
+int gut_forward_split_tensors(GutHandle* handle, void* stream, const GutFrame* frame,
+                              const GutParticleTensors* particles, const float* sph_albedo, const float* sph_specular,
+                              const float* ray_origin, const float* ray_direction,
+                              void* out_feat_density, float* out_hit_distance,
+                              float* out_hit_count, int32_t* out_visibility);
+int gut_backward_unpacked_split_tensors(GutHandle* handle, void* stream, const GutFrame* frame,
+                                        const GutParticleTensors* particles, const float* sph_albedo, const float* sph_specular,
+                                        const float* ray_origin, const float* ray_direction,
+                                        const void* feat_density, const float* hit_distance, const float* grad_hit_distance,
+                                        const GutGradIO* io, float* grad_sph_albedo, float* grad_sph_specular);
 
 int gut_backward_factored(GutHandle* handle, void* stream, const GutFrame* frame,
                           const float* particle_density, const void* particle_sph,
```

New measurement: 1.091 billion rays/s (median of 6 runs). No clear change (+0.9%).
